# AlvinYH/Faster-VoxelPose

Measured on AMD Instinct MI355X. Metric: frames/sec at 5-view 80x80x20 voxel (heatmaps -> 3D joints); MPJPE vs ref (mm) in mpjpe_vs_ref_mm, higher is better.
Workload: dtype f32

## Files before the change

faster-voxelpose_amd/_capi.py:

```python
import ctypes as C
import os

_HERE = os.path.dirname(os.path.abspath(__file__))
LIB_NAME = "libfvp_hip.so"
ABI_VERSION = 17
LIB_PATH = os.path.join(_HERE, LIB_NAME)

FVP_CAM_FLOATS = 24
FVP_MAX_VIEWS = 8
FVP_MAX_JOINTS = 32
FVP_TRACK_MAX_DETS = 32
FVP_TRACK_MAX_TRACKS = 64
FVP_VIS_MAX_PEOPLE = 32
FVP_VIS_MAX_PRIMS = 64

OP_CONV, OP_POOL2, OP_CONVT2 = 0, 1, 2
EPI_RELU, EPI_RES, EPI_RES_AFTER_RELU = 1, 2, 4
K_PROJECT_WHOLE, K_PROJECT_TRIPLANE, K_CONV, K_SOFTARGMAX, K_OTHER, K_CONV_WINO, K_BACKBONE, K_CONV_WINO_SMALL, K_COUNT = 0, 1, 2, 3, 4, 5, 6, 7, 8
BB_CONV, BB_MAXPOOL, BB_DECONV = 0, 1, 2
BB_OUT_HEAT = 8
BB_STEM = 16
INGEST_SWAP_RB, INGEST_GENERAL = 1, 2
YUV_BT601_LIMITED, YUV_BT709_LIMITED, YUV_BT601_FULL, YUV_BT709_FULL = 0, 1, 2, 3


class FvpGeom(C.Structure):
    _fields_ = [("clamp_max", C.c_float), ("rt", C.c_float * 6), ("hm_w", C.c_float), ("hm_h", C.c_float),
                ("img_w", C.c_float), ("img_h", C.c_float), ("W", C.c_int32), ("H", C.c_int32),
                ("V", C.c_int32), ("J", C.c_int32), ("JP", C.c_int32)]


class FvpConvOp(C.Structure):
    _fields_ = [("kind", C.c_int32), ("src", C.c_int32), ("dst", C.c_int32), ("res", C.c_int32),
                ("cin", C.c_int32), ("cout", C.c_int32), ("kh", C.c_int32), ("kw", C.c_int32),
                ("h", C.c_int32), ("w", C.c_int32), ("flags", C.c_int32), ("w_off", C.c_int32),
                ("e_off", C.c_int32), ("cinp", C.c_int32), ("coutp", C.c_int32), ("wino_off", C.c_int32), ("pair_off", C.c_int32)]


class FvpBbOp(C.Structure):
    _fields_ = [(n, C.c_int32) for n in ("kind", "src", "dst", "res", "cin", "cinp", "cout", "coutp", "cbuf", "kh", "kw",
                                         "stride", "pad", "h", "w", "oh", "ow", "flags", "w_off", "e_off")]


_P = C.c_void_p
_I = C.c_int
_F = C.c_float
_G = C.POINTER(FvpGeom)

SIGNATURES = {
    "fvp_version": [],
    "fvp_diag_build": [],
    "fvp_sizeof": [_I],
    "fvp_error_string": [_I],
    "fvp_heatmaps_to_cl": [_P, _P, _I, _G, _P],
    "fvp_sample_grid": [_P, _P, _P, _I, _I, _I, _P, _G, _P, _P],
    "fvp_project_whole": [_P, _P, _P, _P, _P, _P, _I, _I, _I, _I, _G, _P, _P, _P],
    "fvp_project_columns": [_P, _P, _P, _P, _P, _P, _I, _I, _I, _I, _G, _P, _I, _P, _P],
    "fvp_joint_evidence": [_P, _P, _P, _P, _I, _I, _G, _P, _P, _P],
    "fvp_track_update": [_P, _P, _P, _P, _P, _P, _P, _P, _P, _I, _I, _I, _I, _I, _F, _I, _P],
    "fvp_track_smooth": [_P] * 12 + [_I] * 5 + [_F] * 6 + [_I, _P],
    "fvp_zmax": [_P, _P, C.c_long, _I, _P],
    "fvp_person_boxes": [_P, _I, _P, _P, _P, _P, _P],
    "fvp_project_individual": [_P, _P, _P, _P, _P, _P, _P, _P, _P, _P, _I, _I, _G, _P, _P],
    "fvp_triplane_max": [_P, _P, _I, _I, _I, _P],
    "fvp_project_individual_triplane": [_P, _P, _P, _P, _P, _P, _P, _P, _P, _P, _I, _I, _G, _P, _I, _P, _P],
    "fvp_conv_stack_run": [C.POINTER(FvpConvOp), _I, _P, C.POINTER(_P), _I, _I, _P, _I, _P],
    "fvp_conv_stack_run_fused_1d": [C.POINTER(FvpConvOp), _I, _P, _P, _P, _I, _P],
    "fvp_pack_conv": [_P, _P, _P, _P, _P, _P, _F, _I, C.POINTER(FvpConvOp), _P, _P],
    "fvp_nms_topk": [_P, _I, _I, _I, _I, _P, _P, _P, _P],
    "fvp_gather_proposals": [_P, _P, _P, _I, _I, _I, _I, _I, _I, _P, _P, _P, _P],
    "fvp_proposals": [_P, _P, _P, _P, _P, _F, _I, _I, _I, _P, _P, _P, _P],
    "fvp_proposal_layer": [_P, _P, _P, _P, _F, _I, _I, _P, _P],
    "fvp_softargmax_weightnet": [_P, _P, _P, _F, _I, _I, _I, _I, _I, _P, _P, _P, _P, _P],
    "fvp_pack_weightnet": [_P, _P, _P, _P, _P, _P, _F, _P, _P, _P, _P, _I, _I, _P, _P],
    "fvp_fuse_poses": [_P, _P, _P, _P, _P, _I, _I, _P, _P, _P, _P],
    "fvp_rasterise_heatmaps": [_P, _P, _I, _I, _I, _I, _I, C.c_double, C.c_double, C.c_double, _P, _P, _I, _P],
    "fvp_ingest_frames": [_P, _I, _I, _I, C.POINTER(_F), C.POINTER(_F), C.POINTER(_F), _I, _I, _I, _P, _P, _P],
    "fvp_ingest_nv12": [_P, _P, _I, _I, _I, C.c_long, C.c_long, C.c_long, C.c_long, _I, C.POINTER(_F), C.POINTER(_F),
                        C.POINTER(_F), _I, _I, _P, _P, _P],
    "fvp_draw_poses": [_P, _I, _I, _I, _I, _P, _P, _P, _I, _I, C.POINTER(C.c_int32), _I, C.POINTER(C.c_uint8), _I, _I, _I, _I,
                       _F, _P],
    "fvp_draw_poses_nv12": [_P, _P, _I, _I, _I, _I, C.c_long, C.c_long, C.c_long, C.c_long, _I, _P, _P, _P, _I, _I,
                            C.POINTER(C.c_int32), _I, C.POINTER(C.c_uint8), _I, _I, _I, _I, _F, _P],
    "fvp_person_rois": [_P, _P, _P, _I, _I, _I, _I, C.c_uint32, _I, _F, _F, _F, _F, _P, _P, _P, _P],
    "fvp_crop_rois": [_P, _I, _I, _I, _P, _I, _I, C.POINTER(_F), C.POINTER(_F), _I, _I, _I, _P, _P, _P],
    "fvp_crop_rois_nv12": [_P, _P, _I, _I, _I, C.c_long, C.c_long, C.c_long, C.c_long, _I, _P, _I, _I, C.POINTER(_F),
                           C.POINTER(_F), _I, _I, _P, _P, _P],
    "fvp_joint_visibility": [_P, _P, _P, _P, _P, _I, _I, _I, _I, C.POINTER(C.c_int32), C.POINTER(_F), _I, _F, _I, _I, _P, _P,
                             _P, _P],
    "fvp_bb_input": [_P, _P, _I, _I, _I, _I, _P],
    "fvp_bb_pack": [_P, _P, _P, _P, _P, _P, _F, C.POINTER(FvpBbOp), _P, _P, _P],
    "fvp_bb_run": [C.POINTER(FvpBbOp), _I, _P, _P, C.POINTER(_P), _I, _I, _P, _I, _P, _P],
    "fvp_bb_tune": [C.POINTER(FvpBbOp), _I, _P, _P, C.POINTER(_P), _I, _I, _P],
    "fvp_prof_enable": [_I],
    "fvp_prof_read": [_I, C.POINTER(C.c_double), C.POINTER(C.c_int64), C.POINTER(C.c_double)],
    "fvp_prof_reset": [],
}
_RESTYPES = {"fvp_error_string": C.c_char_p}


class FvpError(RuntimeError):
    pass


def bind(lib):
    for name, args in SIGNATURES.items():
        fn = getattr(lib, name)
        fn.argtypes = args
        fn.restype = _RESTYPES.get(name, C.c_int)
    return lib


_lib = None


def load():
    global _lib
    if _lib is None:
        if not os.path.isfile(LIB_PATH):
            raise FvpError(
                f"{LIB_PATH} not found: the HIP extension is required (there is no CPU fallback). "
                "Build it with `python -c 'import __graft_entry__ as g; g.build()'` or "
                "`faster-voxelpose_amd/csrc/build.sh`.")
        import torch
        _lib = bind(C.CDLL(LIB_PATH))
        if _lib.fvp_version() != ABI_VERSION:
            raise FvpError("libfvp_hip.so ABI version mismatch (rebuild with faster-voxelpose_amd/csrc/build.sh)")
        if _lib.fvp_sizeof(0) != C.sizeof(FvpGeom) or _lib.fvp_sizeof(1) != C.sizeof(FvpConvOp) \
                or _lib.fvp_sizeof(2) != C.sizeof(FvpBbOp):
            raise FvpError("libfvp_hip.so struct layout differs from the ctypes mirrors in _capi.py")
    return _lib


def check(lib, rc, what=""):
    if rc != 0:
        msg = lib.fvp_error_string(rc)
        raise FvpError(f"{what}: error {rc}: {msg.decode() if msg else '?'}")
```

faster-voxelpose_amd/csrc/fvp_project.hip:

```cpp
#include <hip/hip_runtime.h>

#include <cfloat>
#include <cstdlib>

#include "fvp_common.h"
#include "fvp_geom.h"

namespace fvp {

template <int NV>
__global__ void __launch_bounds__(256) k_heat_to_cl(const float* __restrict__ heat, float* __restrict__ cl,
                                                    int J, int HW) {
  const int pix = blockIdx.x * 256 + threadIdx.x;
  const size_t bv = blockIdx.y;
  if (pix >= HW) return;
  const float* src = heat + bv * size_t(J) * HW + pix;
  float v[4 * NV];
#pragma unroll
  for (int j = 0; j < 4 * NV; ++j) v[j] = (j < J) ? src[size_t(j) * HW] : 0.0f;
  float4* dst = reinterpret_cast<float4*>(cl + (bv * HW + pix) * size_t(4 * NV));
#pragma unroll
  for (int q = 0; q < NV; ++q) dst[q] = make_float4(v[4 * q], v[4 * q + 1], v[4 * q + 2], v[4 * q + 3]);
}

__global__ void __launch_bounds__(256) k_sample_grid(const float* __restrict__ ax, const float* __restrict__ ay,
                                                     const float* __restrict__ az, int nx, int ny, int nz,
                                                     const Cam* __restrict__ cams, FvpGeom g,
                                                     float* __restrict__ grid) {
  const int n = nx * ny * nz;
  const int i = blockIdx.x * 256 + threadIdx.x;
  const int v = blockIdx.y;
  if (i >= n) return;
  const int iz = i % nz, iy = (i / nz) % ny, ix = i / (nz * ny);
  float gx, gy;
  project_norm(cams[v], g, ax[ix], ay[iy], az[iz], gx, gy);
  grid[(size_t(v) * n + i) * 2 + 0] = gx;
  grid[(size_t(v) * n + i) * 2 + 1] = gy;
}

template <int NV>
__device__ __forceinline__ void backproject_point(const float* __restrict__ heat_cl_frame,
                                                  const Cam* __restrict__ cams, const FvpGeom& g, float wx,
                                                  float wy, float wz, float (&acc)[4 * NV]) {
  const size_t view_stride = size_t(g.H) * g.W * (4 * NV);
  for (int v = 0; v < g.V; ++v) {
    float gx, gy;
    project_norm(cams[v], g, wx, wy, wz, gx, gy);
    const Taps t = bilinear_taps(gx, gy, g.W, g.H);
    float s[4 * NV];
    if (t.inside) {
      sample_view<NV>(heat_cl_frame + v * view_stride, t, s);
    } else {
#pragma unroll
      for (int c = 0; c < 4 * NV; ++c) s[c] = 0.0f;
    }
#pragma unroll
    for (int c = 0; c < 4 * NV; ++c) acc[c] = (v == 0) ? s[c] : __fadd_rn(acc[c], s[c]);
  }
  const float nv = float(g.V);
#pragma unroll
  for (int c = 0; c < 4 * NV; ++c) acc[c] = clampf(__fdiv_rn(acc[c], nv), 0.0f, 1.0f);
}

__global__ void __launch_bounds__(256)
k_joint_evidence(const float* __restrict__ heat_cl, const Cam* __restrict__ cams, const int* __restrict__ frame_set,
                 const float* __restrict__ fused, int B, int N, FvpGeom g, float* __restrict__ views,
                 float* __restrict__ conf) {
  const int i = blockIdx.x * 256 + threadIdx.x;
  const int J = g.J, JP = g.JP;
  if (i >= B * N * J) return;
  const int bn = i / J, j = i - bn * J;
  const int b = bn / N, n = bn - b * N;
  const bool valid = fused[size_t(bn) * J * 5 + 3] >= 0.0f;
  const float* p = fused + size_t(i) * 5;
  const float wx = p[0], wy = p[1], wz = p[2];
  const size_t view_stride = size_t(g.H) * g.W * JP;
  const float* frame = heat_cl + size_t(b) * g.V * view_stride;
  const Cam* cm = cams + size_t(frame_set[b]) * g.V;
  float acc = 0.0f;
  for (int v = 0; v < g.V; ++v) {
    float px = 0.0f, py = 0.0f, depth = 0.0f, s = 0.0f;
    if (valid) {
      float gx, gy;
      project_pixel(cm[v], wx, wy, wz, px, py, depth);
      pixel_to_norm(g, px, py, gx, gy);
      const Taps t = bilinear_taps(gx, gy, g.W, g.H);
      if (t.inside) {
        const float* cl = frame + v * view_stride + j;
        float h[4];
#pragma unroll
        for (int k = 0; k < 4; ++k) h[k] = ((t.inside >> k) & 1) ? cl[size_t(t.off[k]) * JP] : 0.0f;
        s = __fmul_rn(h[0], t.w[0]);
#pragma unroll
        for (int k = 1; k < 4; ++k) s = __fmaf_rn(h[k], t.w[k], s);
      }
    }
    acc = (v == 0) ? s : __fadd_rn(acc, s);
    if (views)
      reinterpret_cast<float4*>(views)[((size_t(b) * g.V + v) * N + n) * J + j] = make_float4(px, py, depth, s);
  }
  if (conf) conf[i] = clampf(__fdiv_rn(acc, float(g.V)), 0.0f, 1.0f);
}

struct VisPrims {
  int n;
  int ik[FVP_VIS_MAX_PRIMS];
  float r[FVP_VIS_MAX_PRIMS];
};

__device__ __forceinline__ float dot3(float p0, float p1, float p2, float q0, float q1, float q2) {
  return __fadd_rn(__fadd_rn(__fmul_rn(p0, q0), __fmul_rn(p1, q1)), __fmul_rn(p2, q2));
}

__global__ void __launch_bounds__(256)
k_joint_visibility(const float* __restrict__ fused, const Cam* __restrict__ cams, const int* __restrict__ frame_set,
                   const int* __restrict__ ids, const float* __restrict__ views, int V, int N, int J, VisPrims prm,
                   float guard, float xmax, float ymax, int* __restrict__ occluder, float* __restrict__ vis_conf,
                   int* __restrict__ vis_count) {
  __shared__ float4 pose[FVP_VIS_MAX_PEOPLE * FVP_MAX_JOINTS];
  __shared__ int present[FVP_VIS_MAX_PEOPLE];
  __shared__ float seen_s[FVP_MAX_VIEWS * FVP_MAX_JOINTS];
  __shared__ int seen[FVP_MAX_VIEWS * FVP_MAX_JOINTS];
  const int b = blockIdx.x / N, n = blockIdx.x - b * N;
  const int tid = threadIdx.x;
  const float* frame = fused + size_t(b) * N * J * 5;
  for (int q = tid; q < N * J; q += 256) {
    const float x = frame[q * 5 + 0], y = frame[q * 5 + 1], z = frame[q * 5 + 2];
    const bool fin = fabsf(x) <= FLT_MAX && fabsf(y) <= FLT_MAX && fabsf(z) <= FLT_MAX;
    pose[q] = make_float4(x, y, z, fin ? 1.0f : 0.0f);
  }
  if (tid < N) present[tid] = frame[tid * J * 5 + 3] >= 0.0f && (!ids || ids[b * N + tid] >= 0);
  __syncthreads();
  const int v = tid / J, j = tid - v * J;
  if (v < V) {
    const Cam& cm = cams[size_t(frame_set[b]) * V + v];
    const float c0 = cm.T[0], c1 = cm.T[1], c2 = cm.T[2];
    const float4 P = pose[n * J + j];
    const float d10 = __fsub_rn(P.x, c0), d11 = __fsub_rn(P.y, c1), d12 = __fsub_rn(P.z, c2);
    const float a = dot3(d10, d11, d12, d10, d11, d12);
    const float len = sqrtf(a);
    int occ = -2;
    if (present[n] && P.w != 0.0f && len > guard) {
      const float smax = __fsub_rn(1.0f, __fdiv_rn(guard, len));
      float best = 0.0f;
      occ = -1;
      for (int m = 0; m < N; ++m) {
        if (!present[m]) continue;
        for (int l = 0; l < prm.n; ++l) {
          const int pi = prm.ik[l] & 255, pk = prm.ik[l] >> 8;
          const float4 A = pose[m * J + pi], Bq = pose[m * J + pk];
          if (A.w == 0.0f || Bq.w == 0.0f || (m == n && (pi == j || pk == j))) continue;
          const float d20 = __fsub_rn(Bq.x, A.x), d21 = __fsub_rn(Bq.y, A.y), d22 = __fsub_rn(Bq.z, A.z);
          const float r00 = __fsub_rn(c0, A.x), r01 = __fsub_rn(c1, A.y), r02 = __fsub_rn(c2, A.z);
          const float e = dot3(d20, d21, d22, d20, d21, d22);
          const float f = dot3(d20, d21, d22, r00, r01, r02);
          const float c = dot3(d10, d11, d12, r00, r01, r02);
          float sv, tv;
          if (e == 0.0f) {
            tv = 0.0f;
            sv = clampf(__fdiv_rn(-c, a), 0.0f, smax);
          } else {
            const float bb = dot3(d10, d11, d12, d20, d21, d22);
            const float den = __fsub_rn(__fmul_rn(a, e), __fmul_rn(bb, bb));
            sv = den > 0.0f ? clampf(__fdiv_rn(__fsub_rn(__fmul_rn(bb, f), __fmul_rn(c, e)), den), 0.0f, smax) : 0.0f;
            tv = __fdiv_rn(__fadd_rn(__fmul_rn(bb, sv), f), e);
            if (tv < 0.0f) {
              tv = 0.0f;
              sv = clampf(__fdiv_rn(-c, a), 0.0f, smax);
            } else if (tv > 1.0f) {
              tv = 1.0f;
              sv = clampf(__fdiv_rn(__fsub_rn(bb, c), a), 0.0f, smax);
            }
          }
          const float w0 = __fsub_rn(__fadd_rn(c0, __fmul_rn(d10, sv)), __fadd_rn(A.x, __fmul_rn(d20, tv)));
          const float w1 = __fsub_rn(__fadd_rn(c1, __fmul_rn(d11, sv)), __fadd_rn(A.y, __fmul_rn(d21, tv)));
          const float w2 = __fsub_rn(__fadd_rn(c2, __fmul_rn(d12, sv)), __fadd_rn(A.z, __fmul_rn(d22, tv)));
          const float rr = __fmul_rn(prm.r[l], prm.r[l]);
          if (dot3(w0, w1, w2, w0, w1, w2) <= rr && (occ < 0 || sv < best)) {
            best = sv;
            occ = m;
          }
        }
      }
    }
    const size_t o = ((size_t(b) * V + v) * N + n) * J + j;
    if (occluder) occluder[o] = occ;
    if (views) {
      const float4 e4 = reinterpret_cast<const float4*>(views)[o];
      seen[tid] = occ == -1 && e4.z > 0.0f && e4.x >= 0.0f && e4.x <= xmax && e4.y >= 0.0f && e4.y <= ymax;
      seen_s[tid] = e4.w;
    }
  }
  if (!views) return;
  __syncthreads();
  if (tid < J) {
    float sum = 0.0f;
    int cnt = 0;
    for (int u = 0; u < V; ++u)
      if (seen[u * J + tid]) {
        sum = __fadd_rn(sum, seen_s[u * J + tid]);
        ++cnt;
      }
    const size_t o = (size_t(b) * N + n) * J + tid;
    if (vis_conf) vis_conf[o] = cnt ? clampf(__fdiv_rn(sum, float(cnt)), 0.0f, 1.0f) : 0.0f;
    if (vis_count) vis_count[o] = cnt;
  }
}

template <int NV>
__global__ void __launch_bounds__(256)
k_project_whole(const float* __restrict__ heat_cl, const Cam* __restrict__ cams, const int* __restrict__ frame_set,
                const float* __restrict__ ax, const float* __restrict__ ay, const float* __restrict__ az, int X,
                int Y, int Z, FvpGeom g, float* __restrict__ cubes, float* __restrict__ zmax) {
  __shared__ float sm[4 * NV][256];
  const int cpb = 256 / Z;
  const int b = blockIdx.y;
  const int t = threadIdx.x;
  const int cl_ = t / Z, z = t - cl_ * Z;
  const int col = blockIdx.x * cpb + cl_;
  const int ncol = X * Y;
  const bool active = cl_ < cpb && col < ncol;
  const int J = g.J;
  float acc[4 * NV];
#pragma unroll
  for (int c = 0; c < 4 * NV; ++c) acc[c] = 0.0f;
  if (active) {
    const int x = col / Y, y = col - x * Y;
    const float* frame = heat_cl + size_t(b) * g.V * g.H * g.W * (4 * NV);
    backproject_point<NV>(frame, cams + size_t(frame_set[b]) * g.V, g, ax[x], ay[y], az[z], acc);
    if (cubes) {
      const size_t vox = size_t(col) * Z + z;
      const size_t nvox = size_t(ncol) * Z;
#pragma unroll
      for (int c = 0; c < 4 * NV; ++c)
        if (c < J) cubes[(size_t(b) * J + c) * nvox + vox] = acc[c];
    }
  }
  if (zmax) {
#pragma unroll
    for (int c = 0; c < 4 * NV; ++c) sm[c][t] = acc[c];
    __syncthreads();
    for (int item = t; item < cpb * J; item += 256) {
      const int c = item / cpb, k = item - c * cpb;
      const int cc = blockIdx.x * cpb + k;
      if (cc < ncol) {
        float m = sm[c][k * Z];
        for (int zz = 1; zz < Z; ++zz) m = fmaxf(m, sm[c][k * Z + zz]);
        zmax[(size_t(b) * J + c) * ncol + cc] = m;
      }
    }
  }
}

template <int NV>
__global__ void __launch_bounds__(256)
k_project_individual(const float* __restrict__ heat_cl, const Cam* __restrict__ cams,
                     const int* __restrict__ frame_set, const int* __restrict__ person_frame,
                     const uint8_t* __restrict__ person_valid, const int* __restrict__ boxes,
                     const float* __restrict__ fx, const float* __restrict__ fy, const float* __restrict__ fz, int C,
                     FvpGeom g, float* __restrict__ cubes) {
  const int p = blockIdx.y;
  const int lv = blockIdx.x * 256 + threadIdx.x;
  const int nvox = C * C * C;
  if (lv >= nvox) return;
  const int J = g.J;
  const int lz = lv % C, ly = (lv / C) % C, lx = lv / (C * C);
  const int* bx = boxes + p * 9;
  const int gx_ = bx[0] + lx, gy_ = bx[1] + ly, gz_ = bx[2] + lz;
  bool in = (!person_valid || person_valid[p]);
  in = in && bx[3] < bx[6] && bx[4] < bx[7] && bx[5] < bx[8];
  in = in && gx_ >= bx[3] && gx_ < bx[6] && gy_ >= bx[4] && gy_ < bx[7] && gz_ >= bx[5] && gz_ < bx[8];
  float acc[4 * NV];
#pragma unroll
  for (int c = 0; c < 4 * NV; ++c) acc[c] = 0.0f;
  if (in) {
    const int b = person_frame[p];
    const float* frame = heat_cl + size_t(b) * g.V * g.H * g.W * (4 * NV);
    backproject_point<NV>(frame, cams + size_t(frame_set[b]) * g.V, g, fx[gx_], fy[gy_], fz[gz_], acc);
  }
#pragma unroll
  for (int c = 0; c < 4 * NV; ++c)
    if (c < J) cubes[(size_t(p) * J + c) * nvox + lv] = acc[c];
}

template <int PER>
__global__ void __launch_bounds__(256)
k_triplane_max(const float* __restrict__ cubes, float* __restrict__ planes, int J, int C) {
  HIP_DYNAMIC_SHARED(float, slab)
  const int j = blockIdx.x, p = blockIdx.y, t = threadIdx.x;
  const int CC = C * C, ld = C + 1;
  const float* cube = cubes + (size_t(p) * J + j) * CC * C;
  float* pxy = planes + ((size_t(p) * 3 + 0) * J + j) * CC;
  float* pxz = planes + ((size_t(p) * 3 + 1) * J + j) * CC;
  float* pyz = planes + ((size_t(p) * 3 + 2) * J + j) * CC;
  float run[PER];
#pragma unroll
  for (int i = 0; i < PER; ++i) run[i] = -INFINITY;
  for (int x = 0; x < C; ++x) {
    __syncthreads();
    int ncell = CC;
    FVP_OPAQUE(ncell);
#pragma unroll
    for (int i = 0; i < PER; ++i) {
      const int cell = t + i * 256;
      if (cell < ncell) {
        const float v = cube[size_t(x) * CC + cell];
        slab[(cell / C) * ld + (cell % C)] = v;
        run[i] = fmaxf(run[i], v);
      }
    }
    __syncthreads();
    for (int r = t; r < 2 * C; r += 256) {
      if (r < C) {
        float m = slab[r * ld];
        for (int z = 1; z < C; ++z) m = fmaxf(m, slab[r * ld + z]);
        pxy[x * C + r] = m;
      } else {
        const int z = r - C;
        float m = slab[z];
        for (int y = 1; y < C; ++y) m = fmaxf(m, slab[y * ld + z]);
        pxz[x * C + z] = m;
      }
    }
  }
#pragma unroll
  for (int i = 0; i < PER; ++i) {
    const int cell = t + i * 256;
    if (cell < CC) pyz[cell] = run[i];
  }
}

struct TapD {
  int off[4];
  float w[4];
  int inside;
};

template <int SRC>
__device__ __forceinline__ int quad_bcast_i(int v) {
  return __builtin_amdgcn_update_dpp(0, v, SRC * 0x55, 0xf, 0xf, false);
}
template <int SRC>
__device__ __forceinline__ TapD quad_bcast(const TapD& t) {
  TapD r;
#pragma unroll
  for (int k = 0; k < 4; ++k) {
    r.off[k] = quad_bcast_i<SRC>(t.off[k]);
    r.w[k] = __int_as_float(quad_bcast_i<SRC>(__float_as_int(t.w[k])));
  }
  r.inside = quad_bcast_i<SRC>(t.inside);
  return r;
}

__device__ __forceinline__ TapD make_taps(const Cam& cm, const FvpGeom& g, float wx, float wy, float wz) {
  float gx, gy;
  project_norm(cm, g, wx, wy, wz, gx, gy);
  const Taps t = bilinear_taps(gx, gy, g.W, g.H);
  TapD d;
#pragma unroll
  for (int k = 0; k < 4; ++k) { d.off[k] = t.off[k]; d.w[k] = t.w[k]; }
  d.inside = t.inside;
  return d;
}

__device__ __forceinline__ void sample4(const float* __restrict__ cl, int JP, int ch0, const TapD& t, bool first,
                                        float (&acc)[4]) {
  float4 v[4];
#pragma unroll
  for (int k = 0; k < 4; ++k) {
    const bool in = (t.inside >> k) & 1;
    v[k] = *reinterpret_cast<const float4*>(cl + size_t(in ? t.off[k] : 0) * JP + ch0);
    if (!in) v[k] = make_float4(0.f, 0.f, 0.f, 0.f);
  }
  float s[4] = {__fmul_rn(v[0].x, t.w[0]), __fmul_rn(v[0].y, t.w[0]), __fmul_rn(v[0].z, t.w[0]),
                __fmul_rn(v[0].w, t.w[0])};
#pragma unroll
  for (int k = 1; k < 4; ++k) {
    s[0] = __fmaf_rn(v[k].x, t.w[k], s[0]);
    s[1] = __fmaf_rn(v[k].y, t.w[k], s[1]);
    s[2] = __fmaf_rn(v[k].z, t.w[k], s[2]);
    s[3] = __fmaf_rn(v[k].w, t.w[k], s[3]);
  }
#pragma unroll
  for (int i = 0; i < 4; ++i) acc[i] = first ? s[i] : __fadd_rn(acc[i], s[i]);
}

template <int NVL>
__device__ __forceinline__ void whole_point_quad(const float* __restrict__ frame, const Cam* __restrict__ cm,
                                                 const FvpGeom& g, int q, bool active, float wx, float wy, float wz,
                                                 float (&out)[NVL][4]) {
  const int JP = g.JP;
  const size_t view_stride = size_t(g.H) * g.W * JP;
  float acc[NVL][4];
#pragma unroll
  for (int n = 0; n < NVL; ++n)
#pragma unroll
    for (int i = 0; i < 4; ++i) acc[n][i] = 0.0f;
  TapD mine;
  mine.inside = 0;
#pragma unroll
  for (int k = 0; k < 4; ++k) { mine.off[k] = 0; mine.w[k] = 0.0f; }
  if (active && q < g.V) mine = make_taps(cm[q], g, wx, wy, wz);
  auto add_view = [&](const TapD& tv, int v) {
#pragma unroll
    for (int n = 0; n < NVL; ++n) {
      const int ch0 = 16 * n + 4 * q;
      if (ch0 < JP) {
        if (tv.inside) sample4(frame + v * view_stride, JP, ch0, tv, v == 0, acc[n]);
        else if (v == 0) { acc[n][0] = acc[n][1] = acc[n][2] = acc[n][3] = 0.0f; }
      }
    }
  };
  { const TapD tv = quad_bcast<0>(mine); if (active) add_view(tv, 0); }
  if (g.V > 1) { const TapD tv = quad_bcast<1>(mine); if (active) add_view(tv, 1); }
  if (g.V > 2) { const TapD tv = quad_bcast<2>(mine); if (active) add_view(tv, 2); }
  if (g.V > 3) { const TapD tv = quad_bcast<3>(mine); if (active) add_view(tv, 3); }
  for (int v = 4; v < g.V; ++v)
    if (active) add_view(make_taps(cm[v], g, wx, wy, wz), v);
  const float nv = float(g.V);
#pragma unroll
  for (int n = 0; n < NVL; ++n)
#pragma unroll
    for (int i = 0; i < 4; ++i) out[n][i] = clampf(__fdiv_rn(acc[n][i], nv), 0.0f, 1.0f);
}

template <int NVL>
__global__ void __launch_bounds__(1024)
k_project_whole_q(const float* __restrict__ heat_cl, const Cam* __restrict__ cams,
                  const int* __restrict__ frame_set, const float* __restrict__ ax, const float* __restrict__ ay,
                  const float* __restrict__ az, int X, int Y, int Z, int B, int nblk, FvpGeom g,
                  float* __restrict__ cubes, float* __restrict__ zmax) {
  __shared__ float sm[16 * NVL][256];
  const int cpb = 256 / Z;
  int b, bxi;
  if (B % 8 == 0) {
    const int xcd = blockIdx.x & 7, j = blockIdx.x >> 3;
    b = xcd + 8 * (j / nblk);
    bxi = j % nblk;
  } else {
    b = blockIdx.x / nblk;
    bxi = blockIdx.x % nblk;
  }
  const int t = threadIdx.x, q = t & 3, vl = t >> 2;
  const int cl_ = vl / Z, z = vl - cl_ * Z;
  const int col = bxi * cpb + cl_;
  const int ncol = X * Y;
  const bool active = cl_ < cpb && col < ncol;
  const int J = g.J, JP = g.JP;
  const size_t view_stride = size_t(g.H) * g.W * JP;
  const float* frame = heat_cl + size_t(b) * g.V * view_stride;
  const Cam* cm = cams + size_t(frame_set[b]) * g.V;
  float wx = 0.0f, wy = 0.0f, wz = 0.0f;
  if (active) {
    const int x = col / Y, y = col - x * Y;
    wx = ax[x];
    wy = ay[y];
    wz = az[z];
  }
  float val[NVL][4];
  whole_point_quad<NVL>(frame, cm, g, q, active, wx, wy, wz, val);
  const size_t vox = size_t(col) * Z + z;
  const size_t nvox = size_t(ncol) * Z;
#pragma unroll
  for (int n = 0; n < NVL; ++n)
#pragma unroll
    for (int i = 0; i < 4; ++i) {
      const int c = 16 * n + 4 * q + i;
      const float v = val[n][i];
      if (zmax) sm[c][vl] = active ? v : 0.0f;
      if (cubes && active && c < J) cubes[(size_t(b) * J + c) * nvox + vox] = v;
    }
  if (zmax) {
    __syncthreads();
    for (int item = t; item < cpb * J; item += 1024) {
      const int c = item / cpb, k = item - c * cpb;
      const int cc = bxi * cpb + k;
      if (cc < ncol) {
        float m = sm[c][k * Z];
        for (int zz = 1; zz < Z; ++zz) m = fmaxf(m, sm[c][k * Z + zz]);
        zmax[(size_t(b) * J + c) * ncol + cc] = m;
      }
    }
  }
}

template <int NVL>
__global__ void __launch_bounds__(1024)
k_project_columns_q(const float* __restrict__ heat_cl, const Cam* __restrict__ cams, const int* __restrict__ frame_set,
                    const float* __restrict__ ax, const float* __restrict__ ay, const float* __restrict__ az, int Y,
                    int Z, int ncol, int N, FvpGeom g, const long long* __restrict__ flat, float* __restrict__ feat1d) {
  const int pi = blockIdx.x, b = pi / N;
  const int t = threadIdx.x, q = t & 3, z = t >> 2;
  const long long col = flat[pi];
  const bool active = z < Z && col >= 0 && col < ncol;
  const int J = g.J;
  const size_t view_stride = size_t(g.H) * g.W * g.JP;
  const float* frame = heat_cl + size_t(b) * g.V * view_stride;
  const Cam* cm = cams + size_t(frame_set[b]) * g.V;
  float wx = 0.0f, wy = 0.0f, wz = 0.0f;
  if (active) {
    const int x = int(col) / Y, y = int(col) - x * Y;
    wx = ax[x];
    wy = ay[y];
    wz = az[z];
  }
  float val[NVL][4];
  whole_point_quad<NVL>(frame, cm, g, q, active, wx, wy, wz, val);
#pragma unroll
  for (int n = 0; n < NVL; ++n)
#pragma unroll
    for (int i = 0; i < 4; ++i) {
      const int c = 16 * n + 4 * q + i;
      if (z < Z && c < J) feat1d[(size_t(pi) * J + c) * Z + z] = active ? val[n][i] : 0.0f;
    }
}

#if FVP_DIAG
template <int NVL>
__global__ void __launch_bounds__(1024)
k_project_triplane(const float* __restrict__ heat_cl, const Cam* __restrict__ cams, const int* __restrict__ frame_set,
                   const int* __restrict__ person_frame, const uint8_t* __restrict__ person_valid,
                   const int* __restrict__ boxes, const float* __restrict__ fx, const float* __restrict__ fy,
                   const float* __restrict__ fz, int C, int nP, int chunks, int ppf, FvpGeom g,
                   float* __restrict__ planes) {
  __shared__ float sm_xz[4 * NVL * 4][256];
  __shared__ float sm_xy[16][4 * NVL * 4];
  int p, chunk;
  {
    const int id = blockIdx.x;
    const int bpf = ppf * chunks;
    const int nframes = nP / ppf;
    if (nframes % 8 == 0) {
      const int xcd = id & 7, j = id >> 3;
      const int frame = xcd + 8 * (j / bpf), r = j % bpf;
      p = frame * ppf + r / chunks;
      chunk = r % chunks;
    } else {
      p = id / chunks;
      chunk = id % chunks;
    }
  }
  if (person_valid && !person_valid[p]) return;
  const int* bx = boxes + p * 9;
  const int tl0 = bx[0], tl1 = bx[1], tl2 = bx[2];
  const int s0 = bx[3], s1 = bx[4], s2 = bx[5], e0 = bx[6], e1 = bx[7], e2 = bx[8];
  if (s0 >= e0 || s1 >= e1 || s2 >= e2) return;
  const int t = threadIdx.x, q = t & 3, lane = t & 63, wave = t >> 6;
  const int J = g.J, JP = g.JP, CC = C * C;
  const int rows = 256 / C > 0 ? 256 / C : 1;
  const int cell_l = t >> 2;
  const int cell = chunk * 256 + cell_l;
  const int y = cell / C, z = cell - y * C;
  const int y_first = (chunk * 256) / C;
  if (tl1 + y_first >= e1 || tl1 + y_first + rows - 1 < s1) return;
  const int gy_ = tl1 + y, gz_ = tl2 + z;
  const bool yz_in = y < C && gy_ >= s1 && gy_ < e1 && gz_ >= s2 && gz_ < e2;
  const int b = person_frame[p];
  const size_t view_stride = size_t(g.H) * g.W * JP;
  const float* frame = heat_cl + size_t(b) * g.V * view_stride;
  const Cam* cm = cams + size_t(frame_set[b]) * g.V;
  const float wy = yz_in ? fy[gy_] : 0.0f, wz = yz_in ? fz[gz_] : 0.0f;
  float* pxy = planes + (size_t(p) * 3 + 0) * J * CC;
  float* pxz = planes + (size_t(p) * 3 + 1) * J * CC;
  float* pyz = planes + (size_t(p) * 3 + 2) * J * CC;
  const int wpr = C >= 16 ? C / 16 : 1;
  float run[NVL][4];
#pragma unroll
  for (int n = 0; n < NVL; ++n)
#pragma unroll
    for (int i = 0; i < 4; ++i) run[n][i] = 0.0f;
  const float nv = float(g.V);
  const int lx0 = s0 - tl0, lx1 = e0 - tl0;
  for (int lx = lx0; lx < lx1; ++lx) {
    const float wx = fx[tl0 + lx];
    float acc[NVL][4];
#pragma unroll
    for (int n = 0; n < NVL; ++n)
#pragma unroll
      for (int i = 0; i < 4; ++i) acc[n][i] = 0.0f;
    TapD mine;
    mine.inside = 0;
#pragma unroll
    for (int k = 0; k < 4; ++k) { mine.off[k] = 0; mine.w[k] = 0.0f; }
    if (yz_in && q < g.V) mine = make_taps(cm[q], g, wx, wy, wz);
    auto add_view = [&](const TapD& tv, int v) {
#pragma unroll
      for (int n = 0; n < NVL; ++n) {
        const int ch0 = 16 * n + 4 * q;
        if (ch0 < JP) {
          if (tv.inside) sample4(frame + v * view_stride, JP, ch0, tv, v == 0, acc[n]);
          else if (v == 0) { acc[n][0] = acc[n][1] = acc[n][2] = acc[n][3] = 0.0f; }
        }
      }
    };
    { const TapD tv = quad_bcast<0>(mine); if (yz_in) add_view(tv, 0); }
    if (g.V > 1) { const TapD tv = quad_bcast<1>(mine); if (yz_in) add_view(tv, 1); }
    if (g.V > 2) { const TapD tv = quad_bcast<2>(mine); if (yz_in) add_view(tv, 2); }
    if (g.V > 3) { const TapD tv = quad_bcast<3>(mine); if (yz_in) add_view(tv, 3); }
    for (int v = 4; v < g.V; ++v)
      if (yz_in) add_view(make_taps(cm[v], g, wx, wy, wz), v);
#pragma unroll
    for (int n = 0; n < NVL; ++n)
#pragma unroll
      for (int i = 0; i < 4; ++i) {
        acc[n][i] = clampf(__fdiv_rn(acc[n][i], nv), 0.0f, 1.0f);
        run[n][i] = fmaxf(run[n][i], acc[n][i]);
      }
    __syncthreads();
#pragma unroll
    for (int n = 0; n < NVL; ++n)
#pragma unroll
      for (int i = 0; i < 4; ++i) {
        const int c = 16 * n + 4 * q + i;
        sm_xz[c][cell_l] = acc[n][i];
        float m = acc[n][i];
        const int zw = C < 16 ? C : 16;
        for (int o = (zw >> 1) * 4; o >= 4; o >>= 1) m = fmaxf(m, __shfl_xor(m, o));
        if (C >= 16) { if ((lane >> 2) == 0) sm_xy[wave][c] = m; }
        else if (((lane >> 2) & (zw - 1)) == 0 && c < J && y < C && m > 0.0f) pxy[size_t(c) * CC + lx * C + y] = m;
      }
    __syncthreads();
    if (C >= 16) {
      const int nitem = rows * J;
      if (t < nitem) {
        const int r = t / J, c = t - r * J;
        float m = sm_xy[r * wpr][c];
        for (int k = 1; k < wpr; ++k) m = fmaxf(m, sm_xy[r * wpr + k][c]);
        const int yy = y_first + r;
        if (yy < C && m > 0.0f) pxy[size_t(c) * CC + lx * C + yy] = m;
      }
    }
    for (int item = t; item < J * C; item += 1024) {
      const int c = item / C, zz = item - c * C;
      float m = sm_xz[c][zz];
      for (int r = 1; r < rows; ++r) m = fmaxf(m, sm_xz[c][r * C + zz]);
      if (m > 0.0f) {
        if (chunks > 1) atomicMax(reinterpret_cast<int*>(&pxz[size_t(c) * CC + lx * C + zz]), __float_as_int(m));
        else pxz[size_t(c) * CC + lx * C + zz] = m;
      }
    }
  }
  if (y < C) {
#pragma unroll
    for (int n = 0; n < NVL; ++n)
#pragma unroll
      for (int i = 0; i < 4; ++i) {
        const int c = 16 * n + 4 * q + i;
        if (c < J && run[n][i] > 0.0f) pyz[size_t(c) * CC + y * C + z] = run[n][i];
      }
  }
}

#endif

}
#include "fvp_project_lds.h"
namespace fvp {

__global__ void __launch_bounds__(256) k_zmax(const float* __restrict__ cubes, float* __restrict__ zmax, long n, int Z) {
  const long i = long(blockIdx.x) * 256 + threadIdx.x;
  if (i >= n) return;
  const float* c = cubes + i * Z;
  float m = c[0];
  for (int z = 1; z < Z; ++z) m = fmaxf(m, c[z]);
  zmax[i] = m;
}

__global__ void __launch_bounds__(64)
k_person_boxes(const float* __restrict__ centers, int n, const float* __restrict__ consts, int f0, int f1, int f2,
               int c0, int c1, int c2, int* __restrict__ boxes, float* __restrict__ offset) {
  const int i = blockIdx.x * 64 + threadIdx.x;
  if (i >= n) return;
  const float* pc = centers + size_t(i) * 7;
  const int fine[3] = {f0, f1, f2}, cube[3] = {c0, c1, c2};
  int tl[3], m[3];
  for (int a = 0; a < 3; ++a) {
    const float v = __fadd_rn(__fmul_rn(pc[a], consts[a]), consts[3 + a]);
    tl[a] = int(rintf(v));
    const float whole = consts[6 + a], ind = consts[9 + a];
    float o = __fmul_rn(__fdiv_rn(float(tl[a]), float(fine[a] - 1)), whole);
    o = __fadd_rn(__fsub_rn(o, __fdiv_rn(whole, 2.0f)), __fdiv_rn(ind, 2.0f));
    offset[size_t(i) * 3 + a] = o;
  }
  for (int a = 0; a < 2; ++a) {
    const float r = __fmul_rn(__fdiv_rn(__fsub_rn(1.0f, pc[5 + a]), 2.0f), float(cube[a] - 1));
    m[a] = int(r);
    if (m[a] < 0) m[a] = 0;
  }
  m[2] = 0;
  for (int a = 0; a < 3; ++a) {
    const int s = tl[a] + m[a], e = tl[a] + cube[a] - m[a];
    boxes[i * 9 + a] = tl[a];
    boxes[i * 9 + 3 + a] = s >= 0 ? s : 0;
    boxes[i * 9 + 6 + a] = e <= fine[a] ? e : fine[a];
  }
}

}

using namespace fvp;

#define FVP_NV_SWITCH(nv, CALL)     \
  switch (nv) {                     \
    case 1: { CALL(1); } break;     \
    case 2: { CALL(2); } break;     \
    case 3: { CALL(3); } break;     \
    case 4: { CALL(4); } break;     \
    case 5: { CALL(5); } break;     \
    case 6: { CALL(6); } break;     \
    case 7: { CALL(7); } break;     \
    case 8: { CALL(8); } break;     \
    default: return FVP_ELIMIT;     \
  }

static int check_geom(const FvpGeom* g) {
  if (!g) return FVP_EINVAL;
  if (g->V < 1 || g->V > FVP_MAX_VIEWS || g->J < 1 || g->J > FVP_MAX_JOINTS) return FVP_ELIMIT;
  if (g->JP != 4 * ((g->J + 3) / 4) || g->W < 2 || g->H < 2) return FVP_EINVAL;
  return 0;
}

extern "C" int fvp_heatmaps_to_cl(const float* heat, float* heat_cl, int B, const FvpGeom* g, fvp_stream_t s) {
  FVP_REQUIRE(heat && heat_cl && B >= 0);
  if (int e = check_geom(g)) return e;
  if (B == 0) return 0;
  const int HW = g->H * g->W;
  ProfScope ps(FVP_K_OTHER, as_stream(s));
#define CALL(NV)                                                                                             \
  auto k = &k_heat_to_cl<NV>;                                                                                \
  hipLaunchKernelGGL(k, dim3(ceil_div(HW, 256), B * g->V), dim3(256), 0, as_stream(s), heat, heat_cl, g->J, HW);
  FVP_NV_SWITCH(g->JP / 4, CALL)
#undef CALL
  return launch_status();
}

extern "C" int fvp_sample_grid(const float* ax, const float* ay, const float* az, int nx, int ny, int nz,
                               const float* cams, const FvpGeom* g, float* grid, fvp_stream_t s) {
  FVP_REQUIRE(ax && ay && az && cams && grid && nx > 0 && ny > 0 && nz > 0);
  if (int e = check_geom(g)) return e;
  const int n = nx * ny * nz;
  ProfScope ps(FVP_K_OTHER, as_stream(s));
  hipLaunchKernelGGL(k_sample_grid, dim3(ceil_div(n, 256), g->V), dim3(256), 0, as_stream(s), ax, ay, az, nx, ny,
                     nz, reinterpret_cast<const Cam*>(cams), *g, grid);
  return launch_status();
}

extern "C" int fvp_project_whole(const float* heat_cl, const float* cams, const int32_t* frame_set,
                                 const float* ax, const float* ay, const float* az, int X, int Y, int Z, int B,
                                 const FvpGeom* g, float* cubes, float* zmax, fvp_stream_t s) {
  FVP_REQUIRE(heat_cl && cams && frame_set && ax && ay && az && (cubes || zmax) && X > 0 && Y > 0 && Z > 0);
  if (int e = check_geom(g)) return e;
  FVP_LIMIT(Z <= 256);
  if (B == 0) return 0;
  const int cpb = 256 / Z;
  ProfScope ps(FVP_K_PROJECT_WHOLE, as_stream(s));
  static const bool no_quad = fvp::diag_env("FVP_WHOLE_NO_QUAD") != nullptr;
  const int nvl = ceil_div(g->JP, 16);
  if (!no_quad && nvl <= 2) {
    const int nblk = ceil_div(X * Y, cpb);
    if (nvl == 1)
      hipLaunchKernelGGL(k_project_whole_q<1>, dim3(nblk * B), dim3(1024), 0, as_stream(s), heat_cl,
                         reinterpret_cast<const Cam*>(cams), frame_set, ax, ay, az, X, Y, Z, B, nblk, *g, cubes, zmax);
    else
      hipLaunchKernelGGL(k_project_whole_q<2>, dim3(nblk * B), dim3(1024), 0, as_stream(s), heat_cl,
                         reinterpret_cast<const Cam*>(cams), frame_set, ax, ay, az, X, Y, Z, B, nblk, *g, cubes, zmax);
    return launch_status();
  }
#define CALL(NV)                                                                                              \
  auto k = &k_project_whole<NV>;                                                                              \
  hipLaunchKernelGGL(k, dim3(ceil_div(X * Y, cpb), B), dim3(256), 0, as_stream(s), heat_cl,                   \
                     reinterpret_cast<const Cam*>(cams), frame_set, ax, ay, az, X, Y, Z, *g, cubes, zmax);
  FVP_NV_SWITCH(g->JP / 4, CALL)
#undef CALL
  return launch_status();
}

extern "C" int fvp_joint_evidence(const float* heat_cl, const float* cams, const int32_t* frame_set,
                                  const float* fused_poses, int B, int N, const FvpGeom* g, float* views,
                                  float* joint_conf, fvp_stream_t s) {
  FVP_REQUIRE(heat_cl && cams && frame_set && fused_poses && (views || joint_conf) && B >= 0 && N >= 0);
  if (int e = check_geom(g)) return e;
  FVP_LIMIT(size_t(B) * N * g->J * g->V < (size_t(1) << 29));
  if (B == 0 || N == 0) return 0;
  ProfScope ps(FVP_K_OTHER, as_stream(s));
  hipLaunchKernelGGL(k_joint_evidence, dim3(ceil_div(B * N * g->J, 256)), dim3(256), 0, as_stream(s), heat_cl,
                     reinterpret_cast<const Cam*>(cams), frame_set, fused_poses, B, N, *g, views, joint_conf);
  return launch_status();
}

extern "C" int fvp_joint_visibility(const float* fused_poses, const float* cams, const int32_t* frame_set,
                                    const int32_t* ids, const float* views, int B, int V, int N, int J,
                                    const int32_t* prims, const float* radius_mm, int L, float guard_mm, int Hs, int Ws,
                                    int32_t* occluder, float* vis_conf, int32_t* vis_count, fvp_stream_t s) {
  FVP_REQUIRE(fused_poses && cams && frame_set && ((prims && radius_mm) || L <= 0));
  FVP_REQUIRE((occluder || vis_conf || vis_count) && (views || (!vis_conf && !vis_count)));
  FVP_REQUIRE(B >= 0 && V >= 1 && N >= 1 && J >= 1 && Hs >= 1 && Ws >= 1 && L >= 0);
  FVP_REQUIRE(guard_mm >= 0.0f && guard_mm <= FLT_MAX);
  FVP_LIMIT(N <= FVP_VIS_MAX_PEOPLE && J <= FVP_MAX_JOINTS && V <= FVP_MAX_VIEWS && L <= FVP_VIS_MAX_PRIMS);
  VisPrims prm;
  prm.n = L;
  for (int l = 0; l < FVP_VIS_MAX_PRIMS; ++l) {
    prm.ik[l] = 0;
    prm.r[l] = 0.0f;
    if (l >= L) continue;
    const int i = prims[2 * l], k = prims[2 * l + 1];
    FVP_REQUIRE(i >= 0 && i < J && k >= 0 && k < J && radius_mm[l] > 0.0f && radius_mm[l] <= FLT_MAX);
    prm.ik[l] = i | (k << 8);
    prm.r[l] = radius_mm[l];
  }
  if (B == 0) return 0;
  ProfScope ps(FVP_K_OTHER, as_stream(s));
  hipLaunchKernelGGL(k_joint_visibility, dim3(B * N), dim3(256), 0, as_stream(s), fused_poses,
                     reinterpret_cast<const Cam*>(cams), frame_set, ids, views, V, N, J, prm, guard_mm, float(Ws - 1),
                     float(Hs - 1), occluder, vis_conf, vis_count);
  return launch_status();
}

extern "C" int fvp_project_columns(const float* heat_cl, const float* cams, const int32_t* frame_set, const float* ax,
                                   const float* ay, const float* az, int X, int Y, int Z, int B, const FvpGeom* g,
                                   const int64_t* flat, int N, float* feat1d, fvp_stream_t s) {
  FVP_REQUIRE(heat_cl && cams && frame_set && ax && ay && az && flat && feat1d && X > 0 && Y > 0 && Z > 0 && N > 0);
  if (int e = check_geom(g)) return e;
  FVP_LIMIT(Z <= 256 && g->JP <= 32);
  if (B == 0) return 0;
  ProfScope ps(FVP_K_PROJECT_WHOLE, as_stream(s));
  const int threads = ceil_div(4 * Z, 64) * 64;
  if (g->JP <= 16)
    hipLaunchKernelGGL(k_project_columns_q<1>, dim3(B * N), dim3(threads), 0, as_stream(s), heat_cl,
                       reinterpret_cast<const Cam*>(cams), frame_set, ax, ay, az, Y, Z, X * Y, N, *g,
                       reinterpret_cast<const long long*>(flat), feat1d);
  else
    hipLaunchKernelGGL(k_project_columns_q<2>, dim3(B * N), dim3(threads), 0, as_stream(s), heat_cl,
                       reinterpret_cast<const Cam*>(cams), frame_set, ax, ay, az, Y, Z, X * Y, N, *g,
                       reinterpret_cast<const long long*>(flat), feat1d);
  return launch_status();
}

extern "C" int fvp_zmax(const float* cubes, float* zmax, long n, int Z, fvp_stream_t s) {
  FVP_REQUIRE(cubes && zmax && n >= 0 && Z > 0);
  if (n == 0) return 0;
  hipLaunchKernelGGL(k_zmax, dim3(unsigned((n + 255) / 256)), dim3(256), 0, as_stream(s), cubes, zmax, n, Z);
  return launch_status();
}

extern "C" int fvp_person_boxes(const float* centers, int n, const float* consts, const int32_t* fine_cube,
                                int32_t* boxes, float* offset, fvp_stream_t s) {
  FVP_REQUIRE(centers && consts && fine_cube && boxes && offset && n >= 0);
  if (n == 0) return 0;
  hipLaunchKernelGGL(k_person_boxes, dim3(ceil_div(n, 64)), dim3(64), 0, as_stream(s), centers, n, consts,
                     fine_cube[0], fine_cube[1], fine_cube[2], fine_cube[3], fine_cube[4], fine_cube[5], boxes,
                     offset);
  return launch_status();
}

static int check_cube(int C) {
  if (C < 4 || C > 256 || (C & (C - 1)) != 0) return FVP_ELIMIT;
  return 0;
}

extern "C" int fvp_project_individual(const float* heat_cl, const float* cams, const int32_t* frame_set,
                                      const int32_t* person_frame, const uint8_t* person_valid,
                                      const int32_t* boxes, const float* fx, const float* fy, const float* fz,
                                      const int32_t* fine, int C, int nP, const FvpGeom* g, float* cubes,
                                      fvp_stream_t s) {
  FVP_REQUIRE(heat_cl && cams && frame_set && person_frame && boxes && fx && fy && fz && cubes && nP >= 0);
  (void)fine;
  if (int e = check_geom(g)) return e;
  if (int e = check_cube(C)) return e;
  if (nP == 0) return 0;
  ProfScope ps(FVP_K_OTHER, as_stream(s));
#define CALL(NV)                                                                                                 \
  auto k = &k_project_individual<NV>;                                                                            \
  hipLaunchKernelGGL(k, dim3(ceil_div(C * C * C, 256), nP), dim3(256), 0, as_stream(s), heat_cl,                 \
                     reinterpret_cast<const Cam*>(cams), frame_set, person_frame, person_valid, boxes, fx, fy, fz, \
                     C, *g, cubes);
  FVP_NV_SWITCH(g->JP / 4, CALL)
#undef CALL
  return launch_status();
}

extern "C" int fvp_triplane_max(const float* cubes, float* planes, int nP, int J, int C, fvp_stream_t s) {
  FVP_REQUIRE(cubes && planes && nP >= 0 && J > 0);
  if (int e = check_cube(C)) return e;
  FVP_LIMIT(C <= 128);
  if (nP == 0) return 0;
  ProfScope ps(FVP_K_OTHER, as_stream(s));
  const int per = (C * C + 255) / 256;
  const dim3 grid(J, nP);
  const size_t lds = size_t(C) * (C + 1) * sizeof(float);
#define FVP_TRIMAX(PER_) hipLaunchKernelGGL(k_triplane_max<PER_>, grid, dim3(256), lds, as_stream(s), cubes, planes, J, C)
  if (per <= 1) FVP_TRIMAX(1);
  else if (per <= 4) FVP_TRIMAX(4);
  else if (per <= 16) FVP_TRIMAX(16);
  else FVP_TRIMAX(64);
#undef FVP_TRIMAX
  return launch_status();
}

extern "C" int fvp_project_individual_triplane(const float* heat_cl, const float* cams, const int32_t* frame_set,
                                               const int32_t* person_frame, const uint8_t* person_valid,
                                               const int32_t* boxes, const float* fx, const float* fy,
                                               const float* fz, const int32_t* fine, int C, int nP, const FvpGeom* g,
                                               float* planes, int persons_per_frame, const float* fine_grid,
                                               fvp_stream_t s) {
  FVP_REQUIRE(heat_cl && cams && frame_set && person_frame && boxes && fx && fy && fz && planes && nP >= 0);
  FVP_REQUIRE(!fine_grid || fine);
  if (int e = check_geom(g)) return e;
  if (int e = check_cube(C)) return e;
  if (nP == 0) return 0;
  const int ppf = (persons_per_frame > 0 && nP % persons_per_frame == 0) ? persons_per_frame : nP;
  [[maybe_unused]] const int chunks = ceil_div(C * C, 256);
  const int nvl = ceil_div(g->JP, 16);
  ProfScope ps(FVP_K_PROJECT_TRIPLANE, as_stream(s));
  const int F0 = fine_grid ? fine[0] : 0, F1 = fine_grid ? fine[1] : 0, F2 = fine_grid ? fine[2] : 0;
  const int nby = ceil_div(C, kBY);
#if FVP_DIAG
  const int nbx = ceil_div(C, kBX);
  static const bool gather = fvp::diag_env("FVP_TRIPLANE_GATHER") != nullptr;
  const bool quad_form = fvp::diag_env("FVP_TRIPLANE_QUAD") != nullptr;
  static const int tri_ablate_env = fvp::diag_env("FVP_TRI_ABLATE") ? atoi(fvp::diag_env("FVP_TRI_ABLATE")) : 0;
  const char* tt_env = fvp::diag_env("FVP_TRI_TWO_TILE");
  const bool staged = fvp::diag_env("FVP_TRIPLANE_STAGED") != nullptr;
  const bool force_lane = fvp::diag_env("FVP_TRIPLANE_LANE") != nullptr;
  const bool lane_form = !gather && !quad_form && g->JP <= 20 && ((staged && g->JP != 16) || force_lane);
  const int tri_ablate = (tri_ablate_env & ~16) | ((tt_env ? atoi(tt_env) != 0 : lane_form) ? 16 : 0);
  auto cap_lim = [](int cap) { const char* e = fvp::diag_env("FVP_TRI_CAP_PX"); const int v = e ? atoi(e) : cap; return v > 0 && v < cap ? v : cap; };
  const int cap_px = int((36 * 1024) / (size_t(g->JP) * 4));
  const size_t lds = 2 * size_t(cap_px) * g->JP * 4 + 64;
  if (lane_form) {
    const int lq = (g->JP / 4) | 1;
    const int cap_px = int((36 * 1024) / (size_t(lq) * 16));
    const size_t lds = 2 * size_t(cap_px) * lq * 16 + 64;
    FVP_LIMIT(size_t(cap_px) * lq * 4 >= size_t(kBX * kBY + (kBX + kBY) * 32) * g->JP);
#define CALL2(NQ_, CACHED_)                                                                                       \
  {                                                                                                                \
    static LdsOptIn optin;                                                                                         \
    auto k = &k_project_triplane_lds2<NQ_, CACHED_>;                                                              \
    if (int e = lds_opt_in(optin, reinterpret_cast<const void*>(k), lds)) return e;                                \
    hipLaunchKernelGGL(k, dim3(nbx * nby * nP), dim3(kTriThreads), lds, as_stream(s), heat_cl,                     \
                       reinterpret_cast<const Cam*>(cams), frame_set, person_frame, person_valid, boxes, fx, fy, fz, C, \
                       nP, nbx, nby, ppf, cap_px, *g, fine_grid, F0, F1, F2, planes, tri_ablate, cap_lim(cap_px));                  \
  }
#define CASE2(NQ_) case NQ_: if (fine_grid) CALL2(NQ_, true) else CALL2(NQ_, false) break;
    switch (g->JP / 4) {
      CASE2(1) CASE2(2) CASE2(3) CASE2(4) CASE2(5)
      default: return FVP_ELIMIT;
    }
#undef CASE2
#undef CALL2
    return launch_status();
  }
  const bool blk_form = !gather && !quad_form && !staged;
#else
  constexpr bool blk_form = true;
#endif
  if (blk_form && nvl <= 2) {
    const int nbx2 = ceil_div(C, kBlkBX);
    const int bz = nvl == 2 ? 16 : kBlkBZ;
    int zsh = 0;
    while ((1 << zsh) < C) ++zsh;
    const size_t lds_z = (size_t(kBlkBX + kBY) << zsh) * (g->JP + 1) * 4;
#if FVP_DIAG
    const char* zr_env = fvp::diag_env("FVP_TRI_ZRES");
    const bool zres = zr_env && atoi(zr_env) != 0 && (1 << zsh) >= bz && lds_z <= kTriZresMaxLds;
#else
    constexpr bool zres = false;
#endif
    const size_t lds_b = zres ? lds_z : size_t(kBlkBX * kBY + (kBlkBX + kBY) * bz) * (g->JP + 1) * 4;
#define CALLB(NVL_, CACHED_, ZRES_)                                                                                          \
  hipLaunchKernelGGL((k_project_triplane_blk<NVL_, CACHED_, ZRES_>), dim3(nbx2 * nby * nP), dim3(kBlkThreads), lds_b,       \
                     as_stream(s), heat_cl, reinterpret_cast<const Cam*>(cams), frame_set, person_frame, person_valid, boxes, \
                     fx, fy, fz, C, nP, nbx2, nby, ppf, *g, fine_grid, F0, F1, F2, planes, zsh)
#if FVP_DIAG
#define CALLB2(NVL_)                                                                     \
  {                                                                                      \
    if (fine_grid) { if (zres) CALLB(NVL_, true, true); else CALLB(NVL_, true, false); } \
    else { if (zres) CALLB(NVL_, false, true); else CALLB(NVL_, false, false); }         \
  }
#else
#define CALLB2(NVL_)                                                                     \
  {                                                                                      \
    if (fine_grid) CALLB(NVL_, true, false); else CALLB(NVL_, false, false);             \
  }
#endif
    const bool q5 = nvl == 2 && g->JP == 20 && !zres && fvp::diag_env("FVP_TRI_NO_Q5") == nullptr;
    if (q5) {
      if (fine_grid)
        hipLaunchKernelGGL((k_project_triplane_blk<2, true, false, true>), dim3(nbx2 * nby * nP), dim3(kBlkThreads), lds_b, as_stream(s),
                           heat_cl, reinterpret_cast<const Cam*>(cams), frame_set, person_frame, person_valid, boxes, fx, fy, fz, C, nP,
                           nbx2, nby, ppf, *g, fine_grid, F0, F1, F2, planes, zsh);
      else
        hipLaunchKernelGGL((k_project_triplane_blk<2, false, false, true>), dim3(nbx2 * nby * nP), dim3(kBlkThreads), lds_b, as_stream(s),
                           heat_cl, reinterpret_cast<const Cam*>(cams), frame_set, person_frame, person_valid, boxes, fx, fy, fz, C, nP,
                           nbx2, nby, ppf, *g, fine_grid, F0, F1, F2, planes, zsh);
    } else if (nvl == 2) CALLB2(2) else CALLB2(1)
#undef CALLB2
#undef CALLB
    return launch_status();
  }
#if FVP_DIAG
  if (!gather && nvl <= 2) {
    FVP_LIMIT(cap_px >= kBX * kBY + (kBX + kBY) * (nvl == 1 ? 32 : 16));
#define CALL(NVL_, CACHED_)                                                                                        \
  {                                                                                                                \
    static LdsOptIn optin;                                                                                         \
    auto k = &k_project_triplane_lds<NVL_, CACHED_>;                                                               \
    if (int e = lds_opt_in(optin, reinterpret_cast<const void*>(k), lds)) return e;                                \
    hipLaunchKernelGGL(k, dim3(nbx * nby * nP), dim3(kTriThreads), lds, as_stream(s), heat_cl,                     \
                       reinterpret_cast<const Cam*>(cams), frame_set, person_frame, person_valid, boxes, fx, fy, fz, C, \
                       nP, nbx, nby, ppf, cap_px, *g, fine_grid, F0, F1, F2, planes, tri_ablate, cap_lim(cap_px));                  \
  }
    if (nvl == 1) {
      if (fine_grid) CALL(1, true) else CALL(1, false)
    } else {
      if (fine_grid) CALL(2, true) else CALL(2, false)
    }
#undef CALL
    return launch_status();
  }
  if (nvl == 1) {
    auto k = &k_project_triplane<1>;
    hipLaunchKernelGGL(k, dim3(chunks * nP), dim3(1024), 0, as_stream(s), heat_cl, reinterpret_cast<const Cam*>(cams),
                       frame_set, person_frame, person_valid, boxes, fx, fy, fz, C, nP, chunks, ppf, *g, planes);
  } else if (nvl == 2) {
    auto k = &k_project_triplane<2>;
    hipLaunchKernelGGL(k, dim3(chunks * nP), dim3(1024), 0, as_stream(s), heat_cl, reinterpret_cast<const Cam*>(cams),
                       frame_set, person_frame, person_valid, boxes, fx, fy, fz, C, nP, chunks, ppf, *g, planes);
  } else {
    return FVP_ELIMIT;
  }
  return launch_status();
#else
  return FVP_ELIMIT;
#endif
}
```

faster-voxelpose_amd/csrc/fvp_project_lds.h:

```cpp
#pragma once
#include <type_traits>
#include <climits>

namespace fvp {

typedef float f32x2 __attribute__((ext_vector_type(2)));
#ifndef FVP_TRI_PACKED
#define FVP_TRI_PACKED 1
#endif
#ifndef FVP_TRI_EXPLICIT_AS
#define FVP_TRI_EXPLICIT_AS 1
#endif

typedef float f32x4v __attribute__((ext_vector_type(4)));
__device__ __forceinline__ float4 lds_ld4(const float* p) {
  const f32x4v v = *(const __attribute__((address_space(3))) f32x4v*)p;
  return make_float4(v.x, v.y, v.z, v.w);
}
__device__ __forceinline__ float4 glb_ld4(const float* p) {
  const f32x4v v = *(const __attribute__((address_space(1))) f32x4v*)p;
  return make_float4(v.x, v.y, v.z, v.w);
}

struct TapL {
  int base;
  int dx, dy;
  float w[4];
};

template <int SRC>
__device__ __forceinline__ TapL quad_bcast_l(const TapL& t) {
  TapL r;
  r.base = quad_bcast_i<SRC>(t.base);
  r.dx = quad_bcast_i<SRC>(t.dx);
  r.dy = quad_bcast_i<SRC>(t.dy);
#pragma unroll
  for (int k = 0; k < 4; ++k) r.w[k] = __int_as_float(quad_bcast_i<SRC>(__float_as_int(t.w[k])));
  return r;
}

__device__ __forceinline__ void tap_origin(float gx, float gy, int W, int H, int& x0, int& y0, float (&w)[4], int& inside) {
  const float ix = __fmul_rn(__fadd_rn(gx, 1.0f), 0.5f * float(W - 1));
  const float iy = __fmul_rn(__fadd_rn(gy, 1.0f), 0.5f * float(H - 1));
  const float x0f = floorf(ix), y0f = floorf(iy);
  const float x1f = __fadd_rn(x0f, 1.0f), y1f = __fadd_rn(y0f, 1.0f);
  w[0] = __fmul_rn(__fsub_rn(x1f, ix), __fsub_rn(y1f, iy));
  w[1] = __fmul_rn(__fsub_rn(ix, x0f), __fsub_rn(y1f, iy));
  w[2] = __fmul_rn(__fsub_rn(x1f, ix), __fsub_rn(iy, y0f));
  w[3] = __fmul_rn(__fsub_rn(ix, x0f), __fsub_rn(iy, y0f));
  x0 = int(x0f);
  y0 = int(y0f);
  const bool x0in = x0 >= 0 && x0 < W, x1in = x0 + 1 >= 0 && x0 + 1 < W;
  const bool y0in = y0 >= 0 && y0 < H, y1in = y0 + 1 >= 0 && y0 + 1 < H;
  inside = (x0in && y0in ? 1 : 0) | (x1in && y0in ? 2 : 0) | (x0in && y1in ? 4 : 0) | (x1in && y1in ? 8 : 0);
}

__device__ __forceinline__ int imax(int a, int b) { return a > b ? a : b; }
__device__ __forceinline__ int imin(int a, int b) { return a < b ? a : b; }
template <int CTRL>
__device__ __forceinline__ int dpp_i(int v) { return __builtin_amdgcn_update_dpp(0, v, CTRL, 0xf, 0xf, false); }
__device__ __forceinline__ int row_max(int v) {
  v = imax(v, dpp_i<0xB1>(v));
  v = imax(v, dpp_i<0x4E>(v));
  v = imax(v, dpp_i<0x141>(v));
  v = imax(v, dpp_i<0x140>(v));
  return v;
}

__device__ __forceinline__ void plane_max(float* cell, int vv) { atomicMax(reinterpret_cast<int*>(cell), vv); }

constexpr int kBX = 8, kBY = 4;
constexpr int kTriThreads = kBX * kBY * 4 * 4;

#if FVP_DIAG
template <int NVL, bool CACHED>
__global__ void __launch_bounds__(kTriThreads, 4)
k_project_triplane_lds(const float* __restrict__ heat_cl, const Cam* __restrict__ cams, const int* __restrict__ frame_set,
                       const int* __restrict__ person_frame, const uint8_t* __restrict__ person_valid,
                       const int* __restrict__ boxes, const float* __restrict__ fx, const float* __restrict__ fy,
                       const float* __restrict__ fz, int C, int nP, int nbx, int nby, int ppf, int cap_px, FvpGeom g,
                       const float* __restrict__ fgrid, int F0, int F1, int F2, float* __restrict__ planes, int ablate, int cap_lim) {
  constexpr int BZ = NVL == 1 ? 32 : 16;
  constexpr int VPT = BZ / 4;
  constexpr int OWN = VPT / 4;
  HIP_DYNAMIC_SHARED(float, smem)
  constexpr int NT = kTriThreads;
  const int J = g.J, JP = g.JP, CC = C * C, V = g.V, W = g.W, H = g.H;
  const int tile_sz = cap_px * JP;
  int* rect = reinterpret_cast<int*>(smem + 2 * size_t(tile_sz));
  int p, blk;
  {
    const int id = blockIdx.x;
    const int bpp = nbx * nby, bpf = ppf * bpp;
    const int nframes = nP / ppf;
    if (nframes % 8 == 0) {
      const int xcd = id & 7, j = id >> 3;
      const int frame = xcd + 8 * (j / bpf), r = j % bpf;
      p = frame * ppf + r / bpp;
      blk = r % bpp;
    } else {
      p = id / bpp;
      blk = id % bpp;
    }
  }
  if (person_valid && !person_valid[p]) return;
  const int* bx = boxes + p * 9;
  const int tl0 = bx[0], tl1 = bx[1], tl2 = bx[2];
  const int s0 = bx[3], s1 = bx[4], s2 = bx[5], e0 = bx[6], e1 = bx[7], e2 = bx[8];
  if (s0 >= e0 || s1 >= e1 || s2 >= e2) return;
  const int xb = blk / nby, yb = blk - xb * nby;
  const int gx0 = s0 + xb * kBX, gy0 = s1 + yb * kBY;
  if (gx0 >= e0 || gy0 >= e1) return;

  const int t = threadIdx.x, q = t & 3, lane = t & 63, wave = t >> 6;
  const int slot = t >> 2, zs = slot & 3, yy = (slot >> 2) & (kBY - 1), xx = slot / (4 * kBY);
  const int gxi = gx0 + xx, gyi = gy0 + yy;
  const bool col_in = gxi < e0 && gyi < e1;
  const int b = person_frame[p];
  const size_t view_stride = size_t(H) * W * JP;
  const float* frame = heat_cl + size_t(b) * V * view_stride;
  const Cam* cm = cams + size_t(frame_set[b]) * V;
  const float wx = col_in ? fx[gxi] : 0.0f, wy = col_in ? fy[gyi] : 0.0f;
  const size_t nfine = size_t(F0) * F1 * F2;
  const float2* gcol = CACHED ? reinterpret_cast<const float2*>(fgrid) + size_t(frame_set[b]) * V * nfine +
                                    (size_t(col_in ? gxi : 0) * F1 + (col_in ? gyi : 0)) * F2
                              : nullptr;
  float* pxy = planes + (size_t(p) * 3 + 0) * J * CC;
  float* pxz = planes + (size_t(p) * 3 + 1) * J * CC;
  float* pyz = planes + (size_t(p) * 3 + 2) * J * CC;
  const float nv = float(V);
  const int qn = JP >> 2;
  const unsigned m_qn = unsigned((1ull << 32) / unsigned(qn)) + 1u;

  struct Own { int xy[OWN]; int inside[OWN]; float w[OWN][4]; };
  float2 crd[OWN];
  auto load_coords = [&](int v, int gz0) {
#pragma unroll
    for (int k = 0; k < OWN; ++k) {
      const int gzi = gz0 + zs + 4 * (q + 4 * k);
      crd[k] = gcol[size_t(v) * nfine + (gzi < F2 ? gzi : F2 - 1)];
    }
  };
  auto project = [&](int v, int gz0, Own& o) {
    int mnx = INT_MIN, mxx = INT_MIN, mny = INT_MIN, mxy = INT_MIN;
#pragma unroll
    for (int k = 0; k < OWN; ++k) {
      const int gzi = gz0 + zs + 4 * (q + 4 * k);
      const bool vin = col_in && gzi < e2;
      o.inside[k] = 0;
      o.xy[k] = 0;
      o.w[k][0] = o.w[k][1] = o.w[k][2] = o.w[k][3] = 0.0f;
      if (vin) {
        float sx, sy;
        if (CACHED) {
          sx = crd[k].x;
          sy = crd[k].y;
        } else {
          project_norm(cm[v], g, wx, wy, fz[gzi], sx, sy);
        }
        int x0, y0;
        tap_origin(sx, sy, W, H, x0, y0, o.w[k], o.inside[k]);
        o.xy[k] = int((unsigned(y0) << 16) | (unsigned(x0) & 0xffffu));
        if (o.inside[k]) {
          mnx = imax(mnx, -imax(x0, 0)); mxx = imax(mxx, imin(x0 + 1, W - 1));
          mny = imax(mny, -imax(y0, 0)); mxy = imax(mxy, imin(y0 + 1, H - 1));
        }
      }
    }
    mnx = row_max(mnx); mxx = row_max(mxx); mny = row_max(mny); mxy = row_max(mxy);
    if ((lane & 15) == 0 && mxx != INT_MIN) {
      int* rc = rect + 4 * (v % 3);
      atomicMax(&rc[0], mnx); atomicMax(&rc[1], mxx); atomicMax(&rc[2], mny); atomicMax(&rc[3], mxy);
    }
  };
  struct Rect { int x0, y0, w, h, pitch; bool any, staged, big, lds; };
  auto read_rect = [&](int v) {
    const int* rc = rect + 4 * (v % 3);
    const int c0 = __builtin_amdgcn_readfirstlane(rc[0]), c1 = __builtin_amdgcn_readfirstlane(rc[1]);
    const int c2 = __builtin_amdgcn_readfirstlane(rc[2]), c3 = __builtin_amdgcn_readfirstlane(rc[3]);
    Rect r;
    r.any = c1 != INT_MIN;
    r.x0 = r.any ? -c0 : 0;
    r.y0 = r.any ? -c2 : 0;
    r.w = r.any ? c1 - r.x0 + 1 : 0;
    r.h = r.any ? c3 - r.y0 + 1 : 0;
    r.pitch = r.w | 1;
    r.staged = r.any && r.h * r.pitch <= cap_lim;
    r.big = r.any && !r.staged && r.h * r.pitch <= 2 * cap_lim && (ablate & 16);
    r.lds = r.staged || r.big;
    return r;
  };
  auto issue_dma = [&](int v, const Rect& r) {
    if (!r.lds || (ablate & 2)) return;
    float* tile = r.big ? smem : smem + (v & 1) * tile_sz;
    const float* plane = frame + size_t(v) * view_stride + (size_t(r.y0) * W + r.x0) * JP;
    const int pq = r.pitch * qn;
    for (int c0 = 0; c0 < pq; c0 += 64) {
      const int col = c0 + lane;
      int px = qn == 4 ? col >> 2 : (qn == 1 ? col : int(__umulhi(unsigned(col), m_qn)));
      const int cq = col - px * qn;
      px = px < r.w ? px : r.w - 1;
      const float* src0 = plane + size_t(px) * JP + 4 * cq;
      for (int row = wave; row < r.h; row += NT / 64) {
        if (col < pq)
          __builtin_amdgcn_global_load_lds((const __attribute__((address_space(1))) void*)(src0 + size_t(row) * W * JP),
                                           (__attribute__((address_space(3))) void*)(tile + size_t(row * pq + c0) * 4), 16, 0, 0);
      }
    }
  };
  auto finish = [&](const Own& o, int k, const Rect& r) {
    TapL d;
    const int x0 = (o.xy[k] << 16) >> 16, y0 = o.xy[k] >> 16;
    const int rx0 = r.lds ? r.x0 : 0, ry0 = r.lds ? r.y0 : 0;
    const int rx1 = r.lds ? r.x0 + r.w - 1 : W - 1, ry1 = r.lds ? r.y0 + r.h - 1 : H - 1;
    const int pitch = r.lds ? r.pitch : W;
    const int cx0 = imin(imax(x0, rx0), rx1), cx1 = imin(imax(x0 + 1, rx0), rx1);
    const int cy0 = imin(imax(y0, ry0), ry1), cy1 = imin(imax(y0 + 1, ry0), ry1);
    d.base = ((cy0 - ry0) * pitch + (cx0 - rx0)) * JP;
    d.dx = (cx1 - cx0) * JP;
    d.dy = (cy1 - cy0) * pitch * JP;
#pragma unroll
    for (int c = 0; c < 4; ++c) d.w[c] = ((o.inside[k] >> c) & 1) ? o.w[k][c] : 0.0f;
    return d;
  };

  for (int gz0 = s2; gz0 < e2; gz0 += BZ) {
    if (t < 12) rect[t] = INT_MIN;
    __syncthreads();
    float acc[VPT][NVL][4];
#pragma unroll
    for (int i = 0; i < VPT; ++i)
#pragma unroll
      for (int n = 0; n < NVL; ++n)
#pragma unroll
        for (int c = 0; c < 4; ++c) acc[i][n][c] = 0.0f;

    Own cur, nxt;
    if (CACHED) load_coords(0, gz0);
    project(0, gz0, cur);
    __syncthreads();
    Rect rcur = read_rect(0);
    if (rcur.staged) issue_dma(0, rcur);
    if (CACHED && V > 1) load_coords(1, gz0);
    for (int v = 0; v < V; ++v) {
      if (v + 1 < V) project(v + 1, gz0, nxt);
      wait_vmcnt(0);
      __syncthreads();
      Rect rnxt = rcur;
      if (v + 1 < V) rnxt = read_rect(v + 1);
      if (rcur.big) {
        issue_dma(v, rcur);
        if (CACHED && v + 2 < V) load_coords(v + 2, gz0);
        wait_vmcnt(0);
        __syncthreads();
      } else if (v + 1 < V) {
        if (rnxt.staged) issue_dma(v + 1, rnxt);
        if (CACHED && v + 2 < V) load_coords(v + 2, gz0);
      }
      if (t < 4) rect[4 * (v % 3) + t] = INT_MIN;
      if (rcur.any && !(ablate & 1) && (rcur.lds || !(ablate & 8))) {
        const bool from_lds = rcur.lds;
        const float* lsrc = smem + ((rcur.big || !(v & 1)) ? 0 : tile_sz);
        const float* gsrc = frame + size_t(v) * view_stride;
        constexpr bool EXPLICIT_AS = (FVP_TRI_EXPLICIT_AS == 1) ? NVL > 1 : (FVP_TRI_EXPLICIT_AS > 1);
        const float* src = from_lds ? lsrc : gsrc;
        auto sample = [&](const TapL& tv, float (&a)[NVL][4]) {
#pragma unroll
          for (int n = 0; n < NVL; ++n) {
            const int ch0 = 16 * n + 4 * q;
            if (ch0 < JP) {
              float4 v0, v1, v2, v3;
              if constexpr (!EXPLICIT_AS) {
                const float* p0 = src + tv.base + ch0;
                v0 = *reinterpret_cast<const float4*>(p0);
                v1 = *reinterpret_cast<const float4*>(p0 + tv.dx);
                v2 = *reinterpret_cast<const float4*>(p0 + tv.dy);
                v3 = *reinterpret_cast<const float4*>(p0 + tv.dy + tv.dx);
              } else if (from_lds) {
                const float* p0 = lsrc + tv.base + ch0;
                v0 = lds_ld4(p0);
                v1 = lds_ld4(p0 + tv.dx);
                v2 = lds_ld4(p0 + tv.dy);
                v3 = lds_ld4(p0 + tv.dy + tv.dx);
              } else {
                const float* p0 = gsrc + tv.base + ch0;
                v0 = glb_ld4(p0);
                v1 = glb_ld4(p0 + tv.dx);
                v2 = glb_ld4(p0 + tv.dy);
                v3 = glb_ld4(p0 + tv.dy + tv.dx);
              }
#if FVP_TRI_PACKED
              const f32x2 w0 = f32x2{tv.w[0], tv.w[0]}, w1 = f32x2{tv.w[1], tv.w[1]}, w2 = f32x2{tv.w[2], tv.w[2]},
                          w3 = f32x2{tv.w[3], tv.w[3]};
              f32x2 lo = f32x2{v0.x, v0.y} * w0, hi = f32x2{v0.z, v0.w} * w0;
              lo = __builtin_elementwise_fma(f32x2{v1.x, v1.y}, w1, lo);
              hi = __builtin_elementwise_fma(f32x2{v1.z, v1.w}, w1, hi);
              lo = __builtin_elementwise_fma(f32x2{v2.x, v2.y}, w2, lo);
              hi = __builtin_elementwise_fma(f32x2{v2.z, v2.w}, w2, hi);
              lo = __builtin_elementwise_fma(f32x2{v3.x, v3.y}, w3, lo);
              hi = __builtin_elementwise_fma(f32x2{v3.z, v3.w}, w3, hi);
              const f32x2 alo = f32x2{a[n][0], a[n][1]} + lo, ahi = f32x2{a[n][2], a[n][3]} + hi;
              a[n][0] = alo.x; a[n][1] = alo.y; a[n][2] = ahi.x; a[n][3] = ahi.y;
#else
              float s0_ = __fmul_rn(v0.x, tv.w[0]), s1_ = __fmul_rn(v0.y, tv.w[0]);
              float s2_ = __fmul_rn(v0.z, tv.w[0]), s3_ = __fmul_rn(v0.w, tv.w[0]);
              s0_ = __fmaf_rn(v1.x, tv.w[1], s0_); s1_ = __fmaf_rn(v1.y, tv.w[1], s1_);
              s2_ = __fmaf_rn(v1.z, tv.w[1], s2_); s3_ = __fmaf_rn(v1.w, tv.w[1], s3_);
              s0_ = __fmaf_rn(v2.x, tv.w[2], s0_); s1_ = __fmaf_rn(v2.y, tv.w[2], s1_);
              s2_ = __fmaf_rn(v2.z, tv.w[2], s2_); s3_ = __fmaf_rn(v2.w, tv.w[2], s3_);
              s0_ = __fmaf_rn(v3.x, tv.w[3], s0_); s1_ = __fmaf_rn(v3.y, tv.w[3], s1_);
              s2_ = __fmaf_rn(v3.z, tv.w[3], s2_); s3_ = __fmaf_rn(v3.w, tv.w[3], s3_);
              a[n][0] = __fadd_rn(a[n][0], s0_); a[n][1] = __fadd_rn(a[n][1], s1_);
              a[n][2] = __fadd_rn(a[n][2], s2_); a[n][3] = __fadd_rn(a[n][3], s3_);
#endif
            }
          }
        };
#pragma unroll
        for (int k = 0; k < OWN; ++k) {
          const TapL mine = finish(cur, k, rcur);
          { const TapL tv = quad_bcast_l<0>(mine); sample(tv, acc[4 * k + 0]); }
          { const TapL tv = quad_bcast_l<1>(mine); sample(tv, acc[4 * k + 1]); }
          { const TapL tv = quad_bcast_l<2>(mine); sample(tv, acc[4 * k + 2]); }
          { const TapL tv = quad_bcast_l<3>(mine); sample(tv, acc[4 * k + 3]); }
        }
      }
      if (rcur.big) {
        __syncthreads();
        if (v + 1 < V && rnxt.staged) issue_dma(v + 1, rnxt);
      }
      cur = nxt;
      rcur = rnxt;
    }
    __syncthreads();
    if (ablate & 4) continue;
    int* cxy = reinterpret_cast<int*>(smem);
    int* cxz = cxy + kBX * kBY * JP;
    int* cyz = cxz + kBX * BZ * JP;
    const int ncell = (kBX * kBY + (kBX + kBY) * BZ) * JP;
    for (int i = t; i < ncell; i += NT) cxy[i] = 0;
    __syncthreads();
#pragma unroll
    for (int n = 0; n < NVL; ++n)
#pragma unroll
      for (int c = 0; c < 4; ++c) {
        const int ch = 16 * n + 4 * q + c;
        float mz = 0.0f;
#pragma unroll
        for (int i = 0; i < VPT; ++i) {
          const float val = fmaxf(acc[i][n][c], 0.0f);
          mz = fmaxf(mz, val);
          if (val > 0.0f && ch < JP) {
            const int z = zs + 4 * i;
            atomicMax(&cxz[(xx * BZ + z) * JP + ch], __float_as_int(val));
            atomicMax(&cyz[(yy * BZ + z) * JP + ch], __float_as_int(val));
          }
        }
        int mi = __float_as_int(mz);
        mi = imax(mi, dpp_i<0x124>(mi));
        mi = imax(mi, dpp_i<0x128>(mi));
        if (zs == 0 && mi > 0 && ch < JP) cxy[(xx * kBY + yy) * JP + ch] = mi;
      }
    __syncthreads();
    const int lz0 = gz0 - tl2;
    for (int i = t; i < kBX * kBY * J; i += NT) {
      const int ch = i / (kBX * kBY), col = i - ch * (kBX * kBY), cx = col / kBY, cy = col - cx * kBY;
      const int raw = cxy[col * JP + ch];
      if (raw > 0 && gx0 + cx < e0 && gy0 + cy < e1) {
        const int vv = __float_as_int(clampf(__fdiv_rn(__int_as_float(raw), nv), 0.0f, 1.0f));
        if (vv > 0) plane_max(&pxy[size_t(ch) * CC + (gx0 + cx - tl0) * C + (gy0 + cy - tl1)], vv);
      }
    }
    for (int i = t; i < (kBX + kBY) * BZ * J; i += NT) {
      const int ch = i / ((kBX + kBY) * BZ), r = i - ch * ((kBX + kBY) * BZ), a = r / BZ, z = r - a * BZ;
      if (gz0 + z < e2) {
        const int raw = cxz[r * JP + ch];
        const int vv = raw > 0 ? __float_as_int(clampf(__fdiv_rn(__int_as_float(raw), nv), 0.0f, 1.0f)) : 0;
        if (vv > 0) {
          if (a < kBX) {
            if (gx0 + a < e0) plane_max(&pxz[size_t(ch) * CC + (gx0 + a - tl0) * C + lz0 + z], vv);
          } else if (gy0 + a - kBX < e1) {
            plane_max(&pyz[size_t(ch) * CC + (gy0 + a - kBX - tl1) * C + lz0 + z], vv);
          }
        }
      }
    }
    __syncthreads();
  }
}

#endif

#ifndef FVP_TRI_BLK_OCC
#define FVP_TRI_BLK_OCC 4
#endif
#ifndef FVP_TRI_BLK_BX
#define FVP_TRI_BLK_BX 4
#endif
#ifndef FVP_TRI_BLK_BZ
#define FVP_TRI_BLK_BZ 16
#endif
constexpr int kBlkBX = FVP_TRI_BLK_BX, kBlkBZ = FVP_TRI_BLK_BZ;
constexpr int kBlkThreads = kBlkBX * kBY * 4 * 4;
#ifndef FVP_TRI_ZRES_MAX_KB
#define FVP_TRI_ZRES_MAX_KB 48
#endif
constexpr size_t kTriZresMaxLds = size_t(FVP_TRI_ZRES_MAX_KB) * 1024;
template <int NVL, bool CACHED, bool ZRES, bool Q5 = false>
__global__ void __launch_bounds__(kBlkThreads, FVP_TRI_BLK_OCC)
k_project_triplane_blk(const float* __restrict__ heat_cl, const Cam* __restrict__ cams, const int* __restrict__ frame_set,
                       const int* __restrict__ person_frame, const uint8_t* __restrict__ person_valid,
                       const int* __restrict__ boxes, const float* __restrict__ fx, const float* __restrict__ fy,
                       const float* __restrict__ fz, int C, int nP, int nbx, int nby, int ppf, FvpGeom g,
                       const float* __restrict__ fgrid, int F0, int F1, int F2, float* __restrict__ planes, int zsh) {
  static_assert(!Q5 || (NVL == 2 && !ZRES), "the five-quad form replaces the two-group form of the per-z-block kernel");
  constexpr int NVA = Q5 ? 1 : NVL;
  constexpr int BZ = NVL == 1 ? kBlkBZ : 16;
  constexpr int VPT = BZ / 4;
  constexpr int OWN = VPT / 4;
  HIP_DYNAMIC_SHARED(float, smem)
  constexpr int NT = kBlkThreads;
  constexpr int kBX = kBlkBX;
  const int J = g.J, JP = g.JP, CC = C * C, V = g.V, W = g.W, H = g.H;
  int p, blk;
  {
    const int id = blockIdx.x;
    const int bpp = nbx * nby, bpf = ppf * bpp;
    const int nframes = nP / ppf;
    if (nframes % 8 == 0) {
      const int xcd = id & 7, j = id >> 3;
      const int frame = xcd + 8 * (j / bpf), r = j % bpf;
      p = frame * ppf + r / bpp;
      blk = r % bpp;
    } else {
      p = id / bpp;
      blk = id % bpp;
    }
  }
  if (person_valid && !person_valid[p]) return;
  const int* bx = boxes + p * 9;
  const int tl0 = bx[0], tl1 = bx[1], tl2 = bx[2];
  const int s0 = bx[3], s1 = bx[4], s2 = bx[5], e0 = bx[6], e1 = bx[7], e2 = bx[8];
  if (s0 >= e0 || s1 >= e1 || s2 >= e2) return;
  const int xb = blk / nby, yb = blk - xb * nby;
  const int gx0 = s0 + xb * kBX, gy0 = s1 + yb * kBY;
  if (gx0 >= e0 || gy0 >= e1) return;

  const int t = threadIdx.x, q = t & 3;
  const int slot = t >> 2, zs = slot & 3, yy = (slot >> 2) & (kBY - 1), xx = slot / (4 * kBY);
  const int gxi = gx0 + xx, gyi = gy0 + yy;
  const bool col_in = gxi < e0 && gyi < e1;
  const int b = person_frame[p];
  const size_t view_stride = size_t(H) * W * JP;
  const float* frame = heat_cl + size_t(b) * V * view_stride;
  const Cam* cm = cams + size_t(frame_set[b]) * V;
  const float wx = col_in ? fx[gxi] : 0.0f, wy = col_in ? fy[gyi] : 0.0f;
  const size_t nfine = size_t(F0) * F1 * F2;
  const float2* gcol = CACHED ? reinterpret_cast<const float2*>(fgrid) + size_t(frame_set[b]) * V * nfine +
                                    (size_t(col_in ? gxi : 0) * F1 + (col_in ? gyi : 0)) * F2
                              : nullptr;
  float* pxy = planes + (size_t(p) * 3 + 0) * J * CC;
  float* pxz = planes + (size_t(p) * 3 + 1) * J * CC;
  float* pyz = planes + (size_t(p) * 3 + 2) * J * CC;
  const float nv = float(V);
  const int JPp = JP + 1;
  [[maybe_unused]] int mxy[NVL][4];
  [[maybe_unused]] const int zt = 1 << zsh;
  if constexpr (ZRES) {
#pragma unroll
    for (int n = 0; n < NVL; ++n)
#pragma unroll
      for (int c = 0; c < 4; ++c) mxy[n][c] = 0;
    int* cz = reinterpret_cast<int*>(smem);
    const int ncell = ((kBX + kBY) << zsh) * JPp;
    for (int i = t; i < ncell; i += NT) cz[i] = 0;
    __syncthreads();
  }

  for (int gz0 = s2; gz0 < e2; gz0 += BZ) {
    float acc[VPT][NVA][4];
#pragma unroll
    for (int i = 0; i < VPT; ++i)
#pragma unroll
      for (int n = 0; n < NVA; ++n)
#pragma unroll
        for (int c = 0; c < 4; ++c) acc[i][n][c] = 0.0f;
    [[maybe_unused]] float accx[OWN][1][4];
#pragma unroll
    for (int kk = 0; kk < OWN; ++kk)
#pragma unroll
      for (int c = 0; c < 4; ++c) accx[kk][0][c] = 0.0f;
    float2 crd[OWN];
    auto load_coords = [&](int v) {
#pragma unroll
      for (int k = 0; k < OWN; ++k) {
        const int gzi = gz0 + zs + 4 * (q + 4 * k);
        crd[k] = gcol[size_t(v) * nfine + (gzi < F2 ? gzi : F2 - 1)];
      }
    };
    if (CACHED) load_coords(0);
    for (int v = 0; v < V; ++v) {
      TapL mine[OWN];
#pragma unroll
      for (int k = 0; k < OWN; ++k) {
        const int gzi = gz0 + zs + 4 * (q + 4 * k);
        const bool vin = col_in && gzi < e2;
        TapL d;
        d.base = d.dx = d.dy = 0;
        d.w[0] = d.w[1] = d.w[2] = d.w[3] = 0.0f;
        if (vin) {
          float sx, sy;
          if (CACHED) {
            sx = crd[k].x;
            sy = crd[k].y;
          } else {
            project_norm(cm[v], g, wx, wy, fz[gzi], sx, sy);
          }
          int x0, y0, inside;
          float w4[4];
          tap_origin(sx, sy, W, H, x0, y0, w4, inside);
          const int cx0 = imin(imax(x0, 0), W - 1), cx1 = imin(imax(x0 + 1, 0), W - 1);
          const int cy0 = imin(imax(y0, 0), H - 1), cy1 = imin(imax(y0 + 1, 0), H - 1);
          d.base = (cy0 * W + cx0) * JP;
          d.dx = (cx1 - cx0) * JP;
          d.dy = (cy1 - cy0) * W * JP;
#pragma unroll
          for (int c = 0; c < 4; ++c) d.w[c] = ((inside >> c) & 1) ? w4[c] : 0.0f;
        }
        mine[k] = d;
      }
      if (CACHED && v + 1 < V) load_coords(v + 1);
#ifdef FVP_TRI_BLK_NOSAMPLE
      if (mine[0].base != -12345) { acc[0][0][0] += mine[0].w[0] + mine[OWN - 1].w[3] + float(mine[0].base); continue; }
#endif
      const float* gsrc = frame + size_t(v) * view_stride;
      auto sample = [&](const TapL& tv, auto& a, auto own) {
        constexpr bool kOwn = decltype(own)::value;
#pragma unroll
        for (int n = 0; n < (kOwn ? 1 : NVA); ++n) {
          const int ch0 = kOwn ? 16 : 16 * n + 4 * q;
          if (kOwn || ch0 < JP) {
            const float* p0 = gsrc + tv.base + ch0;
            const float4 v0 = glb_ld4(p0), v1 = glb_ld4(p0 + tv.dx), v2 = glb_ld4(p0 + tv.dy), v3 = glb_ld4(p0 + tv.dy + tv.dx);
            const f32x2 w0 = f32x2{tv.w[0], tv.w[0]}, w1 = f32x2{tv.w[1], tv.w[1]}, w2 = f32x2{tv.w[2], tv.w[2]},
                        w3 = f32x2{tv.w[3], tv.w[3]};
            f32x2 lo = f32x2{v0.x, v0.y} * w0, hi = f32x2{v0.z, v0.w} * w0;
            lo = __builtin_elementwise_fma(f32x2{v1.x, v1.y}, w1, lo);
            hi = __builtin_elementwise_fma(f32x2{v1.z, v1.w}, w1, hi);
            lo = __builtin_elementwise_fma(f32x2{v2.x, v2.y}, w2, lo);
            hi = __builtin_elementwise_fma(f32x2{v2.z, v2.w}, w2, hi);
            lo = __builtin_elementwise_fma(f32x2{v3.x, v3.y}, w3, lo);
            hi = __builtin_elementwise_fma(f32x2{v3.z, v3.w}, w3, hi);
            const f32x2 alo = f32x2{a[n][0], a[n][1]} + lo, ahi = f32x2{a[n][2], a[n][3]} + hi;
            a[n][0] = alo.x; a[n][1] = alo.y; a[n][2] = ahi.x; a[n][3] = ahi.y;
          }
        }
      };
#pragma unroll
      for (int k = 0; k < OWN; ++k) {
        { const TapL tv = quad_bcast_l<0>(mine[k]); sample(tv, acc[4 * k + 0], std::false_type{}); }
        { const TapL tv = quad_bcast_l<1>(mine[k]); sample(tv, acc[4 * k + 1], std::false_type{}); }
        { const TapL tv = quad_bcast_l<2>(mine[k]); sample(tv, acc[4 * k + 2], std::false_type{}); }
        { const TapL tv = quad_bcast_l<3>(mine[k]); sample(tv, acc[4 * k + 3], std::false_type{}); }
        if constexpr (Q5) sample(mine[k], accx[k], std::true_type{});
      }
    }
#ifdef FVP_TRI_BLK_NOMAX
    if (acc[0][0][0] != 1.2345e-30f) continue;
#endif
    if constexpr (ZRES) {
      int* rxz = reinterpret_cast<int*>(smem);
      int* ryz = rxz + ((kBX << zsh) * JPp);
      const int zb = gz0 - s2 + zs;
#pragma unroll
      for (int n = 0; n < NVL; ++n)
#pragma unroll
        for (int c = 0; c < 4; ++c) {
          const int ch = 16 * n + 4 * q + c;
          float mz = 0.0f;
#pragma unroll
          for (int i = 0; i < VPT; ++i) {
            const float val = fmaxf(acc[i][n][c], 0.0f);
            mz = fmaxf(mz, val);
            if (val > 0.0f && ch < JP) {
              const int z = zb + 4 * i;
              atomicMax(&rxz[((xx << zsh) + z) * JPp + ch], __float_as_int(val));
              atomicMax(&ryz[((yy << zsh) + z) * JPp + ch], __float_as_int(val));
            }
          }
          int mi = __float_as_int(mz);
          mi = imax(mi, dpp_i<0x124>(mi));
          mi = imax(mi, dpp_i<0x128>(mi));
          mxy[n][c] = imax(mxy[n][c], mi);
        }
      continue;
    }
    int* cxy = reinterpret_cast<int*>(smem);
    int* cxz = cxy + kBX * kBY * JPp;
    int* cyz = cxz + kBX * BZ * JPp;
    const int ncell = (kBX * kBY + (kBX + kBY) * BZ) * JPp;
    __syncthreads();
    for (int i = t; i < ncell; i += NT) cxy[i] = 0;
    __syncthreads();
#pragma unroll
    for (int n = 0; n < NVA; ++n)
#pragma unroll
      for (int c = 0; c < 4; ++c) {
        const int ch = 16 * n + 4 * q + c;
        float mz = 0.0f;
#pragma unroll
        for (int i = 0; i < VPT; ++i) {
          const float val = fmaxf(acc[i][n][c], 0.0f);
          mz = fmaxf(mz, val);
          if (val > 0.0f && ch < JP) {
            const int z = zs + 4 * i;
            atomicMax(&cxz[(xx * BZ + z) * JPp + ch], __float_as_int(val));
            atomicMax(&cyz[(yy * BZ + z) * JPp + ch], __float_as_int(val));
          }
        }
        int mi = __float_as_int(mz);
        mi = imax(mi, dpp_i<0x124>(mi));
        mi = imax(mi, dpp_i<0x128>(mi));
        if (zs == 0 && mi > 0 && ch < JP) cxy[(xx * kBY + yy) * JPp + ch] = mi;
      }
    if constexpr (Q5) {
#pragma unroll
      for (int c = 0; c < 4; ++c) {
        const int ch = 16 + c;
        float mz = 0.0f;
#pragma unroll
        for (int kk = 0; kk < OWN; ++kk) {
          const float val = fmaxf(accx[kk][0][c], 0.0f);
          mz = fmaxf(mz, val);
          if (val > 0.0f) {
            const int z = zs + 4 * (4 * kk + q);
            atomicMax(&cxz[(xx * BZ + z) * JPp + ch], __float_as_int(val));
            atomicMax(&cyz[(yy * BZ + z) * JPp + ch], __float_as_int(val));
          }
        }
        int mi = __float_as_int(mz);
        mi = imax(mi, dpp_i<0x121>(mi));
        mi = imax(mi, dpp_i<0x122>(mi));
        mi = imax(mi, dpp_i<0x124>(mi));
        mi = imax(mi, dpp_i<0x128>(mi));
        if (zs == 0 && q == 0 && mi > 0) cxy[(xx * kBY + yy) * JPp + ch] = mi;
      }
    }
    __syncthreads();
    const int lz0 = gz0 - tl2;
    for (int i = t; i < kBX * kBY * J; i += NT) {
      const int ch = i / (kBX * kBY), col = i - ch * (kBX * kBY), cx = col / kBY, cy = col - cx * kBY;
      const int raw = cxy[col * JPp + ch];
      if (raw > 0 && gx0 + cx < e0 && gy0 + cy < e1) {
        const int vv = __float_as_int(clampf(__fdiv_rn(__int_as_float(raw), nv), 0.0f, 1.0f));
        if (vv > 0) plane_max(&pxy[size_t(ch) * CC + (gx0 + cx - tl0) * C + (gy0 + cy - tl1)], vv);
      }
    }
    for (int i = t; i < (kBX + kBY) * BZ * J; i += NT) {
      const int ch = i / ((kBX + kBY) * BZ), r = i - ch * ((kBX + kBY) * BZ), a = r / BZ, z = r - a * BZ;
      if (gz0 + z < e2) {
        const int raw = cxz[r * JPp + ch];
        const int vv = raw > 0 ? __float_as_int(clampf(__fdiv_rn(__int_as_float(raw), nv), 0.0f, 1.0f)) : 0;
        if (vv > 0) {
          if (a < kBX) {
            if (gx0 + a < e0) plane_max(&pxz[size_t(ch) * CC + (gx0 + a - tl0) * C + lz0 + z], vv);
          } else if (gy0 + a - kBX < e1) {
            plane_max(&pyz[size_t(ch) * CC + (gy0 + a - kBX - tl1) * C + lz0 + z], vv);
          }
        }
      }
    }
  }
  if constexpr (ZRES) {
    __syncthreads();
    if (zs == 0 && col_in) {
#pragma unroll
      for (int n = 0; n < NVL; ++n)
#pragma unroll
        for (int c = 0; c < 4; ++c) {
          const int ch = 16 * n + 4 * q + c;
          if (ch < J && mxy[n][c] > 0) {
            const int vv = __float_as_int(clampf(__fdiv_rn(__int_as_float(mxy[n][c]), nv), 0.0f, 1.0f));
            if (vv > 0) plane_max(&pxy[size_t(ch) * CC + (gxi - tl0) * C + (gyi - tl1)], vv);
          }
        }
    }
    const int* cz = reinterpret_cast<const int*>(smem);
    const int nz = e2 - s2, lz0 = s2 - tl2;
    const int rows = (kBX + kBY) << zsh;
    for (int i = t; i < rows * J; i += NT) {
      static_assert(kBX + kBY == 8, "row count is a power of two");
      const int ch = i >> (zsh + 3), r = i & (rows - 1), a = r >> zsh, z = r & (zt - 1);
      if (z < nz) {
        const int raw = cz[r * JPp + ch];
        const int vv = raw > 0 ? __float_as_int(clampf(__fdiv_rn(__int_as_float(raw), nv), 0.0f, 1.0f)) : 0;
        if (vv > 0) {
          if (a < kBX) {
            if (gx0 + a < e0) plane_max(&pxz[size_t(ch) * CC + (gx0 + a - tl0) * C + lz0 + z], vv);
          } else if (gy0 + a - kBX < e1) {
            plane_max(&pyz[size_t(ch) * CC + (gy0 + a - kBX - tl1) * C + lz0 + z], vv);
          }
        }
      }
    }
  }
}

#if FVP_DIAG
template <int NQ, bool CACHED>
__global__ void __launch_bounds__(kTriThreads, 4)
k_project_triplane_lds2(const float* __restrict__ heat_cl, const Cam* __restrict__ cams, const int* __restrict__ frame_set,
                        const int* __restrict__ person_frame, const uint8_t* __restrict__ person_valid,
                        const int* __restrict__ boxes, const float* __restrict__ fx, const float* __restrict__ fy,
                        const float* __restrict__ fz, int C, int nP, int nbx, int nby, int ppf, int cap_px, FvpGeom g,
                        const float* __restrict__ fgrid, int F0, int F1, int F2, float* __restrict__ planes, int ablate, int cap_lim) {
  constexpr int BZ = 32, VPT = 2, JP = 4 * NQ;
  constexpr int LQ = NQ | 1, LP = 4 * LQ;
  HIP_DYNAMIC_SHARED(float, smem)
  constexpr int NT = kTriThreads;
  const int J = g.J, CC = C * C, V = g.V, W = g.W, H = g.H;
  const int tile_sz = cap_px * LP;
  int* rect = reinterpret_cast<int*>(smem + 2 * size_t(tile_sz));
  int p, blk;
  {
    const int id = blockIdx.x;
    const int bpp = nbx * nby, bpf = ppf * bpp;
    const int nframes = nP / ppf;
    if (nframes % 8 == 0) {
      const int xcd = id & 7, j = id >> 3;
      const int frame = xcd + 8 * (j / bpf), r = j % bpf;
      p = frame * ppf + r / bpp;
      blk = r % bpp;
    } else {
      p = id / bpp;
      blk = id % bpp;
    }
  }
  if (person_valid && !person_valid[p]) return;
  const int* bx = boxes + p * 9;
  const int tl0 = bx[0], tl1 = bx[1], tl2 = bx[2];
  const int s0 = bx[3], s1 = bx[4], s2 = bx[5], e0 = bx[6], e1 = bx[7], e2 = bx[8];
  if (s0 >= e0 || s1 >= e1 || s2 >= e2) return;
  const int xb = blk / nby, yb = blk - xb * nby;
  const int gx0 = s0 + xb * kBX, gy0 = s1 + yb * kBY;
  if (gx0 >= e0 || gy0 >= e1) return;

  const int t = threadIdx.x, lane = t & 63, wave = t >> 6;
  const int z16 = t & 15, yy = (t >> 4) & (kBY - 1), xx = t >> 6;
  const int gxi = gx0 + xx, gyi = gy0 + yy;
  const bool col_in = gxi < e0 && gyi < e1;
  const int b = person_frame[p];
  const size_t view_stride = size_t(H) * W * JP;
  const float* frame = heat_cl + size_t(b) * V * view_stride;
  const Cam* cm = cams + size_t(frame_set[b]) * V;
  const float wx = col_in ? fx[gxi] : 0.0f, wy = col_in ? fy[gyi] : 0.0f;
  const size_t nfine = size_t(F0) * F1 * F2;
  const float2* gcol = CACHED ? reinterpret_cast<const float2*>(fgrid) + size_t(frame_set[b]) * V * nfine +
                                    (size_t(col_in ? gxi : 0) * F1 + (col_in ? gyi : 0)) * F2
                              : nullptr;
  float* pxy = planes + (size_t(p) * 3 + 0) * J * CC;
  float* pxz = planes + (size_t(p) * 3 + 1) * J * CC;
  float* pyz = planes + (size_t(p) * 3 + 2) * J * CC;
  const float nv = float(V);

  struct Own { int xy[VPT]; int inside[VPT]; float w[VPT][4]; };
  float2 crd[VPT];
  auto load_coords = [&](int v, int gz0) {
#pragma unroll
    for (int k = 0; k < VPT; ++k) {
      const int gzi = gz0 + z16 + 16 * k;
      crd[k] = gcol[size_t(v) * nfine + (gzi < F2 ? gzi : F2 - 1)];
    }
  };
  auto project = [&](int v, int gz0, Own& o) {
    int mnx = INT_MIN, mxx = INT_MIN, mny = INT_MIN, mxy = INT_MIN;
#pragma unroll
    for (int k = 0; k < VPT; ++k) {
      const int gzi = gz0 + z16 + 16 * k;
      const bool vin = col_in && gzi < e2;
      o.inside[k] = 0;
      o.xy[k] = 0;
      o.w[k][0] = o.w[k][1] = o.w[k][2] = o.w[k][3] = 0.0f;
      if (vin) {
        float sx, sy;
        if (CACHED) {
          sx = crd[k].x;
          sy = crd[k].y;
        } else {
          project_norm(cm[v], g, wx, wy, fz[gzi], sx, sy);
        }
        int x0, y0;
        tap_origin(sx, sy, W, H, x0, y0, o.w[k], o.inside[k]);
        o.xy[k] = int((unsigned(y0) << 16) | (unsigned(x0) & 0xffffu));
        if (o.inside[k]) {
          mnx = imax(mnx, -imax(x0, 0)); mxx = imax(mxx, imin(x0 + 1, W - 1));
          mny = imax(mny, -imax(y0, 0)); mxy = imax(mxy, imin(y0 + 1, H - 1));
        }
      }
    }
    mnx = row_max(mnx); mxx = row_max(mxx); mny = row_max(mny); mxy = row_max(mxy);
    if ((lane & 15) == 0 && mxx != INT_MIN) {
      int* rc = rect + 4 * (v % 3);
      atomicMax(&rc[0], mnx); atomicMax(&rc[1], mxx); atomicMax(&rc[2], mny); atomicMax(&rc[3], mxy);
    }
  };
  struct Rect { int x0, y0, w, h, pitch; bool any, staged, big, lds; };
  auto read_rect = [&](int v) {
    const int* rc = rect + 4 * (v % 3);
    const int c0 = __builtin_amdgcn_readfirstlane(rc[0]), c1 = __builtin_amdgcn_readfirstlane(rc[1]);
    const int c2 = __builtin_amdgcn_readfirstlane(rc[2]), c3 = __builtin_amdgcn_readfirstlane(rc[3]);
    Rect r;
    r.any = c1 != INT_MIN;
    r.x0 = r.any ? -c0 : 0;
    r.y0 = r.any ? -c2 : 0;
    r.w = r.any ? c1 - r.x0 + 1 : 0;
    r.h = r.any ? c3 - r.y0 + 1 : 0;
    r.pitch = r.w | 1;
    r.staged = r.any && r.h * r.pitch <= cap_lim;
    r.big = r.any && !r.staged && r.h * r.pitch <= 2 * cap_lim && (ablate & 16);
    r.lds = r.staged || r.big;
    return r;
  };
  auto issue_dma = [&](int v, const Rect& r) {
    if (!r.lds || (ablate & 2)) return;
    float* tile = r.big ? smem : smem + (v & 1) * tile_sz;
    const float* plane = frame + size_t(v) * view_stride + (size_t(r.y0) * W + r.x0) * JP;
    const int pq = r.pitch * LQ;
    for (int c0 = 0; c0 < pq; c0 += 64) {
      const int col = c0 + lane;
      int px = col / LQ;
      int cq = col - px * LQ;
      cq = cq < NQ ? cq : NQ - 1;
      px = px < r.w ? px : r.w - 1;
      const float* src0 = plane + size_t(px) * JP + 4 * cq;
      for (int row = wave; row < r.h; row += NT / 64) {
        if (col < pq)
          __builtin_amdgcn_global_load_lds((const __attribute__((address_space(1))) void*)(src0 + size_t(row) * W * JP),
                                           (__attribute__((address_space(3))) void*)(tile + size_t(row * pq + c0) * 4), 16, 0, 0);
      }
    }
  };
  auto finish = [&](const Own& o, int k, const Rect& r) {
    TapL d;
    const int x0 = (o.xy[k] << 16) >> 16, y0 = o.xy[k] >> 16;
    const int rx0 = r.lds ? r.x0 : 0, ry0 = r.lds ? r.y0 : 0;
    const int rx1 = r.lds ? r.x0 + r.w - 1 : W - 1, ry1 = r.lds ? r.y0 + r.h - 1 : H - 1;
    const int pitch = r.lds ? r.pitch : W;
    const int ps = r.lds ? LP : JP;
    const int cx0 = imin(imax(x0, rx0), rx1), cx1 = imin(imax(x0 + 1, rx0), rx1);
    const int cy0 = imin(imax(y0, ry0), ry1), cy1 = imin(imax(y0 + 1, ry0), ry1);
    d.base = ((cy0 - ry0) * pitch + (cx0 - rx0)) * ps;
    d.dx = (cx1 - cx0) * ps;
    d.dy = (cy1 - cy0) * pitch * ps;
#pragma unroll
    for (int c = 0; c < 4; ++c) d.w[c] = ((o.inside[k] >> c) & 1) ? o.w[k][c] : 0.0f;
    return d;
  };

  for (int gz0 = s2; gz0 < e2; gz0 += BZ) {
    if (t < 12) rect[t] = INT_MIN;
    __syncthreads();
    f32x2 acc[VPT][2 * NQ];
#pragma unroll
    for (int k = 0; k < VPT; ++k)
#pragma unroll
      for (int c = 0; c < 2 * NQ; ++c) acc[k][c] = f32x2{0.0f, 0.0f};

    Own cur, nxt;
    if (CACHED) load_coords(0, gz0);
    project(0, gz0, cur);
    __syncthreads();
    Rect rcur = read_rect(0);
    if (rcur.staged) issue_dma(0, rcur);
    if (CACHED && V > 1) load_coords(1, gz0);
    for (int v = 0; v < V; ++v) {
      if (v + 1 < V) project(v + 1, gz0, nxt);
      wait_vmcnt(0);
      __syncthreads();
      Rect rnxt = rcur;
      if (v + 1 < V) rnxt = read_rect(v + 1);
      if (rcur.big) {
        issue_dma(v, rcur);
        if (CACHED && v + 2 < V) load_coords(v + 2, gz0);
        wait_vmcnt(0);
        __syncthreads();
      } else if (v + 1 < V) {
        if (rnxt.staged) issue_dma(v + 1, rnxt);
        if (CACHED && v + 2 < V) load_coords(v + 2, gz0);
      }
      if (t < 4) rect[4 * (v % 3) + t] = INT_MIN;
      if (rcur.any && !(ablate & 1) && (rcur.lds || !(ablate & 8))) {
        const float* src = rcur.big ? smem : (rcur.staged ? smem + (v & 1) * tile_sz : frame + size_t(v) * view_stride);
#pragma unroll
        for (int k = 0; k < VPT; ++k) {
          const TapL d = finish(cur, k, rcur);
          const float* p0 = src + d.base;
          const f32x2 w0 = f32x2{d.w[0], d.w[0]}, w1 = f32x2{d.w[1], d.w[1]}, w2 = f32x2{d.w[2], d.w[2]},
                      w3 = f32x2{d.w[3], d.w[3]};
#pragma unroll
          for (int n = 0; n < NQ; ++n) {
            const float4 v0 = *reinterpret_cast<const float4*>(p0 + 4 * n);
            const float4 v1 = *reinterpret_cast<const float4*>(p0 + d.dx + 4 * n);
            const float4 v2 = *reinterpret_cast<const float4*>(p0 + d.dy + 4 * n);
            const float4 v3 = *reinterpret_cast<const float4*>(p0 + d.dy + d.dx + 4 * n);
            f32x2 lo = f32x2{v0.x, v0.y} * w0, hi = f32x2{v0.z, v0.w} * w0;
            lo = __builtin_elementwise_fma(f32x2{v1.x, v1.y}, w1, lo);
            hi = __builtin_elementwise_fma(f32x2{v1.z, v1.w}, w1, hi);
            lo = __builtin_elementwise_fma(f32x2{v2.x, v2.y}, w2, lo);
            hi = __builtin_elementwise_fma(f32x2{v2.z, v2.w}, w2, hi);
            lo = __builtin_elementwise_fma(f32x2{v3.x, v3.y}, w3, lo);
            hi = __builtin_elementwise_fma(f32x2{v3.z, v3.w}, w3, hi);
            acc[k][2 * n] = acc[k][2 * n] + lo;
            acc[k][2 * n + 1] = acc[k][2 * n + 1] + hi;
          }
        }
      }
      if (rcur.big) {
        __syncthreads();
        if (v + 1 < V && rnxt.staged) issue_dma(v + 1, rnxt);
      }
      cur = nxt;
      rcur = rnxt;
    }
    __syncthreads();
    if (ablate & 4) continue;
    int* cxy = reinterpret_cast<int*>(smem);
    int* cxz = cxy + kBX * kBY * JP;
    int* cyz = cxz + kBX * BZ * JP;
    constexpr int ncell = (kBX * kBY + (kBX + kBY) * BZ) * JP;
    for (int i = t; i < ncell; i += NT) cxy[i] = 0;
    __syncthreads();
#pragma unroll
    for (int c2 = 0; c2 < 2 * NQ; ++c2)
#pragma unroll
      for (int e = 0; e < 2; ++e) {
        const int ch = 2 * c2 + e;
        float mz = 0.0f;
#pragma unroll
        for (int k = 0; k < VPT; ++k) {
          const float val = fmaxf(e ? acc[k][c2].y : acc[k][c2].x, 0.0f);
          mz = fmaxf(mz, val);
          if (val > 0.0f) {
            const int z = z16 + 16 * k;
            atomicMax(&cxz[(xx * BZ + z) * JP + ch], __float_as_int(val));
            atomicMax(&cyz[(yy * BZ + z) * JP + ch], __float_as_int(val));
          }
        }
        const int mi = row_max(__float_as_int(mz));
        if (z16 == 0 && mi > 0) cxy[(xx * kBY + yy) * JP + ch] = mi;
      }
    __syncthreads();
    const int lz0 = gz0 - tl2;
    for (int i = t; i < kBX * kBY * J; i += NT) {
      const int ch = i / (kBX * kBY), col = i - ch * (kBX * kBY), cx = col / kBY, cy = col - cx * kBY;
      const int raw = cxy[col * JP + ch];
      if (raw > 0 && gx0 + cx < e0 && gy0 + cy < e1) {
        const int vv = __float_as_int(clampf(__fdiv_rn(__int_as_float(raw), nv), 0.0f, 1.0f));
        if (vv > 0) plane_max(&pxy[size_t(ch) * CC + (gx0 + cx - tl0) * C + (gy0 + cy - tl1)], vv);
      }
    }
    for (int i = t; i < (kBX + kBY) * BZ * J; i += NT) {
      const int ch = i / ((kBX + kBY) * BZ), r = i - ch * ((kBX + kBY) * BZ), a = r / BZ, z = r - a * BZ;
      if (gz0 + z < e2) {
        const int raw = cxz[r * JP + ch];
        const int vv = raw > 0 ? __float_as_int(clampf(__fdiv_rn(__int_as_float(raw), nv), 0.0f, 1.0f)) : 0;
        if (vv > 0) {
          if (a < kBX) {
            if (gx0 + a < e0) plane_max(&pxz[size_t(ch) * CC + (gx0 + a - tl0) * C + lz0 + z], vv);
          } else if (gy0 + a - kBX < e1) {
            plane_max(&pyz[size_t(ch) * CC + (gy0 + a - kBX - tl1) * C + lz0 + z], vv);
          }
        }
      }
    }
    __syncthreads();
  }
}

#endif

}
```

faster-voxelpose_amd/engine.py:

```python
import ctypes as C

import numpy as np
import torch

from . import _capi as capi
from . import netspec

BN_EPS = 1e-5


def _ptr(t):
    return None if t is None else C.c_void_p(t.data_ptr())


class SharedGeometry:

    def __init__(self):
        self.cams = None
        self.seq_ids = {}
        self.fine_grid = None
        self.fine_grid_key = None
        self.pending = []
        self.users = {}
        self.retired = []

    def retire(self, tensor):
        self.retired = [(t, evs) for t, evs in self.retired if not all(e.query() for e in evs)]
        if tensor is None:
            return
        evs = []
        for st in self.users.values():
            e = torch.cuda.Event()
            e.record(st)
            evs.append(e)
        if evs:
            self.retired.append((tensor, evs))


class HotPath:
    def __init__(self, cfg, _lib=None):
        self._injected = _lib is not None
        self.lib = _lib if _lib is not None else capi.load()
        self.cfg = cfg
        self.device = torch.device(cfg.DEVICE)
        if not self._injected and self.device.type != "cuda":
            raise capi.FvpError(f"cfg.DEVICE={cfg.DEVICE!r}: the HIP path needs a ROCm GPU device "
                                "(spelled 'cuda:N' in PyTorch-ROCm); there is no CPU fallback")
        ds, cs, ins = cfg.DATASET, cfg.CAPTURE_SPEC, cfg.INDIVIDUAL_SPEC
        self.J = int(ds.NUM_JOINTS)
        self.JP = (self.J + 3) // 4 * 4
        self.W, self.H = int(ds.HEATMAP_SIZE[0]), int(ds.HEATMAP_SIZE[1])
        self.N = int(cs.MAX_PEOPLE)
        self.min_score = float(cs.MIN_SCORE)
        self.X, self.Y, self.Z = (int(v) for v in cs.VOXELS_PER_AXIS)
        self.C = int(ins.VOXELS_PER_AXIS[0])
        assert len(set(int(v) for v in ins.VOXELS_PER_AXIS)) == 1, "cubic individual volume expected"
        self.beta = float(cfg.NETWORK.BETA)
        self.F = int(cfg.NETWORK.NUM_CHANNEL_JOINT_FEAT)
        self.Hd = int(cfg.NETWORK.NUM_CHANNEL_JOINT_HIDDEN)
        dev = self.device

        def axes(size, center, nbins):
            return [(torch.linspace(-size[a] / 2, size[a] / 2, int(nbins[a])) + center[a]).to(dev).contiguous()
                    for a in range(3)]
        self.whole_axes = axes(cs.SPACE_SIZE, cs.SPACE_CENTER, cs.VOXELS_PER_AXIS)
        scale = torch.tensor(cs.SPACE_SIZE) / (torch.tensor(cs.VOXELS_PER_AXIS) - 1)
        bias = torch.tensor(cs.SPACE_CENTER) - torch.tensor(cs.SPACE_SIZE) / 2.0
        self.prop_sb = torch.cat([scale, bias]).float().to(dev).contiguous()
        whole_c = torch.tensor(cs.SPACE_CENTER)
        whole_s = torch.tensor(cs.SPACE_SIZE)
        ind_s = torch.tensor(ins.SPACE_SIZE)
        cube = torch.tensor(ins.VOXELS_PER_AXIS, dtype=torch.int32)
        fine = (whole_s / ind_s * (cube - 1)).int() + 1
        ind_scale = (fine.float() - 1) / whole_s
        ind_bias = -ind_s / 2.0 / whole_s * (fine - 1) - ind_scale * (whole_c - whole_s / 2.0)
        self.fine = [int(v) for v in fine]
        self.ind_consts = torch.cat([ind_scale, ind_bias, whole_s, ind_s]).float().to(dev).contiguous()
        self.fine_cube = (C.c_int32 * 6)(*(self.fine + [int(v) for v in cube]))
        self.fine_dev = torch.tensor(self.fine, dtype=torch.int32, device=dev)
        self.fine_host = (C.c_int32 * 3)(*self.fine)
        self.cache_fine_grid = not self._injected
        self.fine_grid_limit_bytes = 2 << 30
        self.fine_grid_total_limit_bytes = 8 << 30
        self.geo = SharedGeometry()
        self.fine_axes = axes(cs.SPACE_SIZE, cs.SPACE_CENTER, self.fine)
        ia = axes(ins.SPACE_SIZE, cs.SPACE_CENTER, ins.VOXELS_PER_AXIS)
        gx, gy, gz = (a.cpu() for a in ia)
        Cn = self.C
        xy = torch.stack([gx.view(Cn, 1).expand(Cn, Cn), gy.view(1, Cn).expand(Cn, Cn)], dim=2).reshape(-1, 2)
        xz = torch.stack([gx.view(Cn, 1).expand(Cn, Cn), gz.view(1, Cn).expand(Cn, Cn)], dim=2).reshape(-1, 2)
        yz = torch.stack([gy.view(Cn, 1).expand(Cn, Cn), gz.view(1, Cn).expand(Cn, Cn)], dim=2).reshape(-1, 2)
        self.center_grid = torch.stack([xy, xz, yz]).to(dev).contiguous()

        self.specs = {
            "center_net": netspec.centernet_spec(self.J, self.X, self.Y),
            "c2c_net": netspec.c2cnet_spec(self.J, self.Z),
            "conv_net": netspec.p2pnet_spec(self.J, self.J, self.C),
        }
        self.params = {k: torch.zeros(max(s.nparams, 4), device=dev) for k, s in self.specs.items()}
        self.wn_params = torch.zeros(self.F * 12 + self.Hd * self.F + 2 * self.Hd + 4, device=dev)
        self._geom = None
        self._geom_key = None
        self._frame_sets = {}
        self._heat_key = None
        self._heat_cl = None
        self._person_frame = {}
        self._scratch = {}
        self.fused_c2c = True
        self.keep_hdn_cubes = False

    def stream(self):
        if self.device.type == "cuda":
            return C.c_void_p(torch.cuda.current_stream(self.device).cuda_stream)
        return None

    def _call(self, name, *args):
        capi.check(self.lib, getattr(self.lib, name)(*args), name)

    def _check_tensor(self, t, what):
        if t.device != self.device and not (self.device.index is None and t.device.type == self.device.type):
            raise capi.FvpError(f"{what} lives on {t.device}, the model was built for {self.device} (cfg.DEVICE)")
        if t.dtype != torch.float32:
            raise capi.FvpError(f"{what} must be float32, got {t.dtype}")

    def geom(self, resize_transform):
        key = None
        if isinstance(resize_transform, torch.Tensor):
            key = (id(resize_transform), resize_transform.data_ptr(), resize_transform._version)
            self._geom_ref = resize_transform
        if self._geom is None or key is None or key != self._geom_key:
            rt = np.asarray(resize_transform.detach().cpu() if isinstance(resize_transform, torch.Tensor)
                            else resize_transform, dtype=np.float32).reshape(6)
            ds = self.cfg.DATASET
            g = capi.FvpGeom()
            g.clamp_max = float(max(ds.ORI_IMAGE_SIZE[0], ds.ORI_IMAGE_SIZE[1]))
            for i in range(6):
                g.rt[i] = float(rt[i])
            g.hm_w, g.hm_h = float(self.W), float(self.H)
            g.img_w, g.img_h = float(ds.IMAGE_SIZE[0]), float(ds.IMAGE_SIZE[1])
            g.W, g.H = self.W, self.H
            g.V = 0
            g.J, g.JP = self.J, self.JP
            self._geom, self._geom_key = g, key
        return self._geom

    @staticmethod
    def _cam_row(cam):
        row = np.zeros(capi.FVP_CAM_FLOATS, np.float32)
        row[0:9] = np.asarray(cam["R"], np.float64).reshape(9)
        row[9:12] = np.asarray(cam["T"], np.float64).reshape(3)
        row[12], row[13] = float(cam["fx"]), float(cam["fy"])
        row[14], row[15] = float(cam["cx"]), float(cam["cy"])
        row[16:19] = np.asarray(cam["k"], np.float64).reshape(3)
        row[19:21] = np.asarray(cam["p"], np.float64).reshape(2)
        return row

    def frame_sets(self, meta, cameras, V):
        geo = self.geo
        seqs = tuple(meta["seq"])
        new = [s for s in dict.fromkeys(seqs) if s not in geo.seq_ids]
        self._await_geometry()
        for s in new:
            assert s in cameras.keys(), "missing camera parameters for the current sequence"
            assert len(cameras[s]) == V, "inconsistent number of cameras"
            rows = np.stack([self._cam_row(cameras[s][c]) for c in range(V)])
            t = torch.from_numpy(rows).to(self.device)
            geo.retire(geo.cams)
            geo.cams = t[None] if geo.cams is None else torch.cat([geo.cams, t[None]], dim=0)
            geo.seq_ids[s] = geo.cams.shape[0] - 1
        if new:
            self._geometry_changed()
        if seqs not in self._frame_sets:
            if len(self._frame_sets) >= 256:
                self._frame_sets.pop(next(iter(self._frame_sets)))
            self._frame_sets[seqs] = torch.tensor([geo.seq_ids[s] for s in seqs], dtype=torch.int32,
                                                  device=self.device)
        return self._frame_sets[seqs]

    def _geometry_changed(self):
        if self.device.type == "cuda":
            ev = torch.cuda.Event()
            ev.record(torch.cuda.current_stream(self.device))
            self.geo.pending.append(ev)

    def _await_geometry(self):
        if self.device.type != "cuda":
            return
        st = torch.cuda.current_stream(self.device)
        geo = self.geo
        geo.users.setdefault(st.cuda_stream, st)
        if geo.pending:
            geo.pending = [ev for ev in geo.pending if not ev.query()]
            for ev in geo.pending:
                st.wait_event(ev)

    def cams_of(self, seq):
        return self.geo.cams[self.geo.seq_ids[seq]]

    def fine_grid_cache(self, resize_transform, V):
        geo = self.geo
        n = self.fine[0] * self.fine[1] * self.fine[2]
        nsets = geo.cams.shape[0]
        if V * n * 8 > self.fine_grid_limit_bytes or nsets * V * n * 8 > self.fine_grid_total_limit_bytes:
            geo.retire(geo.fine_grid)
            geo.fine_grid = None
            return None
        g = self.geom(resize_transform)
        key = (tuple(g.rt), g.clamp_max, V)
        if geo.fine_grid is not None and geo.fine_grid_key != key:
            geo.retire(geo.fine_grid)
            geo.fine_grid = None
        have = 0 if geo.fine_grid is None else geo.fine_grid.shape[0]
        if have < nsets:
            g.V = V
            self._await_geometry()
            new = torch.empty((nsets, V, n, 2), device=self.device)
            if have:
                new[:have] = geo.fine_grid
                geo.retire(geo.fine_grid)
            fa = self.fine_axes
            for i in range(have, nsets):
                self._call("fvp_sample_grid", _ptr(fa[0]), _ptr(fa[1]), _ptr(fa[2]), self.fine[0], self.fine[1],
                           self.fine[2], _ptr(geo.cams[i]), C.byref(g), _ptr(new[i]), self.stream())
            geo.fine_grid, geo.fine_grid_key = new, key
            self._geometry_changed()
        else:
            self._await_geometry()
        return geo.fine_grid

    def heat_cl(self, heatmaps, g, reuse=False):
        self._check_tensor(heatmaps, "heatmaps")
        heatmaps = heatmaps.contiguous()
        key = (heatmaps.data_ptr(), heatmaps._version, tuple(heatmaps.shape))
        if not (reuse or self.__dict__.get("_adopted")) or key != self._heat_key:
            self._adopted = False
            B, V = heatmaps.shape[:2]
            out = self.scratch("heat_cl", (B, V, self.H, self.W, self.JP))
            self._call("fvp_heatmaps_to_cl", _ptr(heatmaps), _ptr(out), B, C.byref(g), self.stream())
            self._heat_cl, self._heat_key = out, key
        return self._heat_cl

    def adopt_staging(self, heatmaps, heat_cl):
        B, V = heatmaps.shape[:2]
        assert heat_cl.is_contiguous() and heat_cl.numel() == B * V * self.H * self.W * self.JP
        self._heat_cl = heat_cl.view(B, V, self.H, self.W, self.JP)
        self._heat_key = (heatmaps.data_ptr(), heatmaps._version, tuple(heatmaps.shape))
        self._adopted = True

    def invalidate_staging(self):
        self._heat_key = None
        self._adopted = False

    def scratch(self, name, shape, dtype=torch.float32, zero=False):
        key = (name, tuple(shape), dtype)
        t = self._scratch.get(key)
        if t is None:
            t = torch.empty(shape, dtype=dtype, device=self.device)
            self._scratch[key] = t
        if zero:
            t.zero_()
        return t

    def pack_stack(self, name, tree):
        spec, blob = self.specs[name], self.params[name]
        s = self.stream()
        for key, bn, transposed, oi in spec.param_keys:
            w = tree.get(key + ".weight")
            self._check_tensor(w, key)
            b = tree.get(key + ".bias")
            bnp = [None] * 4
            if bn is not None:
                bnp = [tree.get(bn + ".weight"), tree.get(bn + ".bias"), tree.get(bn + ".running_mean"),
                       tree.get(bn + ".running_var")]
            self._call("fvp_pack_conv", _ptr(w.contiguous()), _ptr(b), *[_ptr(t) for t in bnp], BN_EPS,
                       1 if transposed else 0, C.byref(spec.op_array[oi]), _ptr(blob), s)

    def pack_weightnet(self, tree):
        g = tree.get
        self._call("fvp_pack_weightnet", _ptr(g("heatmap_feature_net.0.weight").contiguous()),
                   _ptr(g("heatmap_feature_net.0.bias")), _ptr(g("heatmap_feature_net.1.weight")),
                   _ptr(g("heatmap_feature_net.1.bias")), _ptr(g("heatmap_feature_net.1.running_mean")),
                   _ptr(g("heatmap_feature_net.1.running_var")), BN_EPS, _ptr(g("output.0.weight").contiguous()),
                   _ptr(g("output.0.bias")), _ptr(g("output.2.weight").contiguous()), _ptr(g("output.2.bias")),
                   self.F, self.Hd, _ptr(self.wn_params), self.stream())

    def run_stack(self, name, x, planes, plane_valid=None, valid_div=1, fresh=()):
        spec = self.specs[name]
        bufs = [x]
        own = {spec.outputs[k] for k in fresh}
        for i, (c, h, w) in enumerate(spec.bufs[1:], start=1):
            bufs.append(torch.empty((planes, c, h, w), device=self.device) if i in own
                        else self.scratch(f"{name}.buf{i}", (planes, c, h, w)))
        arr = (C.c_void_p * len(bufs))(*[t.data_ptr() for t in bufs])
        self._call("fvp_conv_stack_run", spec.op_array, len(spec.ops), _ptr(self.params[name]), arr, len(bufs),
                   planes, _ptr(plane_valid), valid_div, self.stream())
        return {k: bufs[i] for k, i in spec.outputs.items()}

    def run_stack_fused_1d(self, name, x, planes, fresh=False):
        spec = self.specs[name]
        c, h, w = spec.bufs[spec.outputs["out"]]
        out = torch.empty((planes, c, h, w), device=self.device) if fresh else self.scratch(f"{name}.fused_out", (planes, c, h, w))
        self._call("fvp_conv_stack_run_fused_1d", spec.op_array, len(spec.ops), _ptr(self.params[name]), _ptr(x),
                   _ptr(out), planes, self.stream())
        return {"out": out}

    def project_whole(self, heatmaps, meta, cameras, resize_transform, want_cubes=True, want_zmax=False):
        B, V = heatmaps.shape[:2]
        g = self.geom(resize_transform)
        g.V = V
        fs = self.frame_sets(meta, cameras, V)
        hcl = self.heat_cl(heatmaps, g)
        cubes = torch.empty((B, self.J, self.X, self.Y, self.Z), device=self.device) if want_cubes else None
        zmax = self.scratch("zmax", (B, self.J, self.X, self.Y)) if want_zmax else None
        ax = self.whole_axes
        self._call("fvp_project_whole", _ptr(hcl), _ptr(self.geo.cams), _ptr(fs), _ptr(ax[0]), _ptr(ax[1]), _ptr(ax[2]),
                   self.X, self.Y, self.Z, B, C.byref(g), _ptr(cubes), _ptr(zmax), self.stream())
        return cubes, zmax

    def sample_grid(self, axes3, seq, resize_transform, V):
        g = self.geom(resize_transform)
        g.V = V
        n = axes3[0].numel() * axes3[1].numel() * axes3[2].numel()
        grid = torch.empty((V, 1, n, 2), device=self.device)
        self._call("fvp_sample_grid", _ptr(axes3[0]), _ptr(axes3[1]), _ptr(axes3[2]), axes3[0].numel(),
                   axes3[1].numel(), axes3[2].numel(), _ptr(self.cams_of(seq)), C.byref(g), _ptr(grid), self.stream())
        return grid

    def hdn(self, heatmaps, meta, cameras, resize_transform):
        B = heatmaps.shape[0]
        N, J, X, Y, Z = self.N, self.J, self.X, self.Y, self.Z
        s = self.stream()
        keep = self.keep_hdn_cubes
        cubes, zmax = self.project_whole(heatmaps, meta, cameras, resize_transform, keep, True)
        heads = self.run_stack("center_net", zmax, B, fresh=("output_hm",))
        hm2d = heads["output_hm"]
        bbox_map = heads["output_size"]
        dev = self.device
        conf2d = self.scratch("conf2d", (B, N))
        idx2d = self.scratch("idx2d", (B, N, 2), torch.int64)
        flat = self.scratch("flat", (B, N), torch.int64)
        self._call("fvp_nms_topk", _ptr(hm2d), B, X, Y, N, _ptr(conf2d), _ptr(idx2d), _ptr(flat), s)
        bbox_flat = torch.empty((B, X * Y, 2), device=dev)
        match_bbox = self.scratch("match_bbox", (B, N, 2))
        feat1d = self.scratch("feat1d", (B * N, J, 1, Z))
        if keep:
            self._call("fvp_gather_proposals", _ptr(bbox_map), _ptr(cubes), _ptr(flat), B, J, X, Y, Z, N,
                       _ptr(bbox_flat), _ptr(match_bbox), _ptr(feat1d), s)
        else:
            self._call("fvp_gather_proposals", _ptr(bbox_map), None, _ptr(flat), B, J, X, Y, Z, N, _ptr(bbox_flat),
                       _ptr(match_bbox), None, s)
            g = self.geom(resize_transform)
            ax = self.whole_axes
            self._call("fvp_project_columns", _ptr(self._heat_cl), _ptr(self.geo.cams),
                       _ptr(self.frame_sets(meta, cameras, heatmaps.shape[1])), _ptr(ax[0]), _ptr(ax[1]), _ptr(ax[2]),
                       X, Y, Z, B, C.byref(g), _ptr(flat), N, _ptr(feat1d), s)
        if self.fused_c2c and Z <= 24:
            hm1d = self.run_stack_fused_1d("c2c_net", feat1d, B * N, fresh=True)["out"].view(B, N, Z)
        else:
            hm1d = self.run_stack("c2c_net", feat1d, B * N, fresh=("out",))["out"].view(B, N, Z)
        centers = torch.empty((B, N, 7), device=dev)
        topk_index = self.scratch("topk_index", (B, N, 3), torch.int64)
        valid = self.scratch("proposal_valid", (B, N), torch.uint8)
        self._call("fvp_proposals", _ptr(hm1d), _ptr(conf2d), _ptr(idx2d), _ptr(match_bbox), _ptr(self.prop_sb),
                   self.min_score, B, N, Z, _ptr(topk_index), _ptr(centers), _ptr(valid), s)
        self.last = dict(cubes=cubes, zmax=zmax, conf2d=conf2d, idx2d=idx2d, flat=flat, topk_index=topk_index,
                         bbox_map=bbox_map, feat1d=feat1d, hm2d=hm2d, hm1d=hm1d, bbox_flat=bbox_flat, valid=valid)
        return hm2d, hm1d, centers, bbox_flat

    def proposal_layer(self, topk_index, topk_confs, match_bbox, min_score):
        self._check_tensor(topk_confs, "topk_confs")
        self._check_tensor(match_bbox, "match_bbox_preds")
        B, N = topk_confs.shape
        idx = topk_index.to(torch.int64).contiguous()
        assert idx.shape == (B, N, 3) and match_bbox.shape == (B, N, 2)
        centers = torch.empty((B, N, 7), device=self.device)
        self._call("fvp_proposal_layer", _ptr(idx), _ptr(topk_confs.contiguous()), _ptr(match_bbox.contiguous()),
                   _ptr(self.prop_sb), float(min_score), B, N, _ptr(centers), self.stream())
        return centers

    def person_frame(self, B, N):
        key = (B, N)
        if key not in self._person_frame:
            self._person_frame[key] = (torch.arange(B * N, device=self.device) // N).to(torch.int32)
        return self._person_frame[key]

    def person_boxes(self, centers2d):
        n = centers2d.shape[0]
        boxes = self.scratch("boxes", (n, 9), torch.int32)
        offset = self.scratch("offset", (n, 3))
        self._call("fvp_person_boxes", _ptr(centers2d), n, _ptr(self.ind_consts), self.fine_cube, _ptr(boxes),
                   _ptr(offset), self.stream())
        return boxes, offset

    def softargmax_weightnet(self, joint_features, grids=None):
        x = joint_features
        self._check_tensor(x, "joint_features")
        assert x.dim() == 5 and x.shape[0] == 3 and x.shape[2] == self.J and x.shape[3] == x.shape[4] == self.C
        P, J, Cn = x.shape[1], self.J, self.C
        s = self.stream()
        feat = x.permute(1, 0, 2, 3, 4).contiguous()
        grid = self.center_grid if grids is None else grids.reshape(3, Cn * Cn, 2).contiguous()
        pose2d = torch.empty((P, 3, J, 2), device=self.device)
        pmax = torch.empty((P, 3, J), device=self.device)
        wgt = torch.empty((P, 3, J), device=self.device)
        if P == 0:
            return pose2d.permute(1, 0, 2, 3), torch.empty((0,), device=self.device), wgt.reshape(0, J, 1)
        self._call("fvp_softargmax_weightnet", _ptr(feat), _ptr(grid), _ptr(self.wn_params), self.beta, P, J, Cn,
                   self.F, self.Hd, None, _ptr(pose2d), _ptr(pmax), _ptr(wgt), s)
        centers = torch.zeros((P, 7), device=self.device)
        offset = torch.zeros((P, 3), device=self.device)
        fused5 = torch.empty((P, J, 5), device=self.device)
        planes = torch.empty((3, P, J, 2), device=self.device)
        self._call("fvp_fuse_poses", _ptr(pose2d), _ptr(pmax), _ptr(wgt), _ptr(offset), None, P, J, _ptr(centers),
                   _ptr(fused5), _ptr(planes), s)
        return pose2d.permute(1, 0, 2, 3).contiguous(), centers[:, 4].clone(), \
            wgt.permute(1, 0, 2).reshape(3 * P, J, 1).contiguous()

    def jln(self, meta, heatmaps, proposal_centers, mask, cameras, resize_transform, fused=True,
            reuse_staging=False):
        B, N = proposal_centers.shape[:2]
        V = heatmaps.shape[1]
        J, Cn = self.J, self.C
        nP = B * N
        s = self.stream()
        self._check_tensor(proposal_centers, "proposal_centers")
        assert proposal_centers.is_contiguous(), "proposal_centers must be contiguous (it is updated in place)"
        g = self.geom(resize_transform)
        g.V = V
        fs = self.frame_sets(meta, cameras, V)
        hcl = self.heat_cl(heatmaps, g, reuse=reuse_staging)
        valid = mask.reshape(-1) if (mask.dtype == torch.uint8 and mask.is_contiguous()) else mask.reshape(-1).to(torch.uint8).contiguous()
        pf = self.person_frame(B, N)
        centers2d = proposal_centers.view(nP, 7)
        boxes, offset = self.person_boxes(centers2d)
        fa = self.fine_axes
        planes = self.scratch("planes", (nP, 3, J, Cn, Cn), zero=True)
        if fused:
            fgrid = self.fine_grid_cache(resize_transform, V) if self.cache_fine_grid else None
            self._call("fvp_project_individual_triplane", _ptr(hcl), _ptr(self.geo.cams), _ptr(fs), _ptr(pf), _ptr(valid),
                       _ptr(boxes), _ptr(fa[0]), _ptr(fa[1]), _ptr(fa[2]), self.fine_host, Cn, nP, C.byref(g),
                       _ptr(planes), N, _ptr(fgrid), s)
        else:
            cubes = self.scratch("person_cubes", (nP, J, Cn, Cn, Cn))
            self._call("fvp_project_individual", _ptr(hcl), _ptr(self.geo.cams), _ptr(fs), _ptr(pf), _ptr(valid),
                       _ptr(boxes), _ptr(fa[0]), _ptr(fa[1]), _ptr(fa[2]), _ptr(self.fine_dev), Cn, nP, C.byref(g),
                       _ptr(cubes), s)
            self._call("fvp_triplane_max", _ptr(cubes), _ptr(planes), nP, J, Cn, s)
        feat = self.run_stack("conv_net", planes.view(nP * 3, J, Cn, Cn), nP * 3, valid, 3)["out"]
        pose2d = self.scratch("pose2d", (nP, 3, J, 2))
        pmax = self.scratch("pmax", (nP, 3, J))
        wgt = self.scratch("wgt", (nP, 3, J))
        self._call("fvp_softargmax_weightnet", _ptr(feat), _ptr(self.center_grid), _ptr(self.wn_params), self.beta, nP,
                   J, Cn, self.F, self.Hd, _ptr(valid), _ptr(pose2d), _ptr(pmax), _ptr(wgt), s)
        fused5 = torch.empty((B, N, J, 5), device=self.device)
        plane_poses = torch.empty((3, B, N, J, 2), device=self.device)
        self._call("fvp_fuse_poses", _ptr(pose2d), _ptr(pmax), _ptr(wgt), _ptr(offset), _ptr(valid), nP, J,
                   _ptr(centers2d), _ptr(fused5), _ptr(plane_poses), s)
        self.last_jln = dict(planes=planes, feat=feat, boxes=boxes, offset=offset, pose2d=pose2d, pmax=pmax, wgt=wgt,
                             valid=valid)
        return fused5, plane_poses

    def joint_evidence(self, fused_poses, heatmaps, meta, cameras, resize_transform, reuse_staging=False):
        self._check_tensor(fused_poses, "fused_poses")
        if fused_poses.dim() != 4 or fused_poses.shape[2:] != (self.J, 5) or fused_poses.shape[0] != heatmaps.shape[0] \
                or not fused_poses.is_contiguous():
            raise capi.FvpError(f"fused_poses must be contiguous [B,N,J,5] with B = {heatmaps.shape[0]}, J = {self.J}, "
                                f"got {tuple(fused_poses.shape)}")
        B, N = fused_poses.shape[:2]
        V = heatmaps.shape[1]
        g = self.geom(resize_transform)
        g.V = V
        fs = self.frame_sets(meta, cameras, V)
        hcl = self.heat_cl(heatmaps, g, reuse=reuse_staging)
        views = torch.empty((B, V, N, self.J, 4), device=self.device)
        joint_conf = torch.empty((B, N, self.J), device=self.device)
        if B * N == 0:
            return views, joint_conf
        self._call("fvp_joint_evidence", _ptr(hcl), _ptr(self.geo.cams), _ptr(fs), _ptr(fused_poses), B, N, C.byref(g),
                   _ptr(views), _ptr(joint_conf), self.stream())
        return views, joint_conf
```

faster-voxelpose_amd/models/faster_voxelpose.py:

```python
import time

import torch
import torch.nn as nn

from .. import _capi as capi
from ..dataset.images import Nv12Frames, ingest_frames, ingest_nv12
from ..engine import HotPath
from .human_detection_net import HumanDetectionNet
from .joint_localization_net import JointLocalizationNet


class FasterVoxelPoseNet(nn.Module):
    def __init__(self, cfg, _lib=None):
        super().__init__()
        self.cfg = cfg
        self.max_people = cfg.CAPTURE_SPEC.MAX_PEOPLE
        self.num_joints = cfg.DATASET.NUM_JOINTS
        self.device = torch.device(cfg.DEVICE)
        self.engine = HotPath(cfg, _lib=_lib)
        self.pose_net = HumanDetectionNet(cfg, _engine=self.engine)
        self.joint_net = JointLocalizationNet(cfg, _engine=self.engine)
        self.lambda_loss_2d = cfg.TRAIN.LAMBDA_LOSS_2D
        self.lambda_loss_1d = cfg.TRAIN.LAMBDA_LOSS_1D
        self.lambda_loss_bbox = cfg.TRAIN.LAMBDA_LOSS_BBOX
        self.lambda_loss_fused = cfg.TRAIN.LAMBDA_LOSS_FUSED
        self.evidence = False
        self.last_evidence = None
        self.tracker = None
        self.last_tracks = None
        self.smoother = None
        self.last_smooth = None
        self.overlay = None
        self.last_overlay_views = None
        self.crops = None
        self.last_crops = None
        self.visibility = None
        self.last_visibility = None
        self.eval()

    def joint_evidence(self, fused_poses, input_heatmaps, meta, cameras, resize_transform):
        return self.engine.joint_evidence(fused_poses, input_heatmaps, meta, cameras, resize_transform)

    def forward(self, backbone=None, views=None, meta=None, targets=None, input_heatmaps=None, cameras=None,
                resize_transform=None):
        if self.training:
            raise NotImplementedError("only the inference branch of FasterVoxelPoseNet.forward is implemented "
                                      "(call model.eval()); training losses are outside the hot path")
        if self.smoother is not None and self.tracker is None:
            raise capi.FvpError("model.smoother filters the tracks of model.tracker: set model.tracker (a PoseTracker) too")
        if self.visibility is not None and not self.evidence:
            raise capi.FvpError("model.visibility judges the pixels of model.last_evidence: set model.evidence = True too")
        canvas = None
        if self.overlay is not None:
            if not self.evidence:
                raise capi.FvpError("model.overlay draws the pixels of model.last_evidence: set model.evidence = True too")
            if not (isinstance(views, Nv12Frames) and self.overlay.nv12) \
                    and (not torch.is_tensor(views) or views.dtype != torch.uint8):
                raise capi.FvpError("model.overlay draws into the camera frames: pass them as views, uint8 [B,V,Hs,Ws,3] "
                                    "(NV12 surfaces, float images and input_heatmaps alone leave nothing to draw on; "
                                    "PoseOverlay(..., nv12=True) draws into Nv12Frames views, in the surface itself)")
            canvas = views
        source = None
        if self.crops is not None:
            if not self.evidence:
                raise capi.FvpError("model.crops cuts around the pixels of model.last_evidence: set model.evidence = True too")
            if not isinstance(views, Nv12Frames) and (not torch.is_tensor(views) or views.dtype != torch.uint8):
                raise capi.FvpError("model.crops cuts the patches out of the camera frames: pass them as views, uint8 "
                                    "[B,V,Hs,Ws,3] or Nv12Frames (float images and input_heatmaps alone leave nothing to "
                                    "cut from)")
            source = views
        if views is not None:
            nv12 = isinstance(views, Nv12Frames)
            frames = not nv12 and views.dtype == torch.uint8
            if nv12:
                if len(views.lead) != 2:
                    raise capi.FvpError(f"NV12 views must have leading dimensions [B,V], got {views.lead}")
                if resize_transform is None:
                    raise capi.FvpError("NV12 views need resize_transform (camera -> network pixels) to be resized")
                B, V = views.lead
                if hasattr(backbone, "_run"):
                    nchw, cl = backbone._run(views, True, True, resize_transform=resize_transform)
                    input_heatmaps = nchw.view(B, V, *nchw.shape[1:])
                    if cl.shape[-1] == self.engine.JP:
                        self.engine.adopt_staging(input_heatmaps, cl)
                else:
                    views = ingest_nv12(views, resize_transform, self.cfg.DATASET.IMAGE_SIZE, _lib=self.engine.lib)
                    input_heatmaps = torch.stack([backbone(views[:, c]) for c in range(V)], dim=1)
            elif frames:
                if views.dim() != 5 or views.shape[-1] != 3:
                    raise capi.FvpError(f"uint8 views must be camera frames [B,V,Hs,Ws,3] (HWC), got {tuple(views.shape)}")
                if resize_transform is None:
                    raise capi.FvpError("uint8 views need resize_transform (camera -> network pixels) to be resized")
            if nv12:
                pass
            elif frames and hasattr(backbone, "_run"):
                B, V = views.shape[:2]
                nchw, cl = backbone._run(views.flatten(0, 1), True, True, resize_transform=resize_transform)
                input_heatmaps = nchw.view(B, V, *nchw.shape[1:])
                if cl.shape[-1] == self.engine.JP:
                    self.engine.adopt_staging(input_heatmaps, cl)
            elif frames:
                views = ingest_frames(views, resize_transform, self.cfg.DATASET.IMAGE_SIZE, _lib=self.engine.lib)
                input_heatmaps = torch.stack([backbone(views[:, c]) for c in range(views.shape[1])], dim=1)
            elif hasattr(backbone, "_run"):
                B, V = views.shape[:2]
                nchw, cl = backbone._run(views.flatten(0, 1), True, True)
                input_heatmaps = nchw.view(B, V, *nchw.shape[1:])
                if cl.shape[-1] == self.engine.JP:
                    self.engine.adopt_staging(input_heatmaps, cl)
            else:
                num_views = views.shape[1]
                input_heatmaps = torch.stack([backbone(views[:, c]) for c in range(num_views)], dim=1)
        _, _, proposal_centers, _ = self.pose_net(input_heatmaps, meta, cameras, resize_transform)
        mask = self.engine.last["valid"]
        fused_poses, plane_poses = self.joint_net.forward5(meta, input_heatmaps, proposal_centers, mask, cameras,
                                                           resize_transform, _reuse_staging=True)
        if self.evidence:
            self.last_evidence = self.engine.joint_evidence(fused_poses, input_heatmaps, meta, cameras, resize_transform,
                                                            reuse_staging=True)
        conf = self.last_evidence[1] if self.evidence else None
        if self.visibility is not None:
            vis = self.visibility
            ws, hs = self.cfg.DATASET.ORI_IMAGE_SIZE
            fs = self.engine.frame_sets(meta, cameras, input_heatmaps.shape[1])
            self.last_visibility = vis(fused_poses, self.engine.geo.cams, fs, views=self.last_evidence[0],
                                       frame_size=vis.frame_size or (hs, ws))
            if vis.feeds_conf:
                conf = self.last_visibility[1]
        if self.tracker is not None:
            if len(self.engine.geo.seq_ids) > self.tracker.nseq:
                raise capi.FvpError(f"the engine has seen {len(self.engine.geo.seq_ids)} sequences, model.tracker was "
                                    f"built for nseq = {self.tracker.nseq}")
            fs = self.engine.frame_sets(meta, cameras, input_heatmaps.shape[1])
            self.last_tracks = self.tracker.update(fused_poses, sequences=fs)
            if self.smoother is not None:
                if self.smoother.nseq < self.tracker.nseq:
                    raise capi.FvpError(f"model.smoother was built for nseq = {self.smoother.nseq}, model.tracker for "
                                        f"{self.tracker.nseq}")
                self.last_smooth = self.smoother.update(fused_poses, self.last_tracks[0], self.last_tracks[1],
                                                        joint_conf=conf, sequences=fs)
        if canvas is not None or source is not None:
            px, self.last_overlay_views = self.last_evidence[0], None
            if self.smoother is not None:
                px = self.engine.joint_evidence(self.last_smooth[0], input_heatmaps, meta, cameras, resize_transform,
                                                reuse_staging=True)[0]
                self.last_overlay_views = px
            ids = self.last_tracks[0] if self.tracker is not None else None
            if source is not None:
                self.last_crops = self.crops(source, px, ids=ids, joint_conf=conf)
            if canvas is not None:
                self.overlay.draw(canvas, px, ids=ids, joint_conf=conf)
        self.engine.invalidate_staging()
        return fused_poses, plane_poses, proposal_centers, input_heatmaps, None


class GraphedForward:

    def __init__(self, model, meta, input_heatmaps, cameras, resize_transform, warmup=2):
        self.model = model
        self.static_in = input_heatmaps.clone()
        self.args = dict(meta=meta, cameras=cameras, resize_transform=resize_transform)
        side = torch.cuda.Stream(device=input_heatmaps.device)
        side.wait_stream(torch.cuda.current_stream())
        with torch.cuda.stream(side), torch.no_grad():
            for _ in range(warmup):
                model(input_heatmaps=self.static_in, **self.args)
        torch.cuda.current_stream().wait_stream(side)
        torch.cuda.current_stream().synchronize()
        geo = model.engine.geo
        geo.pending = [ev for ev in geo.pending if not ev.query()]
        self.graph = torch.cuda.CUDAGraph()
        with torch.cuda.graph(self.graph), torch.no_grad():
            self.out = model(input_heatmaps=self.static_in, **self.args)
        self._pinned = (geo.cams, geo.fine_grid)

    def __call__(self, input_heatmaps=None):
        if input_heatmaps is not None and input_heatmaps.data_ptr() != self.static_in.data_ptr():
            self.static_in.copy_(input_heatmaps, non_blocking=True)
        self.graph.replay()
        return self.out


class PipelinedForward:

    def __init__(self, model, depth=2, streams=None, backpressure=True):
        assert depth >= 1
        assert streams is None or len(streams) >= depth
        if model.tracker is not None:
            raise capi.FvpError("PipelinedForward runs batches on several streams and replicas: set model.tracker = None "
                                "and call tracker.update(outputs[0], meta) on the consumer stream in submit order")
        if model.smoother is not None:
            raise capi.FvpError("PipelinedForward runs batches on several streams and replicas: set model.smoother = None "
                                "and call smoother.update(outputs[0], ids, slots, meta=meta) behind tracker.update on the "
                                "consumer stream in submit order")
        if model.overlay is not None:
            raise capi.FvpError("PipelinedForward runs batches on several streams and replicas: set model.overlay = None "
                                "and call overlay.draw(frames, views, ids) on the consumer stream")
        if model.crops is not None:
            raise capi.FvpError("PipelinedForward runs batches on several streams and replicas: set model.crops = None "
                                "and call crops(frames, views, ids) on the consumer stream, with views from "
                                "model.joint_evidence(outputs[0], ...)[0], before any overlay.draw")
        if model.visibility is not None:
            raise capi.FvpError("PipelinedForward runs batches on several streams and replicas: set model.visibility = None "
                                "and call visibility(outputs[0], cameras, meta, views=views) on the consumer stream, with "
                                "views from model.joint_evidence(outputs[0], ...)[0]")
        self.models = [model]
        self.streams = list(streams[:depth]) if streams is not None else [torch.cuda.Stream(device=model.device) for _ in range(depth)]
        for _ in range(1, depth):
            m = FasterVoxelPoseNet(model.cfg).to(model.device)
            m.load_state_dict(model.state_dict())
            m.eval()
            m.evidence = model.evidence
            m.engine.geo = model.engine.geo
            self.models.append(m)
        self.depth = depth
        self._i = 0
        self.backpressure = bool(backpressure)
        self._last = [None] * depth
        self.wait_s = 0.0

    def submit(self, **forward_kwargs):
        k = self._i % self.depth
        self._i += 1
        st = self.streams[k]
        if self.backpressure and self._last[k] is not None:
            t0 = time.perf_counter()
            self._last[k].synchronize()
            self.wait_s += time.perf_counter() - t0
        st.wait_stream(torch.cuda.current_stream())
        for v in forward_kwargs.values():
            if torch.is_tensor(v) and v.is_cuda:
                v.record_stream(st)
        with torch.cuda.stream(st), torch.no_grad():
            out = self.models[k](**forward_kwargs)
            ev = torch.cuda.Event()
            ev.record(st)
        self._last[k] = ev
        return out, ev

    @staticmethod
    def consume(outputs, stream=None):
        stream = stream or torch.cuda.current_stream()
        for t in outputs:
            if torch.is_tensor(t) and t.is_cuda:
                t.record_stream(stream)

    def synchronize(self):
        for st in self.streams:
            st.synchronize()


class GraphedPipeline:

    def __init__(self, model, depth, meta, input_heatmaps, cameras, resize_transform, streams=None, warmup=2):
        self.pipe = PipelinedForward(model, depth=depth, streams=streams)
        self.depth, self._i = depth, 0
        args = dict(meta=meta, cameras=cameras, resize_transform=resize_transform)
        self.static_in, self.graphs, self.outs, self._pinned = [], [], [], []
        cur = torch.cuda.current_stream()
        for k in range(depth):
            st, m = self.pipe.streams[k], self.pipe.models[k]
            buf = input_heatmaps.clone()
            st.wait_stream(cur)
            with torch.cuda.stream(st), torch.no_grad():
                for _ in range(warmup):
                    m(input_heatmaps=buf, **args)
            st.synchronize()
            geo = m.engine.geo
            geo.pending = [ev for ev in geo.pending if not ev.query()]
            assert not geo.pending, "a geometry rebuild is still running on another stream: synchronise before capturing"
            g = torch.cuda.CUDAGraph()
            with torch.cuda.graph(g, stream=st), torch.no_grad():
                out = m(input_heatmaps=buf, **args)
            self._pinned.append((geo.cams, geo.fine_grid))
            self.static_in.append(buf)
            self.graphs.append(g)
            self.outs.append(out)
        torch.cuda.synchronize()

    def submit(self, input_heatmaps):
        k = self._i % self.depth
        self._i += 1
        st = self.pipe.streams[k]
        st.wait_stream(torch.cuda.current_stream())
        input_heatmaps.record_stream(st)
        with torch.cuda.stream(st):
            self.static_in[k].copy_(input_heatmaps, non_blocking=True)
            self.graphs[k].replay()
            ev = torch.cuda.Event()
            ev.record(st)
        return self.outs[k], ev

    def synchronize(self):
        self.pipe.synchronize()


def get(cfg):
    return FasterVoxelPoseNet(cfg)
```

include/fvp.h:

```cpp
#ifndef FVP_H_
#define FVP_H_

#include <stdint.h>

#ifdef __cplusplus
extern "C" {
#endif

#define FVP_ABI_VERSION 17
#define FVP_MAX_VIEWS 8
#define FVP_CAM_FLOATS 24
#define FVP_MAX_JOINTS 32
#define FVP_TRACK_MAX_DETS 32
#define FVP_TRACK_MAX_TRACKS 64
#define FVP_VIS_MAX_PEOPLE 32
#define FVP_VIS_MAX_PRIMS 64

#define FVP_EINVAL 10001
#define FVP_ELIMIT 10002

typedef void* fvp_stream_t;

typedef struct FvpGeom {
  float clamp_max;
  float rt[6];
  float hm_w, hm_h;
  float img_w, img_h;
  int32_t W, H;
  int32_t V, J;
  int32_t JP;
} FvpGeom;

int fvp_version(void);
int fvp_diag_build(void);
int fvp_sizeof(int what);
const char* fvp_error_string(int code);

int fvp_heatmaps_to_cl(const float* heat, float* heat_cl, int B, const FvpGeom* g, fvp_stream_t s);

int fvp_sample_grid(const float* ax, const float* ay, const float* az, int nx, int ny, int nz,
                    const float* cams, const FvpGeom* g, float* grid, fvp_stream_t s);

int fvp_project_whole(const float* heat_cl, const float* cams, const int32_t* frame_set,
                      const float* ax, const float* ay, const float* az, int X, int Y, int Z, int B,
                      const FvpGeom* g, float* cubes, float* zmax, fvp_stream_t s);

int fvp_project_columns(const float* heat_cl, const float* cams, const int32_t* frame_set, const float* ax,
                        const float* ay, const float* az, int X, int Y, int Z, int B, const FvpGeom* g,
                        const int64_t* flat, int N, float* feat1d, fvp_stream_t s);

int fvp_joint_evidence(const float* heat_cl, const float* cams, const int32_t* frame_set,
                       const float* fused_poses, int B, int N, const FvpGeom* g,
                       float* views , float* joint_conf , fvp_stream_t s);

int fvp_track_update(const float* fused_poses, const int32_t* frame_set, float* trk_pose, int32_t* trk_id,
                     int32_t* trk_age, int32_t* next_id, int32_t* ids , int32_t* slots ,
                     float* costs , int B, int N, int J, int nseq, int T, float gate_mm, int max_age,
                     fvp_stream_t s);

int fvp_track_smooth(const float* fused_poses, const int32_t* frame_set, const int32_t* ids, const int32_t* slots,
                     const float* joint_conf, float* flt_pose, float* flt_vel, int32_t* flt_id, int32_t* flt_age,
                     float* smooth , float* track_poses ,
                     int32_t* track_state , int B, int N, int J, int nseq, int T, float rate_hz,
                     float min_cutoff, float beta, float d_cutoff, float conf_min, float damp, int max_age,
                     fvp_stream_t s);

int fvp_zmax(const float* cubes, float* zmax, long n, int Z, fvp_stream_t s);

int fvp_person_boxes(const float* centers, int n, const float* consts, const int32_t* fine_cube,
                     int32_t* boxes, float* offset, fvp_stream_t s);

int fvp_project_individual(const float* heat_cl, const float* cams, const int32_t* frame_set,
                           const int32_t* person_frame, const uint8_t* person_valid, const int32_t* boxes,
                           const float* fx, const float* fy, const float* fz, const int32_t* fine, int C,
                           int nP, const FvpGeom* g, float* cubes, fvp_stream_t s);

int fvp_triplane_max(const float* cubes, float* planes, int nP, int J, int C, fvp_stream_t s);

int fvp_project_individual_triplane(const float* heat_cl, const float* cams, const int32_t* frame_set,
                                    const int32_t* person_frame, const uint8_t* person_valid,
                                    const int32_t* boxes, const float* fx, const float* fy, const float* fz,
                                    const int32_t* fine, int C, int nP, const FvpGeom* g, float* planes,
                                    int persons_per_frame, const float* fine_grid, fvp_stream_t s);

enum {
  FVP_OP_CONV = 0,
  FVP_OP_POOL2 = 1,
  FVP_OP_CONVT2 = 2
};
enum {
  FVP_EPI_RELU = 1,
  FVP_EPI_RES = 2,
  FVP_EPI_RES_AFTER_RELU = 4
};
typedef struct FvpConvOp {
  int32_t kind;
  int32_t src, dst, res;
  int32_t cin, cout;
  int32_t kh, kw;
  int32_t h, w;
  int32_t flags;
  int32_t w_off;
  int32_t e_off;
  int32_t cinp, coutp;
  int32_t wino_off;
  int32_t pair_off;
} FvpConvOp;

int fvp_conv_stack_run(const FvpConvOp* ops, int nops, const float* params, float* const* bufs, int nbufs,
                       int planes, const uint8_t* plane_valid, int valid_div, fvp_stream_t s);

int fvp_conv_stack_run_fused_1d(const FvpConvOp* ops, int nops, const float* params, const float* in,
                                float* out, int planes, fvp_stream_t s);

int fvp_pack_conv(const float* weight, const float* bias, const float* bn_gamma, const float* bn_beta,
                  const float* bn_mean, const float* bn_var, float eps, int transposed, const FvpConvOp* op,
                  float* params, fvp_stream_t s);

int fvp_nms_topk(const float* hm2d, int B, int X, int Y, int N, float* vals, int64_t* idx, int64_t* flat,
                 fvp_stream_t s);

int fvp_gather_proposals(const float* bbox_map, const float* cubes, const int64_t* flat, int B, int J, int X,
                         int Y, int Z, int N, float* bbox_flat, float* match_bbox, float* feat1d,
                         fvp_stream_t s);

int fvp_proposals(const float* hm1d, const float* conf2d, const int64_t* idx2d, const float* match_bbox,
                  const float* sb, float min_score, int B, int N, int Z, int64_t* topk_index, float* centers,
                  uint8_t* valid, fvp_stream_t s);

int fvp_proposal_layer(const int64_t* topk_index, const float* topk_confs, const float* match_bbox, const float* sb,
                       float min_score, int B, int N, float* centers, fvp_stream_t s);

int fvp_softargmax_weightnet(const float* feat, const float* center_grid, const float* wn, float beta,
                             int nP, int J, int C, int F, int Hd, const uint8_t* person_valid, float* pose2d,
                             float* pmax, float* wgt, fvp_stream_t s);
int fvp_pack_weightnet(const float* conv_w, const float* conv_b, const float* bn_gamma, const float* bn_beta,
                       const float* bn_mean, const float* bn_var, float eps, const float* fc1_w,
                       const float* fc1_b, const float* fc2_w, const float* fc2_b, int F, int Hd, float* wn,
                       fvp_stream_t s);

int fvp_fuse_poses(const float* pose2d, const float* pmax, const float* wgt, const float* offset,
                   const uint8_t* person_valid, int nP, int J, float* centers, float* fused_poses,
                   float* plane_poses, fvp_stream_t s);

int fvp_rasterise_heatmaps(const double* joints, const int32_t* num_people, int nimg, int P, int J, int W, int H,
                           double feat_stride_x, double feat_stride_y, double sigma, float* heat_nchw,
                           float* heat_cl, int JP, fvp_stream_t s);

enum { FVP_INGEST_SWAP_RB = 1, FVP_INGEST_GENERAL = 2 };
int fvp_ingest_frames(const uint8_t* frames, int N, int Hs, int Ws, const float inv[6], const float mean[3],
                      const float stdv[3], int H, int W, int flags, uint16_t* nhwc8, float* nchw, fvp_stream_t s);

enum { FVP_YUV_BT601_LIMITED = 0, FVP_YUV_BT709_LIMITED = 1, FVP_YUV_BT601_FULL = 2, FVP_YUV_BT709_FULL = 3 };
#define FVP_YUV_BT601_LIMITED_COEFFS { 16, 1220945, 1673555, -410793, -852458, 2115221 }
#define FVP_YUV_BT709_LIMITED_COEFFS { 16, 1220945, 1879825, -223607, -558796, 2215014 }
#define FVP_YUV_BT601_FULL_COEFFS { 0, 1048576, 1470104, -360853, -748826, 1858077 }
#define FVP_YUV_BT709_FULL_COEFFS { 0, 1048576, 1651297, -196424, -490864, 1945738 }
int fvp_ingest_nv12(const uint8_t* y, const uint8_t* uv, int N, int Hs, int Ws, long y_pitch, long uv_pitch,
                    long y_frame_stride, long uv_frame_stride,
                    int standard, const float inv[6], const float mean[3], const float stdv[3], int H, int W,
                    uint16_t* nhwc8, float* nchw, fvp_stream_t s);

int fvp_draw_poses(uint8_t* frames , int B, int V, int Hs, int Ws,
                   const float* views ,
                   const int32_t* ids , const float* joint_conf ,
                   int N, int J, const int32_t* limbs , int L,
                   const uint8_t* palette , int P,
                   int joint_radius_q4, int limb_half_q4, int alpha, float conf_min, fvp_stream_t s);

#define FVP_RGB2YUV_BT601_LIMITED_COEFFS { 16, 16829, 33039, 6416, 128, -9714, -19071, 28784, 128, 28784, -24103, -4681 }
#define FVP_RGB2YUV_BT709_LIMITED_COEFFS { 16, 11966, 40254, 4064, 128, -6596, -22189, 28784, 128, 28784, -26145, -2639 }
#define FVP_RGB2YUV_BT601_FULL_COEFFS { 0, 19595, 38470, 7471, 128, -11058, -21710, 32768, 128, 32768, -27439, -5329 }
#define FVP_RGB2YUV_BT709_FULL_COEFFS { 0, 13933, 46871, 4732, 128, -7509, -25259, 32768, 128, 32768, -29763, -3005 }
int fvp_draw_poses_nv12(uint8_t* y, uint8_t* uv , int B, int V, int Hs, int Ws, long y_pitch, long uv_pitch,
                        long y_frame_stride, long uv_frame_stride,
                        int standard , const float* views ,
                        const int32_t* ids , const float* joint_conf ,
                        int N, int J, const int32_t* limbs , int L,
                        const uint8_t* palette , int P,
                        int joint_radius_q4, int limb_half_q4, int alpha, float conf_min, fvp_stream_t s);

int fvp_person_rois(const float* views , const int32_t* ids ,
                    const float* joint_conf , int B, int V, int N, int J, uint32_t joint_mask,
                    int min_joints, float scale, float pad_px, float aspect, float conf_min,
                    float* rois , int32_t* roi_count , float* roi_score ,
                    fvp_stream_t s);

int fvp_crop_rois(const uint8_t* frames , int F, int Hs, int Ws, const float* rois ,
                  int R, int rois_per_frame, const float mean[3], const float stdv[3], int h, int w, int flags,
                  uint16_t* nhwc8 , float* nchw , fvp_stream_t s);
int fvp_crop_rois_nv12(const uint8_t* y, const uint8_t* uv, int F, int Hs, int Ws, long y_pitch, long uv_pitch,
                       long y_frame_stride, long uv_frame_stride,
                       int standard , const float* rois , int R, int rois_per_frame,
                       const float mean[3], const float stdv[3], int h, int w, uint16_t* nhwc8, float* nchw,
                       fvp_stream_t s);

int fvp_joint_visibility(const float* fused_poses , const float* cams ,
                         const int32_t* frame_set , const int32_t* ids ,
                         const float* views ,
                         int B, int V, int N, int J,
                         const int32_t* prims , const float* radius_mm , int L,
                         float guard_mm, int Hs, int Ws,
                         int32_t* occluder , float* vis_conf ,
                         int32_t* vis_count , fvp_stream_t s);

enum { FVP_BB_CONV = 0, FVP_BB_MAXPOOL = 1, FVP_BB_DECONV = 2 };
enum { FVP_BB_OUT_HEAT = 8,
       FVP_BB_STEM = 16,
       FVP_BB_CFG_SHIFT = 8 };
typedef struct FvpBbOp {
  int32_t kind;
  int32_t src, dst, res;
  int32_t cin, cinp;
  int32_t cout, coutp, cbuf;
  int32_t kh, kw, stride, pad;
  int32_t h, w, oh, ow;
  int32_t flags;
  int32_t w_off;
  int32_t e_off;
} FvpBbOp;
int fvp_bb_input(const float* images, uint16_t* nhwc8, int N, int C, int H, int W, fvp_stream_t s);
int fvp_bb_pack(const float* weight, const float* bias, const float* bn_gamma, const float* bn_beta,
                const float* bn_mean, const float* bn_var, float eps, const FvpBbOp* op, uint16_t* wblob,
                float* eblob, fvp_stream_t s);
int fvp_bb_run(const FvpBbOp* ops, int nops, const uint16_t* wblob, const float* eblob, void* const* bufs, int nbufs,
               int N, float* heat_cl, int heat_jp, float* heat_nchw, fvp_stream_t s);
int fvp_bb_tune(FvpBbOp* ops, int nops, const uint16_t* wblob, const float* eblob, void* const* bufs, int nbufs, int N,
                fvp_stream_t s);

enum { FVP_K_PROJECT_WHOLE = 0, FVP_K_PROJECT_TRIPLANE = 1, FVP_K_CONV = 2, FVP_K_SOFTARGMAX = 3,
       FVP_K_OTHER = 4, FVP_K_CONV_WINO = 5, FVP_K_BACKBONE = 6, FVP_K_CONV_WINO_SMALL = 7, FVP_K_COUNT = 8 };
int fvp_prof_enable(int on);
int fvp_prof_read(int cls, double* ms, int64_t* launches, double* flops);
int fvp_prof_reset(void);

#ifdef __cplusplus
}
#endif
#endif
```

Before: 3029.

## Cache projected sampling grid for whole-space projection and add 32-bit offset triplane path

Adds a per-camera-set cached table of normalized image coordinates for the coarse whole-space voxel grid, so the whole and column projection kernels read precomputed coordinates instead of projecting each voxel through the camera model every frame. It also adds a triplane kernel variant that uses 32-bit byte offsets for heatmap loads when the buffer fits, and flips the DPP bound_ctrl flag in the quad broadcast. The cost is extra memory traffic for reading the cached grid (8 bytes per view per voxel) and added GPU memory, in exchange for less per-voxel projection arithmetic.

```diff
diff --git a/faster-voxelpose_amd/_capi.py b/faster-voxelpose_amd/_capi.py
--- a/faster-voxelpose_amd/_capi.py
+++ b/faster-voxelpose_amd/_capi.py
@@ -3,7 +3,7 @@
 
 _HERE = os.path.dirname(os.path.abspath(__file__))
 LIB_NAME = "libfvp_hip.so"
-ABI_VERSION = 17
+ABI_VERSION = 18
 LIB_PATH = os.path.join(_HERE, LIB_NAME)
 
 FVP_CAM_FLOATS = 24
@@ -56,6 +56,8 @@
     "fvp_sample_grid": [_P, _P, _P, _I, _I, _I, _P, _G, _P, _P],
     "fvp_project_whole": [_P, _P, _P, _P, _P, _P, _I, _I, _I, _I, _G, _P, _P, _P],
     "fvp_project_columns": [_P, _P, _P, _P, _P, _P, _I, _I, _I, _I, _G, _P, _I, _P, _P],
+    "fvp_project_whole_grid": [_P, _P, _P, _P, _P, _P, _I, _I, _I, _I, _G, _P, _P, _P, _P],
+    "fvp_project_columns_grid": [_P, _P, _P, _P, _P, _P, _I, _I, _I, _I, _G, _P, _I, _P, _P, _P],
     "fvp_joint_evidence": [_P, _P, _P, _P, _I, _I, _G, _P, _P, _P],
     "fvp_track_update": [_P, _P, _P, _P, _P, _P, _P, _P, _P, _I, _I, _I, _I, _I, _F, _I, _P],
     "fvp_track_smooth": [_P] * 12 + [_I] * 5 + [_F] * 6 + [_I, _P],
diff --git a/faster-voxelpose_amd/csrc/fvp_project.hip b/faster-voxelpose_amd/csrc/fvp_project.hip
--- a/faster-voxelpose_amd/csrc/fvp_project.hip
+++ b/faster-voxelpose_amd/csrc/fvp_project.hip
@@ -338,7 +338,7 @@
 
 template <int SRC>
 __device__ __forceinline__ int quad_bcast_i(int v) {
-  return __builtin_amdgcn_update_dpp(0, v, SRC * 0x55, 0xf, 0xf, false);
+  return __builtin_amdgcn_update_dpp(0, v, SRC * 0x55, 0xf, 0xf, true);
 }
 template <int SRC>
 __device__ __forceinline__ TapD quad_bcast(const TapD& t) {
@@ -352,15 +352,19 @@
   return r;
 }
 
+__device__ __forceinline__ TapD taps_of(const FvpGeom& g, float gx, float gy) {
+  const Taps t = bilinear_taps(gx, gy, g.W, g.H);
+  TapD d;
+#pragma unroll
+  for (int k = 0; k < 4; ++k) { d.off[k] = t.off[k]; d.w[k] = t.w[k]; }
+  d.inside = t.inside;
+  return d;
+}
+
 __device__ __forceinline__ TapD make_taps(const Cam& cm, const FvpGeom& g, float wx, float wy, float wz) {
   float gx, gy;
   project_norm(cm, g, wx, wy, wz, gx, gy);
-  const Taps t = bilinear_taps(gx, gy, g.W, g.H);
-  TapD d;
-#pragma unroll
-  for (int k = 0; k < 4; ++k) { d.off[k] = t.off[k]; d.w[k] = t.w[k]; }
-  d.inside = t.inside;
-  return d;
+  return taps_of(g, gx, gy);
 }
 
 __device__ __forceinline__ void sample4(const float* __restrict__ cl, int JP, int ch0, const TapD& t, bool first,
@@ -385,10 +389,10 @@
   for (int i = 0; i < 4; ++i) acc[i] = first ? s[i] : __fadd_rn(acc[i], s[i]);
 }
 
-template <int NVL>
+template <int NVL, bool CACHED>
 __device__ __forceinline__ void whole_point_quad(const float* __restrict__ frame, const Cam* __restrict__ cm,
                                                  const FvpGeom& g, int q, bool active, float wx, float wy, float wz,
-                                                 float (&out)[NVL][4]) {
+                                                 const float2* __restrict__ gv, size_t nvox, float (&out)[NVL][4]) {
   const int JP = g.JP;
   const size_t view_stride = size_t(g.H) * g.W * JP;
   float acc[NVL][4];
@@ -400,7 +404,16 @@
   mine.inside = 0;
 #pragma unroll
   for (int k = 0; k < 4; ++k) { mine.off[k] = 0; mine.w[k] = 0.0f; }
-  if (active && q < g.V) mine = make_taps(cm[q], g, wx, wy, wz);
+  [[maybe_unused]] float2 cnext = make_float2(0.0f, 0.0f);
+  if constexpr (CACHED) {
+    if (active && q < g.V) {
+      const float2 c = gv[size_t(q) * nvox];
+      mine = taps_of(g, c.x, c.y);
+    }
+    if (active && g.V > 4) cnext = gv[size_t(4) * nvox];
+  } else {
+    if (active && q < g.V) mine = make_taps(cm[q], g, wx, wy, wz);
+  }
   auto add_view = [&](const TapD& tv, int v) {
 #pragma unroll
     for (int n = 0; n < NVL; ++n) {
@@ -415,8 +428,15 @@
   if (g.V > 1) { const TapD tv = quad_bcast<1>(mine); if (active) add_view(tv, 1); }
   if (g.V > 2) { const TapD tv = quad_bcast<2>(mine); if (active) add_view(tv, 2); }
   if (g.V > 3) { const TapD tv = quad_bcast<3>(mine); if (active) add_view(tv, 3); }
-  for (int v = 4; v < g.V; ++v)
-    if (active) add_view(make_taps(cm[v], g, wx, wy, wz), v);
+  for (int v = 4; v < g.V; ++v) {
+    if constexpr (CACHED) {
+      const float2 c = cnext;
+      if (active && v + 1 < g.V) cnext = gv[size_t(v + 1) * nvox];
+      if (active) add_view(taps_of(g, c.x, c.y), v);
+    } else {
+      if (active) add_view(make_taps(cm[v], g, wx, wy, wz), v);
+    }
+  }
   const float nv = float(g.V);
 #pragma unroll
   for (int n = 0; n < NVL; ++n)
@@ -424,12 +444,12 @@
     for (int i = 0; i < 4; ++i) out[n][i] = clampf(__fdiv_rn(acc[n][i], nv), 0.0f, 1.0f);
 }
 
-template <int NVL>
+template <int NVL, bool CACHED = false>
 __global__ void __launch_bounds__(1024)
 k_project_whole_q(const float* __restrict__ heat_cl, const Cam* __restrict__ cams,
                   const int* __restrict__ frame_set, const float* __restrict__ ax, const float* __restrict__ ay,
                   const float* __restrict__ az, int X, int Y, int Z, int B, int nblk, FvpGeom g,
-                  float* __restrict__ cubes, float* __restrict__ zmax) {
+                  float* __restrict__ cubes, float* __restrict__ zmax, const float* __restrict__ grid) {
   __shared__ float sm[16 * NVL][256];
   const int cpb = 256 / Z;
   int b, bxi;
@@ -450,17 +470,19 @@
   const size_t view_stride = size_t(g.H) * g.W * JP;
   const float* frame = heat_cl + size_t(b) * g.V * view_stride;
   const Cam* cm = cams + size_t(frame_set[b]) * g.V;
+  const size_t vox = size_t(col) * Z + z;
+  const size_t nvox = size_t(ncol) * Z;
   float wx = 0.0f, wy = 0.0f, wz = 0.0f;
-  if (active) {
+  if (!CACHED && active) {
     const int x = col / Y, y = col - x * Y;
     wx = ax[x];
     wy = ay[y];
     wz = az[z];
   }
+  const float2* gv = CACHED ? reinterpret_cast<const float2*>(grid) + size_t(frame_set[b]) * g.V * nvox + (active ? vox : 0)
+                            : nullptr;
   float val[NVL][4];
-  whole_point_quad<NVL>(frame, cm, g, q, active, wx, wy, wz, val);
-  const size_t vox = size_t(col) * Z + z;
-  const size_t nvox = size_t(ncol) * Z;
+  whole_point_quad<NVL, CACHED>(frame, cm, g, q, active, wx, wy, wz, gv, nvox, val);
 #pragma unroll
   for (int n = 0; n < NVL; ++n)
 #pragma unroll
@@ -484,11 +506,12 @@
   }
 }
 
-template <int NVL>
+template <int NVL, bool CACHED = false>
 __global__ void __launch_bounds__(1024)
 k_project_columns_q(const float* __restrict__ heat_cl, const Cam* __restrict__ cams, const int* __restrict__ frame_set,
                     const float* __restrict__ ax, const float* __restrict__ ay, const float* __restrict__ az, int Y,
-                    int Z, int ncol, int N, FvpGeom g, const long long* __restrict__ flat, float* __restrict__ feat1d) {
+                    int Z, int ncol, int N, FvpGeom g, const long long* __restrict__ flat, float* __restrict__ feat1d,
+                    const float* __restrict__ grid) {
   const int pi = blockIdx.x, b = pi / N;
   const int t = threadIdx.x, q = t & 3, z = t >> 2;
   const long long col = flat[pi];
@@ -498,14 +521,18 @@
   const float* frame = heat_cl + size_t(b) * g.V * view_stride;
   const Cam* cm = cams + size_t(frame_set[b]) * g.V;
   float wx = 0.0f, wy = 0.0f, wz = 0.0f;
-  if (active) {
+  if (!CACHED && active) {
     const int x = int(col) / Y, y = int(col) - x * Y;
     wx = ax[x];
     wy = ay[y];
     wz = az[z];
   }
+  const size_t nvox = size_t(ncol) * Z;
+  const float2* gv = CACHED ? reinterpret_cast<const float2*>(grid) + size_t(frame_set[b]) * g.V * nvox +
+                                  (active ? size_t(col) * Z + z : 0)
+                            : nullptr;
   float val[NVL][4];
-  whole_point_quad<NVL>(frame, cm, g, q, active, wx, wy, wz, val);
+  whole_point_quad<NVL, CACHED>(frame, cm, g, q, active, wx, wy, wz, gv, nvox, val);
 #pragma unroll
   for (int n = 0; n < NVL; ++n)
 #pragma unroll
@@ -745,9 +772,9 @@
   return launch_status();
 }
 
-extern "C" int fvp_project_whole(const float* heat_cl, const float* cams, const int32_t* frame_set,
-                                 const float* ax, const float* ay, const float* az, int X, int Y, int Z, int B,
-                                 const FvpGeom* g, float* cubes, float* zmax, fvp_stream_t s) {
+extern "C" int fvp_project_whole_grid(const float* heat_cl, const float* cams, const int32_t* frame_set,
+                                      const float* ax, const float* ay, const float* az, int X, int Y, int Z, int B,
+                                      const FvpGeom* g, float* cubes, float* zmax, const float* grid, fvp_stream_t s) {
   FVP_REQUIRE(heat_cl && cams && frame_set && ax && ay && az && (cubes || zmax) && X > 0 && Y > 0 && Z > 0);
   if (int e = check_geom(g)) return e;
   FVP_LIMIT(Z <= 256);
@@ -758,12 +785,12 @@
   const int nvl = ceil_div(g->JP, 16);
   if (!no_quad && nvl <= 2) {
     const int nblk = ceil_div(X * Y, cpb);
-    if (nvl == 1)
-      hipLaunchKernelGGL(k_project_whole_q<1>, dim3(nblk * B), dim3(1024), 0, as_stream(s), heat_cl,
-                         reinterpret_cast<const Cam*>(cams), frame_set, ax, ay, az, X, Y, Z, B, nblk, *g, cubes, zmax);
-    else
-      hipLaunchKernelGGL(k_project_whole_q<2>, dim3(nblk * B), dim3(1024), 0, as_stream(s), heat_cl,
-                         reinterpret_cast<const Cam*>(cams), frame_set, ax, ay, az, X, Y, Z, B, nblk, *g, cubes, zmax);
+#define CALLW(NVL_, CACHED_)                                                                                            \
+  hipLaunchKernelGGL((k_project_whole_q<NVL_, CACHED_>), dim3(nblk * B), dim3(1024), 0, as_stream(s), heat_cl,        \
+                     reinterpret_cast<const Cam*>(cams), frame_set, ax, ay, az, X, Y, Z, B, nblk, *g, cubes, zmax, grid)
+    if (nvl == 1) { if (grid) CALLW(1, true); else CALLW(1, false); }
+    else { if (grid) CALLW(2, true); else CALLW(2, false); }
+#undef CALLW
     return launch_status();
   }
 #define CALL(NV)                                                                                              \
@@ -773,6 +800,12 @@
   FVP_NV_SWITCH(g->JP / 4, CALL)
 #undef CALL
   return launch_status();
+}
+
+extern "C" int fvp_project_whole(const float* heat_cl, const float* cams, const int32_t* frame_set,
+                                 const float* ax, const float* ay, const float* az, int X, int Y, int Z, int B,
+                                 const FvpGeom* g, float* cubes, float* zmax, fvp_stream_t s) {
+  return fvp_project_whole_grid(heat_cl, cams, frame_set, ax, ay, az, X, Y, Z, B, g, cubes, zmax, nullptr, s);
 }
 
 extern "C" int fvp_joint_evidence(const float* heat_cl, const float* cams, const int32_t* frame_set,
@@ -816,24 +849,30 @@
   return launch_status();
 }
 
-extern "C" int fvp_project_columns(const float* heat_cl, const float* cams, const int32_t* frame_set, const float* ax,
-                                   const float* ay, const float* az, int X, int Y, int Z, int B, const FvpGeom* g,
-                                   const int64_t* flat, int N, float* feat1d, fvp_stream_t s) {
+extern "C" int fvp_project_columns_grid(const float* heat_cl, const float* cams, const int32_t* frame_set,
+                                        const float* ax, const float* ay, const float* az, int X, int Y, int Z, int B,
+                                        const FvpGeom* g, const int64_t* flat, int N, float* feat1d, const float* grid,
+                                        fvp_stream_t s) {
   FVP_REQUIRE(heat_cl && cams && frame_set && ax && ay && az && flat && feat1d && X > 0 && Y > 0 && Z > 0 && N > 0);
   if (int e = check_geom(g)) return e;
   FVP_LIMIT(Z <= 256 && g->JP <= 32);
   if (B == 0) return 0;
   ProfScope ps(FVP_K_PROJECT_WHOLE, as_stream(s));
   const int threads = ceil_div(4 * Z, 64) * 64;
-  if (g->JP <= 16)
-    hipLaunchKernelGGL(k_project_columns_q<1>, dim3(B * N), dim3(threads), 0, as_stream(s), heat_cl,
-                       reinterpret_cast<const Cam*>(cams), frame_set, ax, ay, az, Y, Z, X * Y, N, *g,
-                       reinterpret_cast<const long long*>(flat), feat1d);
-  else
-    hipLaunchKernelGGL(k_project_columns_q<2>, dim3(B * N), dim3(threads), 0, as_stream(s), heat_cl,
-                       reinterpret_cast<const Cam*>(cams), frame_set, ax, ay, az, Y, Z, X * Y, N, *g,
-                       reinterpret_cast<const long long*>(flat), feat1d);
+#define CALLC(NVL_, CACHED_)                                                                                            \
+  hipLaunchKernelGGL((k_project_columns_q<NVL_, CACHED_>), dim3(B * N), dim3(threads), 0, as_stream(s), heat_cl,       \
+                     reinterpret_cast<const Cam*>(cams), frame_set, ax, ay, az, Y, Z, X * Y, N, *g,                     \
+                     reinterpret_cast<const long long*>(flat), feat1d, grid)
+  if (g->JP <= 16) { if (grid) CALLC(1, true); else CALLC(1, false); }
+  else { if (grid) CALLC(2, true); else CALLC(2, false); }
+#undef CALLC
   return launch_status();
+}
+
+extern "C" int fvp_project_columns(const float* heat_cl, const float* cams, const int32_t* frame_set, const float* ax,
+                                   const float* ay, const float* az, int X, int Y, int Z, int B, const FvpGeom* g,
+                                   const int64_t* flat, int N, float* feat1d, fvp_stream_t s) {
+  return fvp_project_columns_grid(heat_cl, cams, frame_set, ax, ay, az, X, Y, Z, B, g, flat, N, feat1d, nullptr, s);
 }
 
 extern "C" int fvp_zmax(const float* cubes, float* zmax, long n, int Z, fvp_stream_t s) {
@@ -984,7 +1023,19 @@
   }
 #endif
     const bool q5 = nvl == 2 && g->JP == 20 && !zres && fvp::diag_env("FVP_TRI_NO_Q5") == nullptr;
-    if (q5) {
+    const char* o32_env = fvp::diag_env("FVP_TRI_NO_O32");
+    const int o32_off = o32_env ? atoi(o32_env) : 0;
+    const bool o32 = fine_grid && !zres && size_t(g->H) * g->W * g->JP * 4 < (size_t(1) << 31) && o32_off != 1;
+#define CALLO(NVL_, Q5_, JPC_)                                                                                             \
+  hipLaunchKernelGGL((k_project_triplane_blk_o32<NVL_, Q5_, JPC_>), dim3(nbx2 * nby * nP), dim3(kBlkThreads), lds_b,      \
+                     as_stream(s), heat_cl, reinterpret_cast<const Cam*>(cams), frame_set, person_frame, person_valid, boxes, \
+                     fx, fy, fz, C, nP, nbx2, nby, ppf, *g, fine_grid, F0, F1, F2, planes, zsh)
+    if (o32) {
+      if (q5) CALLO(2, true, 0);
+      else if (nvl == 2) CALLO(2, false, 0);
+      else if (g->JP == 16 && o32_off != 2) CALLO(1, false, 16);
+      else CALLO(1, false, 0);
+    } else if (q5) {
       if (fine_grid)
         hipLaunchKernelGGL((k_project_triplane_blk<2, true, false, true>), dim3(nbx2 * nby * nP), dim3(kBlkThreads), lds_b, as_stream(s),
                            heat_cl, reinterpret_cast<const Cam*>(cams), frame_set, person_frame, person_valid, boxes, fx, fy, fz, C, nP,
@@ -994,6 +1045,7 @@
                            heat_cl, reinterpret_cast<const Cam*>(cams), frame_set, person_frame, person_valid, boxes, fx, fy, fz, C, nP,
                            nbx2, nby, ppf, *g, fine_grid, F0, F1, F2, planes, zsh);
     } else if (nvl == 2) CALLB2(2) else CALLB2(1)
+#undef CALLO
 #undef CALLB2
 #undef CALLB
     return launch_status();
diff --git a/faster-voxelpose_amd/csrc/fvp_project_lds.h b/faster-voxelpose_amd/csrc/fvp_project_lds.h
--- a/faster-voxelpose_amd/csrc/fvp_project_lds.h
+++ b/faster-voxelpose_amd/csrc/fvp_project_lds.h
@@ -19,6 +19,11 @@
 }
 __device__ __forceinline__ float4 glb_ld4(const float* p) {
   const f32x4v v = *(const __attribute__((address_space(1))) f32x4v*)p;
+  return make_float4(v.x, v.y, v.z, v.w);
+}
+
+__device__ __forceinline__ float4 glb_ld4_o(const char* base, unsigned off) {
+  const f32x4v v = *(const __attribute__((address_space(1))) f32x4v*)(base + off);
   return make_float4(v.x, v.y, v.z, v.w);
 }
 
@@ -406,14 +411,15 @@
 #define FVP_TRI_ZRES_MAX_KB 48
 #endif
 constexpr size_t kTriZresMaxLds = size_t(FVP_TRI_ZRES_MAX_KB) * 1024;
-template <int NVL, bool CACHED, bool ZRES, bool Q5 = false>
-__global__ void __launch_bounds__(kBlkThreads, FVP_TRI_BLK_OCC)
-k_project_triplane_blk(const float* __restrict__ heat_cl, const Cam* __restrict__ cams, const int* __restrict__ frame_set,
-                       const int* __restrict__ person_frame, const uint8_t* __restrict__ person_valid,
-                       const int* __restrict__ boxes, const float* __restrict__ fx, const float* __restrict__ fy,
-                       const float* __restrict__ fz, int C, int nP, int nbx, int nby, int ppf, FvpGeom g,
-                       const float* __restrict__ fgrid, int F0, int F1, int F2, float* __restrict__ planes, int zsh) {
+template <int NVL, bool CACHED, bool ZRES, bool Q5, bool OFF32, int JPC>
+__device__ __forceinline__ void
+triplane_blk_body(const float* __restrict__ heat_cl, const Cam* __restrict__ cams, const int* __restrict__ frame_set,
+                  const int* __restrict__ person_frame, const uint8_t* __restrict__ person_valid,
+                  const int* __restrict__ boxes, const float* __restrict__ fx, const float* __restrict__ fy,
+                  const float* __restrict__ fz, int C, int nP, int nbx, int nby, int ppf, const FvpGeom& g,
+                  const float* __restrict__ fgrid, int F0, int F1, int F2, float* __restrict__ planes, int zsh) {
   static_assert(!Q5 || (NVL == 2 && !ZRES), "the five-quad form replaces the two-group form of the per-z-block kernel");
+  static_assert(JPC == 0 || (JPC == 16 && NVL == 1 && !Q5), "the compile-time joint count is the one-quad-per-lane form's");
   constexpr int NVA = Q5 ? 1 : NVL;
   constexpr int BZ = NVL == 1 ? kBlkBZ : 16;
   constexpr int VPT = BZ / 4;
@@ -421,7 +427,8 @@
   HIP_DYNAMIC_SHARED(float, smem)
   constexpr int NT = kBlkThreads;
   constexpr int kBX = kBlkBX;
-  const int J = g.J, JP = g.JP, CC = C * C, V = g.V, W = g.W, H = g.H;
+  const int J = g.J, JP = JPC ? JPC : g.JP, CC = C * C, V = g.V, W = g.W, H = g.H;
+  constexpr int kOffScale = OFF32 ? 4 : 1;
   int p, blk;
   {
     const int id = blockIdx.x;
@@ -521,9 +528,9 @@
           tap_origin(sx, sy, W, H, x0, y0, w4, inside);
           const int cx0 = imin(imax(x0, 0), W - 1), cx1 = imin(imax(x0 + 1, 0), W - 1);
           const int cy0 = imin(imax(y0, 0), H - 1), cy1 = imin(imax(y0 + 1, 0), H - 1);
-          d.base = (cy0 * W + cx0) * JP;
-          d.dx = (cx1 - cx0) * JP;
-          d.dy = (cy1 - cy0) * W * JP;
+          d.base = (cy0 * W + cx0) * JP * kOffScale;
+          d.dx = (cx1 - cx0) * JP * kOffScale;
+          d.dy = (cy1 - cy0) * W * JP * kOffScale;
 #pragma unroll
           for (int c = 0; c < 4; ++c) d.w[c] = ((inside >> c) & 1) ? w4[c] : 0.0f;
         }
@@ -534,35 +541,68 @@
       if (mine[0].base != -12345) { acc[0][0][0] += mine[0].w[0] + mine[OWN - 1].w[3] + float(mine[0].base); continue; }
 #endif
       const float* gsrc = frame + size_t(v) * view_stride;
+      auto load4 = [&](const TapL& tv, int ch0, float4 (&t)[4]) {
+        if constexpr (OFF32) {
+          const char* vb = reinterpret_cast<const char*>(gsrc);
+          const unsigned o0 = unsigned(tv.base) + unsigned(ch0) * 4u, o2 = o0 + unsigned(tv.dy);
+          t[0] = glb_ld4_o(vb, o0);
+          t[1] = glb_ld4_o(vb, o0 + unsigned(tv.dx));
+          t[2] = glb_ld4_o(vb, o2);
+          t[3] = glb_ld4_o(vb, o2 + unsigned(tv.dx));
+        } else {
+          const float* p0 = gsrc + tv.base + ch0;
+          t[0] = glb_ld4(p0);
+          t[1] = glb_ld4(p0 + tv.dx);
+          t[2] = glb_ld4(p0 + tv.dy);
+          t[3] = glb_ld4(p0 + tv.dy + tv.dx);
+        }
+      };
+      auto accum4 = [&](const TapL& tv, const float4 (&t)[4], float (&a)[4]) {
+        const f32x2 w0 = f32x2{tv.w[0], tv.w[0]}, w1 = f32x2{tv.w[1], tv.w[1]}, w2 = f32x2{tv.w[2], tv.w[2]},
+                    w3 = f32x2{tv.w[3], tv.w[3]};
+        f32x2 lo = f32x2{t[0].x, t[0].y} * w0, hi = f32x2{t[0].z, t[0].w} * w0;
+        lo = __builtin_elementwise_fma(f32x2{t[1].x, t[1].y}, w1, lo);
+        hi = __builtin_elementwise_fma(f32x2{t[1].z, t[1].w}, w1, hi);
+        lo = __builtin_elementwise_fma(f32x2{t[2].x, t[2].y}, w2, lo);
+        hi = __builtin_elementwise_fma(f32x2{t[2].z, t[2].w}, w2, hi);
+        lo = __builtin_elementwise_fma(f32x2{t[3].x, t[3].y}, w3, lo);
+        hi = __builtin_elementwise_fma(f32x2{t[3].z, t[3].w}, w3, hi);
+        const f32x2 alo = f32x2{a[0], a[1]} + lo, ahi = f32x2{a[2], a[3]} + hi;
+        a[0] = alo.x; a[1] = alo.y; a[2] = ahi.x; a[3] = ahi.y;
+      };
       auto sample = [&](const TapL& tv, auto& a, auto own) {
         constexpr bool kOwn = decltype(own)::value;
 #pragma unroll
         for (int n = 0; n < (kOwn ? 1 : NVA); ++n) {
           const int ch0 = kOwn ? 16 : 16 * n + 4 * q;
-          if (kOwn || ch0 < JP) {
-            const float* p0 = gsrc + tv.base + ch0;
-            const float4 v0 = glb_ld4(p0), v1 = glb_ld4(p0 + tv.dx), v2 = glb_ld4(p0 + tv.dy), v3 = glb_ld4(p0 + tv.dy + tv.dx);
-            const f32x2 w0 = f32x2{tv.w[0], tv.w[0]}, w1 = f32x2{tv.w[1], tv.w[1]}, w2 = f32x2{tv.w[2], tv.w[2]},
-                        w3 = f32x2{tv.w[3], tv.w[3]};
-            f32x2 lo = f32x2{v0.x, v0.y} * w0, hi = f32x2{v0.z, v0.w} * w0;
-            lo = __builtin_elementwise_fma(f32x2{v1.x, v1.y}, w1, lo);
-            hi = __builtin_elementwise_fma(f32x2{v1.z, v1.w}, w1, hi);
-            lo = __builtin_elementwise_fma(f32x2{v2.x, v2.y}, w2, lo);
-            hi = __builtin_elementwise_fma(f32x2{v2.z, v2.w}, w2, hi);
-            lo = __builtin_elementwise_fma(f32x2{v3.x, v3.y}, w3, lo);
-            hi = __builtin_elementwise_fma(f32x2{v3.z, v3.w}, w3, hi);
-            const f32x2 alo = f32x2{a[n][0], a[n][1]} + lo, ahi = f32x2{a[n][2], a[n][3]} + hi;
-            a[n][0] = alo.x; a[n][1] = alo.y; a[n][2] = ahi.x; a[n][3] = ahi.y;
+          if (kOwn || JPC != 0 || ch0 < JP) {
+            float4 t[4];
+            load4(tv, ch0, t);
+            accum4(tv, t, a[n]);
           }
         }
       };
 #pragma unroll
       for (int k = 0; k < OWN; ++k) {
-        { const TapL tv = quad_bcast_l<0>(mine[k]); sample(tv, acc[4 * k + 0], std::false_type{}); }
-        { const TapL tv = quad_bcast_l<1>(mine[k]); sample(tv, acc[4 * k + 1], std::false_type{}); }
-        { const TapL tv = quad_bcast_l<2>(mine[k]); sample(tv, acc[4 * k + 2], std::false_type{}); }
-        { const TapL tv = quad_bcast_l<3>(mine[k]); sample(tv, acc[4 * k + 3], std::false_type{}); }
-        if constexpr (Q5) sample(mine[k], accx[k], std::true_type{});
+        if constexpr (JPC != 0) {
+          const int ch0 = 4 * q;
+#pragma unroll
+          for (int h = 0; h < 2; ++h) {
+            const TapL ta = h == 0 ? quad_bcast_l<0>(mine[k]) : quad_bcast_l<2>(mine[k]);
+            const TapL tb = h == 0 ? quad_bcast_l<1>(mine[k]) : quad_bcast_l<3>(mine[k]);
+            float4 va[4], vb[4];
+            load4(ta, ch0, va);
+            load4(tb, ch0, vb);
+            accum4(ta, va, acc[4 * k + 2 * h + 0][0]);
+            accum4(tb, vb, acc[4 * k + 2 * h + 1][0]);
+          }
+        } else {
+          { const TapL tv = quad_bcast_l<0>(mine[k]); sample(tv, acc[4 * k + 0], std::false_type{}); }
+          { const TapL tv = quad_bcast_l<1>(mine[k]); sample(tv, acc[4 * k + 1], std::false_type{}); }
+          { const TapL tv = quad_bcast_l<2>(mine[k]); sample(tv, acc[4 * k + 2], std::false_type{}); }
+          { const TapL tv = quad_bcast_l<3>(mine[k]); sample(tv, acc[4 * k + 3], std::false_type{}); }
+          if constexpr (Q5) sample(mine[k], accx[k], std::true_type{});
+        }
       }
     }
 #ifdef FVP_TRI_BLK_NOMAX
@@ -705,6 +745,25 @@
     }
   }
 }
+
+#define FVP_TRI_BLK_PARAMS                                                                                                \
+  const float* __restrict__ heat_cl, const Cam* __restrict__ cams, const int* __restrict__ frame_set,                      \
+      const int* __restrict__ person_frame, const uint8_t* __restrict__ person_valid, const int* __restrict__ boxes,       \
+      const float* __restrict__ fx, const float* __restrict__ fy, const float* __restrict__ fz, int C, int nP, int nbx,     \
+      int nby, int ppf, FvpGeom g, const float* __restrict__ fgrid, int F0, int F1, int F2, float* __restrict__ planes,     \
+      int zsh
+#define FVP_TRI_BLK_ARGS \
+  heat_cl, cams, frame_set, person_frame, person_valid, boxes, fx, fy, fz, C, nP, nbx, nby, ppf, g, fgrid, F0, F1, F2, planes, zsh
+template <int NVL, bool CACHED, bool ZRES, bool Q5 = false>
+__global__ void __launch_bounds__(kBlkThreads, FVP_TRI_BLK_OCC) k_project_triplane_blk(FVP_TRI_BLK_PARAMS) {
+  triplane_blk_body<NVL, CACHED, ZRES, Q5, false, 0>(FVP_TRI_BLK_ARGS);
+}
+template <int NVL, bool Q5, int JPC>
+__global__ void __launch_bounds__(kBlkThreads, FVP_TRI_BLK_OCC) k_project_triplane_blk_o32(FVP_TRI_BLK_PARAMS) {
+  triplane_blk_body<NVL, true, false, Q5, true, JPC>(FVP_TRI_BLK_ARGS);
+}
+#undef FVP_TRI_BLK_ARGS
+#undef FVP_TRI_BLK_PARAMS
 
 #if FVP_DIAG
 template <int NQ, bool CACHED>
diff --git a/faster-voxelpose_amd/engine.py b/faster-voxelpose_amd/engine.py
--- a/faster-voxelpose_amd/engine.py
+++ b/faster-voxelpose_amd/engine.py
@@ -20,6 +20,8 @@
         self.seq_ids = {}
         self.fine_grid = None
         self.fine_grid_key = None
+        self.whole_grid = None
+        self.whole_grid_key = None
         self.pending = []
         self.users = {}
         self.retired = []
@@ -82,6 +84,7 @@
         self.cache_fine_grid = not self._injected
         self.fine_grid_limit_bytes = 2 << 30
         self.fine_grid_total_limit_bytes = 8 << 30
+        self.cache_whole_grid = True
         self.geo = SharedGeometry()
         self.fine_axes = axes(cs.SPACE_SIZE, cs.SPACE_CENTER, self.fine)
         ia = axes(ins.SPACE_SIZE, cs.SPACE_CENTER, ins.VOXELS_PER_AXIS)
@@ -197,36 +200,44 @@
     def cams_of(self, seq):
         return self.geo.cams[self.geo.seq_ids[seq]]
 
-    def fine_grid_cache(self, resize_transform, V):
+    def _grid_cache(self, which, axes3, dims, resize_transform, V):
         geo = self.geo
-        n = self.fine[0] * self.fine[1] * self.fine[2]
+        name, kname = which + "_grid", which + "_grid_key"
+        n = dims[0] * dims[1] * dims[2]
         nsets = geo.cams.shape[0]
         if V * n * 8 > self.fine_grid_limit_bytes or nsets * V * n * 8 > self.fine_grid_total_limit_bytes:
-            geo.retire(geo.fine_grid)
-            geo.fine_grid = None
+            geo.retire(getattr(geo, name))
+            setattr(geo, name, None)
             return None
         g = self.geom(resize_transform)
         key = (tuple(g.rt), g.clamp_max, V)
-        if geo.fine_grid is not None and geo.fine_grid_key != key:
-            geo.retire(geo.fine_grid)
-            geo.fine_grid = None
-        have = 0 if geo.fine_grid is None else geo.fine_grid.shape[0]
+        if getattr(geo, name) is not None and getattr(geo, kname) != key:
+            geo.retire(getattr(geo, name))
+            setattr(geo, name, None)
+        cur = getattr(geo, name)
+        have = 0 if cur is None else cur.shape[0]
         if have < nsets:
             g.V = V
             self._await_geometry()
             new = torch.empty((nsets, V, n, 2), device=self.device)
             if have:
-                new[:have] = geo.fine_grid
-                geo.retire(geo.fine_grid)
-            fa = self.fine_axes
+                new[:have] = cur
+                geo.retire(cur)
             for i in range(have, nsets):
-                self._call("fvp_sample_grid", _ptr(fa[0]), _ptr(fa[1]), _ptr(fa[2]), self.fine[0], self.fine[1],
-                           self.fine[2], _ptr(geo.cams[i]), C.byref(g), _ptr(new[i]), self.stream())
-            geo.fine_grid, geo.fine_grid_key = new, key
+                self._call("fvp_sample_grid", _ptr(axes3[0]), _ptr(axes3[1]), _ptr(axes3[2]), dims[0], dims[1],
+                           dims[2], _ptr(geo.cams[i]), C.byref(g), _ptr(new[i]), self.stream())
+            setattr(geo, name, new)
+            setattr(geo, kname, key)
             self._geometry_changed()
         else:
             self._await_geometry()
-        return geo.fine_grid
+        return getattr(geo, name)
+
+    def fine_grid_cache(self, resize_transform, V):
+        return self._grid_cache("fine", self.fine_axes, self.fine, resize_transform, V)
+
+    def whole_grid_cache(self, resize_transform, V):
+        return self._grid_cache("whole", self.whole_axes, (self.X, self.Y, self.Z), resize_transform, V)
 
     def heat_cl(self, heatmaps, g, reuse=False):
         self._check_tensor(heatmaps, "heatmaps")
@@ -313,8 +324,9 @@
         cubes = torch.empty((B, self.J, self.X, self.Y, self.Z), device=self.device) if want_cubes else None
         zmax = self.scratch("zmax", (B, self.J, self.X, self.Y)) if want_zmax else None
         ax = self.whole_axes
-        self._call("fvp_project_whole", _ptr(hcl), _ptr(self.geo.cams), _ptr(fs), _ptr(ax[0]), _ptr(ax[1]), _ptr(ax[2]),
-                   self.X, self.Y, self.Z, B, C.byref(g), _ptr(cubes), _ptr(zmax), self.stream())
+        wgrid = self.whole_grid_cache(resize_transform, V) if self.cache_whole_grid else None
+        self._call("fvp_project_whole_grid", _ptr(hcl), _ptr(self.geo.cams), _ptr(fs), _ptr(ax[0]), _ptr(ax[1]),
+                   _ptr(ax[2]), self.X, self.Y, self.Z, B, C.byref(g), _ptr(cubes), _ptr(zmax), _ptr(wgrid), self.stream())
         return cubes, zmax
 
     def sample_grid(self, axes3, seq, resize_transform, V):
@@ -351,9 +363,11 @@
                        _ptr(match_bbox), None, s)
             g = self.geom(resize_transform)
             ax = self.whole_axes
-            self._call("fvp_project_columns", _ptr(self._heat_cl), _ptr(self.geo.cams),
-                       _ptr(self.frame_sets(meta, cameras, heatmaps.shape[1])), _ptr(ax[0]), _ptr(ax[1]), _ptr(ax[2]),
-                       X, Y, Z, B, C.byref(g), _ptr(flat), N, _ptr(feat1d), s)
+            V = heatmaps.shape[1]
+            wgrid = self.whole_grid_cache(resize_transform, V) if self.cache_whole_grid else None
+            self._call("fvp_project_columns_grid", _ptr(self._heat_cl), _ptr(self.geo.cams),
+                       _ptr(self.frame_sets(meta, cameras, V)), _ptr(ax[0]), _ptr(ax[1]), _ptr(ax[2]),
+                       X, Y, Z, B, C.byref(g), _ptr(flat), N, _ptr(feat1d), _ptr(wgrid), s)
         if self.fused_c2c and Z <= 24:
             hm1d = self.run_stack_fused_1d("c2c_net", feat1d, B * N, fresh=True)["out"].view(B, N, Z)
         else:
diff --git a/faster-voxelpose_amd/models/faster_voxelpose.py b/faster-voxelpose_amd/models/faster_voxelpose.py
--- a/faster-voxelpose_amd/models/faster_voxelpose.py
+++ b/faster-voxelpose_amd/models/faster_voxelpose.py
@@ -172,7 +172,7 @@
         self.graph = torch.cuda.CUDAGraph()
         with torch.cuda.graph(self.graph), torch.no_grad():
             self.out = model(input_heatmaps=self.static_in, **self.args)
-        self._pinned = (geo.cams, geo.fine_grid)
+        self._pinned = (geo.cams, geo.fine_grid, geo.whole_grid)
 
     def __call__(self, input_heatmaps=None):
         if input_heatmaps is not None and input_heatmaps.data_ptr() != self.static_in.data_ptr():
@@ -212,6 +212,7 @@
             m.eval()
             m.evidence = model.evidence
             m.engine.geo = model.engine.geo
+            m.engine.cache_fine_grid, m.engine.cache_whole_grid = model.engine.cache_fine_grid, model.engine.cache_whole_grid
             self.models.append(m)
         self.depth = depth
         self._i = 0
@@ -272,7 +273,7 @@
             g = torch.cuda.CUDAGraph()
             with torch.cuda.graph(g, stream=st), torch.no_grad():
                 out = m(input_heatmaps=buf, **args)
-            self._pinned.append((geo.cams, geo.fine_grid))
+            self._pinned.append((geo.cams, geo.fine_grid, geo.whole_grid))
             self.static_in.append(buf)
             self.graphs.append(g)
             self.outs.append(out)
diff --git a/include/fvp.h b/include/fvp.h
--- a/include/fvp.h
+++ b/include/fvp.h
@@ -7,7 +7,7 @@
 extern "C" {
 #endif
 
-#define FVP_ABI_VERSION 17
+#define FVP_ABI_VERSION 18
 #define FVP_MAX_VIEWS 8
 #define FVP_CAM_FLOATS 24
 #define FVP_MAX_JOINTS 32
@@ -48,6 +48,13 @@
 int fvp_project_columns(const float* heat_cl, const float* cams, const int32_t* frame_set, const float* ax,
                         const float* ay, const float* az, int X, int Y, int Z, int B, const FvpGeom* g,
                         const int64_t* flat, int N, float* feat1d, fvp_stream_t s);
+
+int fvp_project_whole_grid(const float* heat_cl, const float* cams, const int32_t* frame_set, const float* ax,
+                           const float* ay, const float* az, int X, int Y, int Z, int B, const FvpGeom* g,
+                           float* cubes, float* zmax, const float* grid, fvp_stream_t s);
+int fvp_project_columns_grid(const float* heat_cl, const float* cams, const int32_t* frame_set, const float* ax,
+                             const float* ay, const float* az, int X, int Y, int Z, int B, const FvpGeom* g,
+                             const int64_t* flat, int N, float* feat1d, const float* grid, fvp_stream_t s);
 
 int fvp_joint_evidence(const float* heat_cl, const float* cams, const int32_t* frame_set,
                        const float* fused_poses, int B, int N, const FvpGeom* g,
```

New measurement: 3037 (median of 6 runs). Within noise of the previous version (+0.3%).
